# Dahan-Wang/Rethinking-Flow-and-Diffusion-Bridge-Models-for-Speech-Enhancement

Hardware: NVIDIA B200
Metric: enhanced audio-sec/sec (5-step SB bridge, ncsnpp_v2) (higher is better)
Workload: dtype fp16

## Files before the change

### include/fdbm_b200.h

```cpp
#ifndef FDBM_B200_H
#define FDBM_B200_H

#include <stddef.h>
#include <stdint.h>

#ifdef __cplusplus
extern "C" {
#endif

#define FDBM_OK        0
#define FDBM_EINVAL   -1
#define FDBM_ECUDA    -2
#define FDBM_EARCH    -3
#define FDBM_ESTATE   -4

#define FDBM_PAD_ZERO        0
#define FDBM_PAD_REFLECTION  1
#define FDBM_PAD_REPLICATION 2
#define FDBM_TRANSFORM_EXPONENT 0
#define FDBM_TRANSFORM_LOG      1
#define FDBM_TRANSFORM_NONE     2
#define FDBM_STEP_ODE 0
#define FDBM_STEP_SDE 1

const char* fdbm_last_error(void);
int fdbm_version(void);
int fdbm_check_device(void);
int fdbm_operand_is_bf16(void);

int fdbm_stft_compress(const float* wave, int batch, int64_t n_samples, int64_t wave_stride,
                       const float* window, int n_fft, int hop,
                       int transform_type, float spec_factor, float abs_exponent,
                       int pad_mode, int n_frames_out, float* spec, void* stream);

int fdbm_stft_compress_var(const float* wave, int batch, const int* lengths, int64_t min_samples, int64_t max_samples,
                           int64_t wave_stride, const float* window, int n_fft, int hop,
                           int transform_type, float spec_factor, float abs_exponent,
                           int pad_mode, int n_frames_out, float* spec, void* stream);

int fdbm_decompress_istft(const float* spec, int batch, int n_frames,
                          const float* window, int n_fft, int hop,
                          int transform_type, float spec_factor, float abs_exponent,
                          int64_t length, int64_t wave_stride, float* wave, void* stream);

int fdbm_decompress_istft_var(const float* spec, int batch, int n_frames,
                              const float* window, int n_fft, int hop,
                              int transform_type, float spec_factor, float abs_exponent,
                              const int* lengths, int64_t max_length, int64_t wave_stride, float* wave, void* stream);

int fdbm_wave_absmax(const float* wave, int batch, int64_t n_samples, const int* lengths, int64_t wave_stride, float* out,
                     void* stream);
int fdbm_stft_compress_ex(const float* wave, int batch, const int* lengths, int64_t min_samples, int64_t max_samples,
                          int64_t wave_stride, const float* window, const float* norm, int n_fft, int hop, int transform_type,
                          float spec_factor, float abs_exponent, int pad_mode, int n_frames_out, float* spec, void* stream);
int fdbm_decompress_istft_ex(const float* spec, int batch, int n_frames, const float* window, int n_fft, int hop,
                             int transform_type, float spec_factor, float abs_exponent, const int* lengths, int64_t max_length,
                             int64_t wave_stride, const float* norm, float* peak, float* wave, void* stream);
int fdbm_clip_rescale(float* wave, int batch, int64_t n_samples, const int* lengths, int64_t wave_stride, const float* peak,
                      float rescale, void* stream);

int fdbm_spec_transform(const float* in, float* out, int64_t n_complex, int transform_type, float spec_factor,
                        float abs_exponent, int inverse, void* stream);
int fdbm_pad_spec(const float* in, int64_t rows, int n_frames, int pad_mode, int n_frames_out, float* out,
                  void* stream);

int fdbm_prior_sample(const float* y, const float* z, float b, float sigma, uint64_t seed, uint64_t offset,
                      int64_t n_complex, float* x, void* stream);
int fdbm_bridge_update4(float* x, const float* d, const float* y, const float* z, const float* coef, uint64_t seed,
                        uint64_t offset, int64_t n_complex, float* x_mean_out, void* stream);
int fdbm_langevin_coef(const float* x, const float* d, const float* y, const float* z, float a, float b, float sigma,
                       float snr, uint64_t seed, uint64_t offset, int batch, int64_t n_per_utt, double* scratch,
                       float* coef_out, void* stream);
int fdbm_lincomb(float* out, const float* const* srcs, const float* coefs, int n_terms, int64_t n_floats, void* stream);
int fdbm_rk_error_norm(const float* const* srcs, const float* coefs, int n_terms, const float* y, const float* y_new,
                       float rtol, float atol, int64_t n_complex, double* out_sumsq, void* stream);
int fdbm_bridge_step(float* x, const float* d, const float* y_or_z, const float* coef, int kind,
                     uint64_t seed, uint64_t offset, int64_t n_complex, void* stream);

typedef struct fdbm_plan fdbm_plan;

typedef struct fdbm_tensor_ref {
  const char* name;
  const float* data;
  int64_t numel;
} fdbm_tensor_ref;

typedef struct fdbm_arch {
  int nf;
  int n_levels;
  int ch_mult[8];
  int num_res_blocks;
  int attn_resolution;
  int predictive;
  int image_size;
  int channel_block_real;
} fdbm_arch;

int fdbm_plan_create(const fdbm_arch* arch, int batch, int n_frames, fdbm_plan** out);
int fdbm_plan_destroy(fdbm_plan* plan);
int fdbm_plan_load_weights(fdbm_plan* plan, const fdbm_tensor_ref* tensors, int n_tensors, void* stream);
int64_t fdbm_plan_device_bytes(const fdbm_plan* plan);
int fdbm_plan_num_launches(const fdbm_plan* plan);

int fdbm_ncsnpp_forward(fdbm_plan* plan, const float* x, const float* y, const float* t, float* out,
                        void* stream);

int fdbm_sampler_run(fdbm_plan* plan, const float* y, float* x, const float* times, const float* coef,
                     int n_steps, int kind, const float* noise, uint64_t seed, void* stream);

int fdbm_plan_create_train(const fdbm_arch* arch, int batch, int n_frames, fdbm_plan** out);
int fdbm_ncsnpp_backward(fdbm_plan* plan, const float* g_out, float loss_scale, int accumulate, void* stream);
int fdbm_plan_param_info(const fdbm_plan* plan, const char* name, int64_t* offset, int64_t* numel);
int fdbm_plan_buffers(fdbm_plan* plan, float** params, float** grads, float** ema, int64_t* numel);
int fdbm_plan_repack_weights(fdbm_plan* plan, void* stream);
int fdbm_plan_num_backward_launches(const fdbm_plan* plan);
int fdbm_plan_profile_backward(fdbm_plan* plan, const float* g_out, float loss_scale, float* ms, int* kinds, int max_ops,
                               void* stream);
int fdbm_plan_optimizer_step(fdbm_plan* plan, float grad_div, float clip_norm, float lr, float beta1, float beta2,
                             float eps, int step, float ema_decay, int ema_warmup, void* stream);
int fdbm_plan_reset_optimizer(fdbm_plan* plan, void* stream);
int fdbm_plan_optimizer_state(fdbm_plan* plan, double* out, void* stream);
int fdbm_plan_set_optimizer_state(fdbm_plan* plan, double applied, double skipped, void* stream);
int fdbm_plan_swap_ema(fdbm_plan* plan, int to_ema, void* stream);

int64_t fdbm_hybrid_loss_workspace_bytes(int batch, int n_frames, int n_fft, int hop);
int fdbm_hybrid_loss(const float* x_hat, const float* x, int batch, int n_frames, const float* window, int n_fft, int hop,
                     int transform_type, float spec_factor, float abs_exponent, float loss_scale, void* workspace,
                     float* loss, float* g_out, void* stream);
int fdbm_data_prediction_loss(const float* x_hat, const float* x, int batch, int n_frames, const float* window, int n_fft, int hop,
                              int transform_type, float spec_factor, float abs_exponent, float l1_weight, float loss_scale,
                              void* workspace, float* loss, float* g_out, void* stream);
int64_t fdbm_mel_tables_bytes(void);
int fdbm_mel_tables_init(void* tables, int sample_rate, void* stream);
int64_t fdbm_mel_loss_workspace_bytes(int batch, int n_frames, int n_fft, int hop);
int fdbm_mel_loss(const float* x_hat, const float* x, int batch, int n_frames, const float* window, int n_fft, int hop,
                  int transform_type, float spec_factor, float abs_exponent, int with_phase, float loss_scale,
                  const void* tables, void* workspace, float* loss, float* g_out, void* stream);

int fdbm_pack_input(const float* x, const float* y, int batch, int n_frames, int f_in, int f_used, int c_in, float* out, void* stream);
int fdbm_im2col_input(const float* in, int c_in, int batch, int n_frames, int n_freq, void* out_h16, void* stream);
int fdbm_time_embedding(const float* t, const float* fourier_w, int nf, const float* w1, const float* b1, const float* w2,
                        const float* b2, int batch, float* out, void* stream);
int fdbm_film_rows(const float* temb_act, const float* weight, const float* bias, int batch, int k, int rows, float* out, void* stream);
int fdbm_combine(float* h, const float* pyramid, int c_pyr, const float* weight, const float* bias, int batch, int n_frames, int n_freq,
                 int channels, void* stream);
int fdbm_output_layer(const float* pyramid, int c_pyr, const float* weight, const float* bias, int batch, int n_frames, int n_freq,
                      int f_out, float* out, void* stream);

#define FDBM_OP_CONV   0
#define FDBM_OP_NORM   1
#define FDBM_OP_STATS  2
#define FDBM_OP_SKINNY 3
#define FDBM_OP_ATTN   4
#define FDBM_OP_SMALL  5
#define FDBM_OP_WGRAD  6
int fdbm_plan_profile_forward(fdbm_plan* plan, const float* x, const float* y, const float* t, float* out,
                              float* ms, int* kinds, double* flops, int max_ops, void* stream);


int fdbm_fir_resample(const float* in, int batch, int T, int F, int C, int mode, float* out, void* stream);

int fdbm_channel_stats(const float* in, int batch, int T, int F, int C, double* sums, void* stream);

int fdbm_groupnorm_act(const float* src1, const double* sums1, int C1,
                       const float* src2, const double* sums2, int C2,
                       const float* gamma, const float* beta, int batch, int T, int F,
                       int silu, int mode, void* act_out, void* raw_out, void* stream);

int fdbm_gn_resample_h16(const void* src1, const double* sums1, int C1, const void* src2, const double* sums2, int C2,
                         const float* gamma, const float* beta, float* table, int batch, int T, int F, int mode,
                         void* act_out, void* raw_out, void* stream);

int fdbm_conv_igemm(const void* in1, int C1, int ksize, const void* in2, int C2,
                    const void* wpack, const float* bias, const float* bias_b, const float* residual,
                    float scale, int batch, int T, int F, int Cout,
                    float* out_f32, void* out_h16, double* sums, void* stream);
int fdbm_conv_igemm_gn(const void* in1, int C1, int ksize, const double* sums1, const float* gamma,
                       const float* beta, int silu, float* table, const void* wpack, const float* bias,
                       const float* residual, float scale, int batch, int T, int F, int Cout,
                       float* out_f32, void* out_h16, double* sums, void* stream);
int fdbm_pack_conv_weights_dgrad(const float* w, int Cout, int Cin, int ksize, void* wpack, int64_t* bytes,
                                 void* stream);
int64_t fdbm_conv_wgrad_workspace_bytes(int Cout, int Cin, int ksize, int batch, int T, int F);
int fdbm_conv_wgrad(const void* dy, int Cout, const void* x, int Cin, int ksize, int batch, int T, int F,
                    float scale, float* dw, float* workspace, void* stream);

int fdbm_groupnorm_act_bwd(const void* g_a, const void* x, int x_is_h16, const double* sums, const float* gamma,
                           const float* beta, int silu, int batch, int T, int F, int C, float* table, double* S,
                           float* g_x_acc, void* g_x_h16, float* dgamma, float* dbeta, void* stream);
int fdbm_fir_resample_h16(const void* in, int batch, int T, int F, int C, int mode, float scale, void* out, void* stream);
int fdbm_attention_bwd(const void* qkv, int batch, int L, int C, const void* d_o, float* scratch, void* g_qkv, void* stream);
int fdbm_adam_ema_step(float* params, const float* grads, float* m, float* v, float* ema, int64_t n, double* scratch,
                       float grad_div, float clip_norm, float lr, float beta1, float beta2, float eps, int step,
                       float ema_decay, int ema_warmup, double* state, void* stream);

int fdbm_pack_conv_weights(const float* w1, int C1, int ksize, const float* w2, int C2, int Cout,
                           void* wpack, int64_t* bytes, void* stream);

int fdbm_attention(const void* q, const void* k, const void* v, int batch, int L, int C, void* o, void* stream);

int64_t fdbm_tfg_lstm_pack_bytes(void);
int fdbm_tfg_lstm_pack(const float* const* w, const float* w_lin, int hidden, void* packed, void* stream);
int fdbm_tfg_lstm_sweep(const void* xn, int n_seq, int L, const void* packed, void* y_fw, void* y_bw, void* stream);
int fdbm_tfg_pad_add_norm(const float* h, const float* emb, const float* gamma, const float* beta, int batch, int T, int Q, float eps,
                          float* xp, void* xn, void* stream);
int fdbm_tfg_sweep_post(const void* y_fw, const void* y_bw, const float* lin_bias, const float* resid, int batch, int T, int Q, int mode,
                        const float* gamma, const float* beta, float eps, float* out_full, void* xn, float* out_crop, int xn_transposed,
                        void* stream);
int fdbm_tfg_input(const float* x, const float* y, const float* w, const float* bias, const float* gn_w, const float* gn_b, int batch,
                   int T, int Q, int Cin, float eps, double* sums, float* out, void* stream);
int fdbm_tfg_time_embedding(const float* t, int t_stride, const float* fourier_w, const float* w1, const float* b1, const float* w2,
                            const float* b2, const float* w_blocks, const float* b_blocks, int n_layers, int batch, float* emb,
                            void* stream);
int64_t fdbm_tfg_attention_workspace_bytes(int batch, int T, int Q);
int fdbm_tfg_attention(const float* z, const float* const* params, int batch, int T, int Q, float eps, void* workspace, float* out,
                       void* stream);
int fdbm_tfg_output(const float* h, const float* w, const float* bias, int batch, int T, int Q, float* out, void* stream);

#ifdef __cplusplus
}
#endif
#endif
```

### rethinking-flow-and-diffusion-bridge-models-for-speech-enhancement_b200/csrc/common.cuh

```cuda
#pragma once
#include <cuda.h>
#include <cuda_runtime.h>
#include <cuda_bf16.h>
#include <cuda_fp16.h>
#include <stdint.h>
#include <stdio.h>
#include <string>
#include <algorithm>
#include "../../include/fdbm_b200.h"

namespace fdbm {

void set_error(const char* fmt, ...);
int cuda_fail(cudaError_t e, const char* what, const char* file, int line);

#define FDBM_CUDA(expr)                                                          \
  do {                                                                           \
    cudaError_t _e = (expr);                                                     \
    if (_e != cudaSuccess) return ::fdbm::cuda_fail(_e, #expr, __FILE__, __LINE__); \
  } while (0)

#define FDBM_REQUIRE(cond, ...)                \
  do {                                         \
    if (!(cond)) {                             \
      ::fdbm::set_error(__VA_ARGS__);          \
      return FDBM_EINVAL;                      \
    }                                          \
  } while (0)

#define FDBM_LAUNCH_CHECK() FDBM_CUDA(cudaGetLastError())

static inline cudaStream_t as_stream(void* s) { return reinterpret_cast<cudaStream_t>(s); }

int require_sm100();
__device__ __forceinline__ void pdl_wait_then_trigger() {
  asm volatile("griddepcontrol.wait;" ::: "memory");
  asm volatile("griddepcontrol.launch_dependents;" ::: "memory");
}
template <typename... KArgs, typename... Args>
inline cudaError_t launch_maybe_pdl(void (*kernel)(KArgs...), dim3 grid, dim3 block, size_t smem, cudaStream_t s, bool pdl, Args... args) {
  cudaLaunchConfig_t cfg = {};
  cfg.gridDim = grid; cfg.blockDim = block; cfg.dynamicSmemBytes = smem; cfg.stream = s;
  cudaLaunchAttribute attr[1];
  attr[0].id = cudaLaunchAttributeProgrammaticStreamSerialization;
  attr[0].val.programmaticStreamSerializationAllowed = 1;
  cfg.attrs = attr; cfg.numAttrs = pdl ? 1 : 0;
  return cudaLaunchKernelEx(&cfg, kernel, static_cast<KArgs>(args)...);
}
int pdl_batch_limit();
struct PdlBatchScope { int prev; explicit PdlBatchScope(int limit); ~PdlBatchScope(); PdlBatchScope(const PdlBatchScope&) = delete; };
bool pdl_enabled();
int num_sms();
int current_device();

struct PerDeviceOnce {
  bool done[64] = {};
  bool first(int dev) { if (dev < 0 || dev >= 64) return true; if (done[dev]) return false; done[dev] = true; return true; }
};

__host__ __device__ constexpr int ceil_div(int a, int b) { return (a + b - 1) / b; }
__host__ __device__ constexpr int64_t ceil_div64(int64_t a, int64_t b) { return (a + b - 1) / b; }

__device__ __forceinline__ float silu_f(float v) { return v / (1.0f + __expf(-v)); }

#ifdef FDBM_OPERAND_BF16
typedef __nv_bfloat16 op_t;
typedef __nv_bfloat162 op2_t;
constexpr int kOperandIsBf16 = 1;
__device__ __forceinline__ op_t f2op(float v) { return __float2bfloat16(v); }
__device__ __forceinline__ float op2f(op_t v) { return __bfloat162float(v); }
__device__ __forceinline__ op2_t f2op2(float a, float b) { return __floats2bfloat162_rn(a, b); }
__device__ __forceinline__ float2 op22f2(op2_t v) { return __bfloat1622float2(v); }
__device__ __forceinline__ op2_t op2_tanh(op2_t v) {
  uint32_t r; asm("tanh.approx.bf16x2 %0, %1;" : "=r"(r) : "r"(*reinterpret_cast<uint32_t*>(&v)));
  return *reinterpret_cast<op2_t*>(&r);
}
#else
typedef __half op_t;
typedef __half2 op2_t;
constexpr int kOperandIsBf16 = 0;
__device__ __forceinline__ float sat16(float v) { return fminf(fmaxf(v, -65504.0f), 65504.0f); }
__device__ __forceinline__ op_t f2op(float v) { return __float2half_rn(sat16(v)); }
__device__ __forceinline__ float op2f(op_t v) { return __half2float(v); }
__device__ __forceinline__ op2_t f2op2(float a, float b) {
  uint32_t r; asm("cvt.rn.satfinite.f16x2.f32 %0, %1, %2;" : "=r"(r) : "f"(b), "f"(a));
  return *reinterpret_cast<op2_t*>(&r);
}
__device__ __forceinline__ float2 op22f2(op2_t v) { return __half22float2(v); }
__device__ __forceinline__ op2_t op2_tanh(op2_t v) {
  uint32_t r; asm("tanh.approx.f16x2 %0, %1;" : "=r"(r) : "r"(*reinterpret_cast<uint32_t*>(&v)));
  return *reinterpret_cast<op2_t*>(&r);
}
#endif
__device__ __forceinline__ uint32_t pack_op2(float a, float b) {
  op2_t v = f2op2(a, b);
  return *reinterpret_cast<uint32_t*>(&v);
}

int launch_fir_resample(const float* in, int B, int T, int F, int C, int mode, float* out, cudaStream_t s);
int launch_fir_resample_scaled(const float* in, int B, int T, int F, int C, int mode, float scale, float* out, cudaStream_t s);
int launch_channel_stats(const float* in, int B, int T, int F, int C, double* sums, cudaStream_t s);
int launch_groupnorm_act(const void* src1, int src1_h16 , const double* sums1, int C1, const void* src2,
                         const double* sums2, int C2, const float* gamma, const float* beta, int B, int T, int F,
                         int silu, int mode, op_t* act_out, op_t* raw_out, cudaStream_t s);
int launch_pack_input(const float* x, const float* y, int B, int T, int F_in, int F, int Cin, float* out,
                      cudaStream_t s);
int launch_im2col_input(const float* in, int Cin, int B, int T, int F, op_t* out, cudaStream_t s);
int launch_combine(float* h, const float* pyr, int Cp, const float* w, const float* bias, int B, int T, int F,
                   int C, cudaStream_t s);
int launch_output_layer(const float* pyr, int Cp, const float* w, const float* bias, int B, int T, int F,
                        int F_out, float* out, cudaStream_t s);
int launch_temb(const float* t, const float* fourier_w, int nf, const float* w1, const float* b1, const float* w2,
                const float* b2, int B, int t_stride, float* temb_act, cudaStream_t s);
int launch_dense_all(const float* temb_act, const float* w, const float* bias, int B, int K, int rows, float* out,
                     cudaStream_t s);
int launch_gn_resample16(const op_t* src1, int C1, const op_t* src2, int C2, const float2* tab, int B, int T, int F,
                         int mode, op_t* act_out, op_t* raw_out, cudaStream_t s);
int launch_gn_finalize(const double* sums1, int C1, const double* sums2, int C2, const float* gamma, const float* beta,
                       int B, int64_t pixels, float2* table, cudaStream_t s, int blk_real = 0, float2* stats = nullptr);
int launch_attention(const op_t* q, const op_t* k, const op_t* v, int ld, int B, int L,
                     int C, op_t* o, int ldo, cudaStream_t s, int fp32_probs = 0);

struct ConvSeg {
  const op_t* in = nullptr; int C = 0; int taps = 9;
  const float2* norm_tab = nullptr; int tab_stride = 0; int act = 0;
};
struct ConvArgs {
  ConvSeg seg[3]; int n_seg = 0;
  const op_t* wpack = nullptr;
  const float* bias = nullptr; const float* bias_b = nullptr; int bias_b_stride = 0; const float* residual = nullptr;
  const op_t* residual_h16 = nullptr;
  float scale = 1.0f; int B = 0, T = 0, F = 0, Cout = 0;
  float* out_f32 = nullptr; op_t* out_h16 = nullptr;
  double* sums = nullptr;
  bool sums_prezeroed = false;
  float* pyr_out = nullptr; const float* pyr_prev = nullptr; int pyr_C = 0;
  bool narrow_n = false;
  const float* comb_pyr = nullptr; const float* comb_w = nullptr; const float* comb_b = nullptr; int comb_C = 0;
};
int launch_conv_igemm(const ConvArgs& a, cudaStream_t s);
int launch_pack_conv_weights_dgrad(const float* w, int Cout, int Cin, int ksize, op_t* wpack, cudaStream_t s, int Cin_total = 0,
                                   int ci_off = 0);
int64_t conv_wgrad_workspace_bytes(int Cout, int Cin, int ksize, int B, int T, int F);
int launch_conv_wgrad(const op_t* dy, int Cout, const op_t* x, int Cin, int ksize, int B, int T, int F, float scale,
                      int io_layout, float* dw, float* workspace, cudaStream_t s);
int launch_grad_prepare(const float* g, int B, int64_t P, int C, float scale, op_t* g16, float* acc_dst, double* sums, cudaStream_t s,
                        bool acc_first = false, bool sums_prezeroed = false);
int launch_gn_bwd_reduce(const op_t* g_a, int g_ld, int g_coff, const void* x, int x16, int C, int C_tot, int c_off,
                         const float2* tab, const float2* stats, int act, int B, int64_t P, double* S, cudaStream_t s, int b0 = 0);
int launch_gn_bwd_apply(const op_t* g_a, int g_ld, int g_coff, const void* x, int x16, int C, int C_tot, int c_off,
                        const float2* tab, const float2* stats, const float* gamma, int act, int B, int64_t P, const double* S,
                        float* acc_dst, op_t* out16, double* out_sums, cudaStream_t s, bool acc_first = false, int b0 = 0,
                        bool sums_prezeroed = false);
int launch_gn_param_grad(const double* S, int B, int C, float inv_scale, float* dgamma, float* dbeta, cudaStream_t s);
int launch_gn_stats(const double* sums1, int C1, const double* sums2, int C2, int B, int64_t pixels, float2* stats, cudaStream_t s);
int launch_fir_resample16(const op_t* in, int in_ld, int in_coff, int B, int T, int F, int C, int mode, float scale,
                          op_t* out16, float* acc_dst, cudaStream_t s);
int launch_col_sums16(const op_t* in, int ld, int c_off, int B, int64_t P, int C, double* sums, cudaStream_t s, bool sums_prezeroed = false);
int launch_col_sums_to(const double* sums, int B, int C, float inv_scale, float* dst, float* per_b, int per_b_ld, cudaStream_t s);
int launch_attention_bwd(const op_t* qkv, int B, int L, int C, const op_t* d_o, float* scratch, op_t* g_qkv, cudaStream_t s);
int launch_adam_ema(float* p, const float* g, float* m, float* v, float* ema, const unsigned char* trainable, int64_t n,
                    double* sumsq_scratch, float grad_div, float clip, float lr, float beta1, float beta2, float eps, int step,
                    float ema_decay, int ema_warmup, double* state, cudaStream_t s);
struct WgradCall {
  const op_t* dy = nullptr; int dy_ld = 0, dy_coff = 0, Cout = 0;
  const op_t* x = nullptr; int x_ld = 0, x_coff = 0, Cin = 0;
  int ksize = 3, B = 0, T = 0, F = 0;
  float scale = 1.0f;
  int layout = 0, Cin_total = 0, ci_off = 0, aux = 0;
  float* dw = nullptr; float* workspace = nullptr;
};
int launch_conv_wgrad_ex(const WgradCall& c, cudaStream_t s);
int launch_output_layer_bwd(const float* g_out, const float* pyr, int Cp, const float* w, int B, int T, int F, int F_out, float inv,
                            float* g_pyr, float* dw, float* db, cudaStream_t s);
int launch_small_col_sums(const float* g, int64_t n_px, int Cp, float inv, float* db, cudaStream_t s);
int launch_combine_bwd(const float* g, const float* pyr, int Cp, int64_t n_px, int C, float inv, float* dw, float* db, cudaStream_t s);
int launch_pack_pyr_dgrad(const float* w, int C, int Cp, op_t* out, cudaStream_t s);
int launch_dense_temb_bwd(const float* d, const float* act, const float* w, int B, int K, int rows, float* dw, float* db, float* g_act,
                          const float* t, const float* fw, int nf, const float* w1, const float* b1, const float* w2, const float* b2,
                          int t_stride, float* dw1, float* db1, float* dw2, float* db2, cudaStream_t s);
int make_act_tile_map(CUtensorMap* map, const op_t* ptr, int B, int T, int F, int C, int box_f, int box_t);
int64_t conv_wpack_bytes(int C1, int ksize, int C2, int Cout);
int launch_pack_conv_weights(const float* w1, int C1, int ksize, const float* w2, int C2, int Cout, int n_rows_total,
                             int row_offset, op_t* wpack, cudaStream_t s);
struct PackDesc {
  const float* w1; const float* w2; op_t* out;
  int kind;
  int C1, ksize, io, C2, Cout, rows_total, row_offset;
  long long total;
  long long first_block;
};
struct DeferDesc {
  const double* src; int B, C, kind;
  float* dst0; float* dst1; float* per_b; int per_b_ld;
};
int launch_deferred_sums(const DeferDesc* descs_dev, int n_descs, float inv_scale, cudaStream_t s);
constexpr int kPackChunk = 2048;
PackDesc pack_desc_fwd(const float* w1, int C1, int ksize, const float* w2, int C2, int Cout, int n_rows_total, int row_offset, op_t* wpack);
PackDesc pack_desc_dgrad(const float* w, int Cout, int Cin, int ksize, op_t* wpack, int Cin_total, int ci_off);
int launch_pack_batch(const PackDesc* descs_dev, int n_descs, long long n_blocks, cudaStream_t s);

}
```

### rethinking-flow-and-diffusion-bridge-models-for-speech-enhancement_b200/csrc/conv_igemm.cu

```cuda
#include <cuda.h>
#include <mutex>
#include <type_traits>
#include "common.cuh"
#include "tc05.cuh"

namespace fdbm {
int make_act_tile_map(CUtensorMap* map, const op_t* ptr, int B, int T, int F, int C, int box_f, int box_t);
namespace {

using namespace tc05;

constexpr int MT = 2;
constexpr int TILE_T = 16, TILE_F = 8;
constexpr int HALO_T = TILE_T + 2, HALO_F = TILE_F + 2;
constexpr int A_TILE_BYTES = HALO_T * HALO_F * 128;
constexpr int A_TILE_STRIDE = 23552;
#ifndef FDBM_A_STAGES
#define FDBM_A_STAGES 3
#define FDBM_B_STAGES 3
#endif
constexpr int A_STAGES = FDBM_A_STAGES;
constexpr int B_STAGES = FDBM_B_STAGES;
constexpr int BN = 128;
constexpr int B_TILE_BYTES = BN * 128;
constexpr int A_SBO = HALO_F * 128;
constexpr int NUM_THREADS = 512;
constexpr int EPI_GROUPS = 2;
constexpr int MAX_SEG = 3;
constexpr int MAX_KB = 16;
constexpr int A_TILE1_BYTES = TILE_T * TILE_F * 128;
constexpr int PIPE_REGS = 56, EPI_REGS = 168, XFORM_REGS = 120;
#ifndef FDBM_SIDE_RING_DEFAULT
#define FDBM_SIDE_RING_DEFAULT 1
#endif
#ifndef FDBM_EPI_RES2
#define FDBM_EPI_RES2 1
#endif
constexpr int STAGE_BYTES = EPI_GROUPS * 4 * 32 * 32 * 4;
constexpr int STAT_SLOTS = 2;
constexpr int STAT_BYTES = EPI_GROUPS * 4 * BN * 8;
constexpr int B_STAGES_NARROW = B_STAGES * B_TILE_BYTES / (16 * 128);
constexpr int SMEM_BYTES = A_STAGES * MT * A_TILE_STRIDE + B_STAGES * B_TILE_BYTES + STAGE_BYTES + STAT_BYTES + 512;

struct SegParams {
  int taps, norm, act, tab_stride;
  int halo;
  const float2* tab;
};

struct ConvParams {
  int B, T, F, Cout;
  int n_seg, n_kb;
  SegParams seg[MAX_SEG];
  uint32_t ksched[MAX_KB];
  int tiles_t, tiles_f, n_mtiles, n_nblocks, n_items;
  uint32_t mg_tiles_t, mg_tiles_f, mg_nblocks;
  int bn;
  int side_ring, n_main, side_gap, n_steps;
  const float* bias;
  const float* bias_b;
  int bias_b_stride;
  const float* residual;
  const op_t* residual_h16;
  float scale;
  float* out_f32;
  op_t* out_h16;
  double* sums;
  float* pyr_out;
  const float* pyr_prev;
  int pyr_C;
  const float* comb_pyr;
  const float* comb_w;
  const float* comb_b;
  int comb_C;
};

struct TileCoord { int b, t0, f0; bool valid; };

__device__ __forceinline__ int fast_div(int n, int d, uint32_t mg) { return d == 1 ? n : static_cast<int>(__umulhi(static_cast<uint32_t>(n), mg)); }
__device__ __forceinline__ int item_tile(const ConvParams& p, int item) { return fast_div(item, p.n_nblocks, p.mg_nblocks); }
__device__ __forceinline__ int item_nblk(const ConvParams& p, int item) { return item - item_tile(p, item) * p.n_nblocks; }

__device__ __forceinline__ TileCoord decode_tile(const ConvParams& p, int mi) {
  TileCoord c;
  c.valid = mi < p.n_mtiles;
  const int rest = fast_div(mi, p.tiles_t, p.mg_tiles_t);
  const int tt = mi - rest * p.tiles_t;
  c.t0 = tt * TILE_T;
  c.b = fast_div(rest, p.tiles_f, p.mg_tiles_f);
  c.f0 = (rest - c.b * p.tiles_f) * TILE_F;
  return c;
}

template <typename F>
__device__ __forceinline__ void walk_steps(const ConvParams& p, F&& f) {
  const int n_side = p.n_kb - p.n_main;
  int sd = 0, cnt = 0;
  for (int m = 0; m < p.n_main; ++m) {
    const int ntaps = p.seg[p.ksched[m] & 15].taps;
    for (int tap = 0; tap < ntaps; ++tap) {
      f(false, m, tap, ntaps);
      if (++cnt == p.side_gap && sd < n_side) { f(true, p.n_main + sd, 0, 1); ++sd; cnt = 0; }
    }
  }
  for (; sd < n_side; ++sd) f(true, p.n_main + sd, 0, 1);
}

template <bool COMB, bool RES16>
__global__ void __launch_bounds__(NUM_THREADS, 1)
conv_igemm_kernel(const __grid_constant__ CUtensorMap map_a0, const __grid_constant__ CUtensorMap map_a1,
                  const __grid_constant__ CUtensorMap map_a2, const __grid_constant__ CUtensorMap map_b,
                  const ConvParams p) {
  extern __shared__ __align__(1024) uint8_t smem_raw[];
  uint8_t* smem = smem_raw;
  if (smem_u32(smem_raw) & 1023u) __trap();
  uint8_t* sA = smem;
  uint8_t* sB = smem + A_STAGES * MT * A_TILE_STRIDE;
  uint8_t* s_stage = sB + B_STAGES * B_TILE_BYTES;
  uint8_t* s_stat = s_stage + STAGE_BYTES;
  uint64_t* bars = reinterpret_cast<uint64_t*>(s_stage + STAGE_BYTES + STAT_BYTES);
  uint64_t* a_full = bars;
  uint64_t* a_empty = a_full + A_STAGES;
  uint64_t* b_full = a_empty + A_STAGES;
  uint64_t* b_empty = b_full + B_STAGES_NARROW;
  uint64_t* acc_full = b_empty + B_STAGES_NARROW;
  const int b_stages = p.bn == 16 ? B_STAGES_NARROW : B_STAGES;
  const int b_stride = p.bn * 128;
  uint64_t* acc_empty = acc_full + 2;
  uint64_t* a_ready = acc_empty + 2;
  uint64_t* side_full = a_ready + A_STAGES;
  uint64_t* side_empty = side_full + 1;
  uint32_t* tmem_slot = reinterpret_cast<uint32_t*>(side_empty + 1);
  static_assert((3 * A_STAGES + 2 * B_STAGES_NARROW + 4 + 2) * 8 + 4 <= 512, "barrier region");
  const int a_stages = p.side_ring ? A_STAGES - 1 : A_STAGES;
  const int n_main = p.side_ring ? p.n_main : p.n_kb;

  const int warp = __shfl_sync(0xffffffffu, static_cast<int>(threadIdx.x >> 5), 0), lane = threadIdx.x & 31;
  const int n_kb = p.n_kb;

  if (threadIdx.x == 0) {
    for (int i = 0; i < A_STAGES; ++i) { mbar_init(a_full + i, 1); mbar_init(a_empty + i, 1); mbar_init(a_ready + i, 128); }
    for (int i = 0; i < B_STAGES_NARROW; ++i) { mbar_init(b_full + i, 1); mbar_init(b_empty + i, 1); }
    for (int i = 0; i < 2; ++i) { mbar_init(acc_full + i, 1); mbar_init(acc_empty + i, 4 * EPI_GROUPS); }
    mbar_init(side_full, 1); mbar_init(side_empty, 1);
    fence_barrier_init();
  }
  if (warp == 0 && lane == 0) {
    tma_prefetch_desc(&map_a0);
    tma_prefetch_desc(&map_b);
    if (p.n_seg > 1) tma_prefetch_desc(&map_a1);
    if (p.n_seg > 2) tma_prefetch_desc(&map_a2);
  }
  if (warp == 3) {
    tmem_alloc(tmem_slot, 512);
    tmem_relinquish();
  }
  fence_before_sync();
  __syncthreads();
  fence_after_sync();
  const uint32_t tmem_base = *tmem_slot;
  asm volatile("griddepcontrol.wait;" ::: "memory");
  asm volatile("griddepcontrol.launch_dependents;" ::: "memory");

  if (warp < 4) {
  reg_dec<PIPE_REGS>();
  if (warp == 0) {
    if (lane == 0) {
      uint32_t stage = 0, phase = 0;
      for (int item = blockIdx.x; item < p.n_items; item += gridDim.x) {
        const int ct = item_tile(p, item);
        TileCoord tc[MT];
        int n_valid = 0;
        for (int j = 0; j < MT; ++j) { tc[j] = decode_tile(p, ct * MT + j); n_valid += tc[j].valid; }
        for (int i = 0; i < n_main; ++i) {
          const uint32_t e = p.ksched[i];
          const int sgi = e & 15, c0 = ((e >> 4) & 0xFFF) * 64;
          const int halo = p.seg[sgi].halo;
          mbar_wait_relaxed<256>(a_empty + stage, phase ^ 1);
          mbar_expect_tx(a_full + stage, n_valid * (halo ? A_TILE_BYTES : A_TILE1_BYTES));
          const CUtensorMap* map = sgi == 0 ? &map_a0 : (sgi == 1 ? &map_a1 : &map_a2);
          for (int j = 0; j < MT; ++j) {
            if (!tc[j].valid) continue;
            tma_load_4d(sA + (stage * MT + j) * A_TILE_STRIDE, map, a_full + stage, c0, tc[j].f0 - halo, tc[j].t0 - halo,
                        tc[j].b);
          }
          if (++stage == a_stages) { stage = 0; phase ^= 1; }
        }
      }
    }
  } else if (warp == 3) {
    if (lane == 0 && p.side_ring) {
      uint32_t phase = 0;
      for (int item = blockIdx.x; item < p.n_items; item += gridDim.x) {
        const int ct = item_tile(p, item);
        TileCoord tc[MT];
        int n_valid = 0;
        for (int j = 0; j < MT; ++j) { tc[j] = decode_tile(p, ct * MT + j); n_valid += tc[j].valid; }
        for (int i = n_main; i < n_kb; ++i) {
          const uint32_t e = p.ksched[i];
          const int sgi = e & 15, c0 = ((e >> 4) & 0xFFF) * 64;
          mbar_wait_relaxed<128>(side_empty, phase ^ 1);
          mbar_expect_tx(side_full, n_valid * A_TILE1_BYTES);
          const CUtensorMap* map = sgi == 0 ? &map_a0 : (sgi == 1 ? &map_a1 : &map_a2);
          for (int j = 0; j < MT; ++j) {
            if (!tc[j].valid) continue;
            tma_load_4d(sA + ((A_STAGES - 1) * MT + j) * A_TILE_STRIDE, map, side_full, c0, tc[j].f0, tc[j].t0, tc[j].b);
          }
          phase ^= 1;
        }
      }
    }
  } else if (warp == 1) {
    if (lane == 0) {
      uint32_t stage = 0, phase = 0;
      for (int item = blockIdx.x; item < p.n_items; item += gridDim.x) {
        const int n0 = item_nblk(p, item) * BN;
        if (p.side_ring) {
          walk_steps(p, [&](bool, int idx, int tap, int) {
            const int kt = static_cast<int>(p.ksched[idx] >> 16) + tap;
            mbar_wait_relaxed<128>(b_empty + stage, phase ^ 1);
            mbar_expect_tx(b_full + stage, b_stride);
            tma_load_2d(sB + stage * b_stride, &map_b, b_full + stage, 0, kt * p.Cout + n0);
            if (++stage == b_stages) { stage = 0; phase ^= 1; }
          });
          continue;
        }
        for (int i = 0; i < n_kb; ++i) {
          const uint32_t e = p.ksched[i];
          const int ntaps = p.seg[e & 15].taps;
          int kt = e >> 16;
          for (int tap = 0; tap < ntaps; ++tap, ++kt) {
            mbar_wait_relaxed<128>(b_empty + stage, phase ^ 1);
            mbar_expect_tx(b_full + stage, b_stride);
            tma_load_2d(sB + stage * b_stride, &map_b, b_full + stage, 0, kt * p.Cout + n0);
            if (++stage == b_stages) { stage = 0; phase ^= 1; }
          }
        }
      }
    }
  } else if (warp == 2) {
    const uint32_t idesc = make_idesc_f16(128, p.bn, kOperandIsBf16);
    const uint64_t a_hi9 = make_desc_sw128(0, A_SBO) & 0xFFFFFFFF00000000ull;
    const uint64_t a_hi1 = make_desc_sw128(0, TILE_F * 128) & 0xFFFFFFFF00000000ull;
    const uint64_t b_hi = make_desc_sw128(0, 1024) & 0xFFFFFFFF00000000ull;
    const uint32_t lo_const = 1u << 16;
    const uint32_t sA_lo = (smem_u32(sA) & 0x3FFFF) >> 4, sB_lo = (smem_u32(sB) & 0x3FFFF) >> 4;
    uint32_t sa = 0, pa = 0, sb = 0, pb = 0, as = 0, pacc = 0, ps = 0;
    for (int item = blockIdx.x; item < p.n_items; item += gridDim.x) {
      const int ct = item_tile(p, item);
      const bool valid1 = (ct * MT + 1) < p.n_mtiles;
      mbar_wait(acc_empty + as, pacc ^ 1);
      fence_after_sync();
      uint32_t accumulate = 0;
      const uint32_t d0 = tmem_base + (as * MT) * BN, d1 = d0 + BN;
      if (p.side_ring) {
        int step = 0;
        walk_steps(p, [&](bool side, int idx, int tap, int ntaps) {
          const SegParams& sg = p.seg[p.ksched[idx] & 15];
          uint32_t a_base0, a_off = 0;
          if (side) {
            mbar_wait(side_full, ps);
            fence_after_sync();
            a_base0 = sA_lo + (((A_STAGES - 1) * MT) * A_TILE_STRIDE >> 4);
          } else {
            if (tap == 0) {
              mbar_wait(sg.norm ? a_ready + sa : a_full + sa, pa);
              fence_after_sync();
            }
            a_base0 = sA_lo + ((sa * MT) * A_TILE_STRIDE >> 4);
            const int df = ntaps == 9 ? tap / 3 : sg.halo, dt = ntaps == 9 ? tap - 3 * (tap / 3) : sg.halo;
            a_off = ((dt * HALO_F + df) * 128) >> 4;
          }
          const uint64_t a_hi = sg.halo ? a_hi9 : a_hi1;
          mbar_wait(b_full + sb, pb);
          fence_after_sync();
          const uint32_t b_lo = (sB_lo + (sb * b_stride >> 4)) | lo_const;
          const uint32_t a_lo0 = (a_base0 + a_off) | lo_const, a_lo1 = (a_base0 + (A_TILE_STRIDE >> 4) + a_off) | lo_const;
          const bool last_tap = tap == ntaps - 1;
          if (elect_one()) {
#pragma unroll
            for (int k = 0; k < 4; ++k)
              mma_f16(d0, a_hi | (a_lo0 + 2 * k), b_hi | (b_lo + 2 * k), idesc, k == 0 ? accumulate : 1u);
            if (valid1) {
#pragma unroll
              for (int k = 0; k < 4; ++k)
                mma_f16(d1, a_hi | (a_lo1 + 2 * k), b_hi | (b_lo + 2 * k), idesc, k == 0 ? accumulate : 1u);
            }
            mma_commit(b_empty + sb);
            if (side) mma_commit(side_empty);
            else if (last_tap) mma_commit(a_empty + sa);
            if (step == p.n_steps - 1) mma_commit(acc_full + as);
          }
          __syncwarp();
          accumulate = 1;
          ++step;
          if (++sb == b_stages) { sb = 0; pb ^= 1; }
          if (side) ps ^= 1;
          else if (last_tap && ++sa == a_stages) { sa = 0; pa ^= 1; }
        });
        if (++as == 2) { as = 0; pacc ^= 1; }
        continue;
      }
      for (int i = 0; i < n_kb; ++i) {
        const SegParams& sg = p.seg[p.ksched[i] & 15];
        const int ntaps = sg.taps;
        const uint64_t a_hi = sg.halo ? a_hi9 : a_hi1;
        mbar_wait(sg.norm ? a_ready + sa : a_full + sa, pa);
        fence_after_sync();
        const uint32_t a_base0 = sA_lo + ((sa * MT) * A_TILE_STRIDE >> 4), a_base1 = a_base0 + (A_TILE_STRIDE >> 4);
        int df = ntaps == 9 ? 0 : sg.halo, dt = df;
        for (int tap = 0; tap < ntaps; ++tap) {
          mbar_wait(b_full + sb, pb);
          fence_after_sync();
          const uint32_t a_off = ((dt * HALO_F + df) * 128) >> 4;
          const uint32_t b_lo = (sB_lo + (sb * b_stride >> 4)) | lo_const;
          const uint32_t a_lo0 = (a_base0 + a_off) | lo_const, a_lo1 = (a_base1 + a_off) | lo_const;
          if (elect_one()) {
#ifdef FDBM_MMA_WS
            if (valid1 && p.bn == BN) {
              mma_f16_ws<0, 0>(d0, a_hi | (a_lo0 + 0), b_hi | (b_lo + 0), idesc, accumulate);
              mma_f16_ws<1, 0>(d0, a_hi | (a_lo0 + 2), b_hi | (b_lo + 2), idesc, 1u);
              mma_f16_ws<2, 0>(d0, a_hi | (a_lo0 + 4), b_hi | (b_lo + 4), idesc, 1u);
              mma_f16_ws<3, 0>(d0, a_hi | (a_lo0 + 6), b_hi | (b_lo + 6), idesc, 1u);
              mma_f16_ws<0, 1>(d1, a_hi | (a_lo1 + 0), b_hi | (b_lo + 0), idesc, accumulate);
              mma_f16_ws<1, 1>(d1, a_hi | (a_lo1 + 2), b_hi | (b_lo + 2), idesc, 1u);
              mma_f16_ws<2, 1>(d1, a_hi | (a_lo1 + 4), b_hi | (b_lo + 4), idesc, 1u);
              mma_f16_ws<3, 1>(d1, a_hi | (a_lo1 + 6), b_hi | (b_lo + 6), idesc, 1u);
            } else
#endif
            {
#pragma unroll
              for (int k = 0; k < 4; ++k)
                mma_f16(d0, a_hi | (a_lo0 + 2 * k), b_hi | (b_lo + 2 * k), idesc, k == 0 ? accumulate : 1u);
              if (valid1) {
#pragma unroll
                for (int k = 0; k < 4; ++k)
                  mma_f16(d1, a_hi | (a_lo1 + 2 * k), b_hi | (b_lo + 2 * k), idesc, k == 0 ? accumulate : 1u);
              }
            }
            mma_commit(b_empty + sb);
            if (tap == ntaps - 1) mma_commit(a_empty + sa);
            if (tap == ntaps - 1 && i == n_kb - 1) mma_commit(acc_full + as);
          }
          __syncwarp();
          accumulate = 1;
          if (++dt == 3) { dt = 0; ++df; }
          if (++sb == b_stages) { sb = 0; pb ^= 1; }
        }
        if (++sa == A_STAGES) { sa = 0; pa ^= 1; }
      }
      if (++as == 2) { as = 0; pacc ^= 1; }
    }
  }
  } else if (warp >= 8 && warp < 12) {
    reg_dec<XFORM_REGS>();
    const int tt = threadIdx.x - 256;
    const int g = tt & 7, p_lane = tt >> 3;
    uint32_t stage = 0, phase = 0;
    const bool any_norm = (p.seg[0].norm | p.seg[1].norm | p.seg[2].norm) != 0;
    for (int item = blockIdx.x; any_norm && item < p.n_items; item += gridDim.x) {
      const int ct = item_tile(p, item);
      TileCoord tc[MT];
      for (int j = 0; j < MT; ++j) tc[j] = decode_tile(p, ct * MT + j);
      for (int i = 0; i < n_main; ++i) {
        const uint32_t e = p.ksched[i];
        const SegParams& sg = p.seg[e & 15];
        float2 sc[MT][4], sh[MT][4];
        if (sg.norm) {
          const int c0 = ((e >> 4) & 0xFFF) * 64 + g * 8;
          const float pre = sg.act ? 0.5f : 1.0f;
#pragma unroll
          for (int j = 0; j < MT; ++j) {
            const float4* tp = reinterpret_cast<const float4*>(sg.tab + static_cast<int64_t>(tc[j].valid ? tc[j].b : 0) * sg.tab_stride + c0);
#pragma unroll
            for (int u = 0; u < 4; ++u) {
              const float4 e = __ldg(tp + u);
              sc[j][u] = make_float2(pre * e.x, pre * e.z); sh[j][u] = make_float2(pre * e.y, pre * e.w);
            }
          }
        }
        mbar_wait_relaxed(a_full + stage, phase);
        if (sg.norm) {
#pragma unroll
          for (int j = 0; j < MT; ++j) {
            if (!tc[j].valid) continue;
            const int r_lo = tc[j].t0 == 0 ? 1 : 0, r_hi = min(HALO_T, p.T - tc[j].t0 + 1);
            const int c_lo = tc[j].f0 == 0 ? 1 : 0, c_hi = min(HALO_F, p.F - tc[j].f0 + 1);
            const bool interior = r_lo == 0 && c_lo == 0 && r_hi == HALO_T && c_hi == HALO_F;
            uint8_t* tile = sA + (stage * MT + j) * A_TILE_STRIDE;
            constexpr int N_PASS = (HALO_T * HALO_F + 63) / 64;
            auto xform = [&](uint4& rawv, auto act_tag) {
              constexpr bool ACT = decltype(act_tag)::value;
              op2_t* h2 = reinterpret_cast<op2_t*>(&rawv);
#pragma unroll
              for (int w = 0; w < 4; ++w) {
                const float2 y = __ffma2_rn(op22f2(h2[w]), sc[j][w], sh[j][w]);
                if (ACT) {
#ifdef FDBM_XF_EXACT
                  const float y0 = 2.0f * y.x, y1 = 2.0f * y.y;
                  h2[w] = f2op2(__fdividef(y0, 1.0f + __expf(-y0)), __fdividef(y1, 1.0f + __expf(-y1)));
#else
                  const op2_t h = f2op2(y.x, y.y);
                  h2[w] = __hfma2(h, op2_tanh(h), h);
#endif
                } else {
                  h2[w] = f2op2(y.x, y.y);
                }
              }
            };
            auto run_interior = [&](auto act_tag) {
              uint8_t* base = tile + p_lane * 128 + ((g ^ (p_lane & 7)) << 4);
#pragma unroll
              for (int pass = 0; pass < N_PASS; ++pass) {
                uint4 raw[4];
#pragma unroll
                for (int u = 0; u < 4; ++u) {
                  const int i = pass * 4 + u;
                  if (i < 11 || p_lane < 4) raw[u] = *reinterpret_cast<uint4*>(base + i * 2048);
                }
#pragma unroll
                for (int u = 0; u < 4; ++u) xform(raw[u], act_tag);
#pragma unroll
                for (int u = 0; u < 4; ++u) {
                  const int i = pass * 4 + u;
                  if (i < 11 || p_lane < 4) *reinterpret_cast<uint4*>(base + i * 2048) = raw[u];
                }
              }
            };
            auto run_border = [&](auto act_tag) {
#pragma unroll 1
              for (int pass = 0; pass < N_PASS; ++pass) {
                uint4 raw[4];
                uint4* slot[4];
                bool on[4];
#pragma unroll
                for (int u = 0; u < 4; ++u) {
                  const int px = p_lane + 16 * (pass * 4 + u);
                  const int hr = px / HALO_F, hc = px - hr * HALO_F;
                  on[u] = px < HALO_T * HALO_F && hr >= r_lo && hr < r_hi && hc >= c_lo && hc < c_hi;
                  slot[u] = reinterpret_cast<uint4*>(tile + px * 128 + ((g ^ (px & 7)) << 4));
                  raw[u] = on[u] ? *slot[u] : make_uint4(0u, 0u, 0u, 0u);
                }
#pragma unroll
                for (int u = 0; u < 4; ++u) xform(raw[u], act_tag);
#pragma unroll
                for (int u = 0; u < 4; ++u)
                  if (on[u]) *slot[u] = raw[u];
              }
            };
            if (interior) { if (sg.act) run_interior(std::true_type{}); else run_interior(std::false_type{}); }
            else { if (sg.act) run_border(std::true_type{}); else run_border(std::false_type{}); }
          }
          fence_proxy_async();
        }
        mbar_arrive(a_ready + stage);
        if (++stage == a_stages) { stage = 0; phase ^= 1; }
      }
    }
  } else {
    reg_inc<EPI_REGS>();
    const int q = warp & 3;
    const int eg = warp >= 12 ? 1 : 0;
    float4* stage = reinterpret_cast<float4*>(s_stage) + (eg * 4 + q) * (32 * 8);
    const int cc = lane & 7;
    const int rsub = lane >> 3;
    const int et = (threadIdx.x & 127);
    uint32_t as = 0, pacc = 0;
    const bool do_stats = p.sums != nullptr;
    float2* wstat = reinterpret_cast<float2*>(s_stat) + eg * 4 * BN;
    double acc_s[STAT_SLOTS], acc_q[STAT_SLOTS];
#pragma unroll
    for (int u = 0; u < STAT_SLOTS; ++u) { acc_s[u] = 0.0; acc_q[u] = 0.0; }
    int stat_b = -1;
    auto flush_stats = [&]() {
#pragma unroll
      for (int u = 0; u < STAT_SLOTS; ++u) {
        if (u < p.n_nblocks) {
          if (et < p.bn) {
            double* dst = p.sums + (static_cast<int64_t>(stat_b) * p.Cout + u * BN + et) * 2;
            atomicAdd(dst, acc_s[u]);
            atomicAdd(dst + 1, acc_q[u]);
          }
        }
        acc_s[u] = 0.0; acc_q[u] = 0.0;
      }
    };
    for (int item = blockIdx.x; item < p.n_items; item += gridDim.x) {
      const int ct = item_tile(p, item);
      const int nblk = item - ct * p.n_nblocks;
      const int n0 = nblk * BN;
      mbar_wait_relaxed(acc_full + as, pacc);
      fence_after_sync();
      for (int j = eg; j <= eg; ++j) {
        const TileCoord tc = decode_tile(p, ct * MT + j);
        if (!tc.valid) continue;
#if defined(FDBM_EPI_TEST)
        {
#if FDBM_EPI_TEST == 1
          uint32_t acc = 0;
#pragma unroll
          for (int ch = 0; ch < BN / 32; ++ch) {
            uint32_t v[32];
            tmem_ld_32x32(tmem_base + ((q * 32u) << 16) + (as * MT + j) * BN + ch * 32, v);
            tmem_ld_wait();
#pragma unroll
            for (int u = 0; u < 32; ++u) acc ^= v[u];
          }
          if (acc == 0x12345678u && p.out_h16) p.out_h16[0] = op_t(0);
#endif
          continue;
        }
#endif
        if (do_stats && stat_b != tc.b) {
          if (stat_b >= 0) flush_stats();
          stat_b = tc.b;
        }
        if (p.pyr_out) {
          uint32_t v[32];
          tmem_ld_32x32(tmem_base + ((q * 32u) << 16) + (as * MT + j) * BN, v);
          tmem_ld_wait();
          const int m = q * 32 + lane;
          const int t = tc.t0 + (m >> 3), f = tc.f0 + (m & 7);
          if (t < p.T && f < p.F) {
            float o[4];
#pragma unroll
            for (int c = 0; c < 4; ++c) o[c] = c < p.pyr_C ? __uint_as_float(v[c]) + __ldg(p.bias + c) : 0.f;
            if (p.pyr_prev) {
              const int Tp = p.T >> 1, Fp = p.F >> 1;
              const int t_a = (t & 1) ? (t >> 1) : (t >> 1) - 1, f_a = (f & 1) ? (f >> 1) : (f >> 1) - 1;
              const float wt_a = (t & 1) ? 0.75f : 0.25f, wf_a = (f & 1) ? 0.75f : 0.25f;
              const float* pb = p.pyr_prev + static_cast<int64_t>(tc.b) * Tp * Fp * p.pyr_C;
              if (p.pyr_C == 4) {
                float4 tap[4];
                float wg[4];
#pragma unroll
                for (int u = 0; u < 2; ++u)
#pragma unroll
                  for (int w = 0; w < 2; ++w) {
                    const int tt = t_a + u, ff = f_a + w;
                    const bool ok = tt >= 0 && tt < Tp && ff >= 0 && ff < Fp;
                    wg[u * 2 + w] = ok ? (u ? 1.0f - wt_a : wt_a) * (w ? 1.0f - wf_a : wf_a) : 0.f;
                    tap[u * 2 + w] = ok ? __ldg(reinterpret_cast<const float4*>(pb + (static_cast<int64_t>(tt) * Fp + ff) * 4))
                                        : make_float4(0.f, 0.f, 0.f, 0.f);
                  }
#pragma unroll
                for (int k = 0; k < 4; ++k) {
                  o[0] = fmaf(wg[k], tap[k].x, o[0]); o[1] = fmaf(wg[k], tap[k].y, o[1]);
                  o[2] = fmaf(wg[k], tap[k].z, o[2]); o[3] = fmaf(wg[k], tap[k].w, o[3]);
                }
              } else {
#pragma unroll
                for (int u = 0; u < 2; ++u) {
                  const int tt = t_a + u;
                  if (tt < 0 || tt >= Tp) continue;
                  const float wt = u ? 1.0f - wt_a : wt_a;
#pragma unroll
                  for (int w = 0; w < 2; ++w) {
                    const int ff = f_a + w;
                    if (ff < 0 || ff >= Fp) continue;
                    const float wgt = wt * (w ? 1.0f - wf_a : wf_a);
                    const float* src = pb + (static_cast<int64_t>(tt) * Fp + ff) * p.pyr_C;
                    for (int c = 0; c < p.pyr_C; ++c) o[c] = fmaf(wgt, __ldg(src + c), o[c]);
                  }
                }
              }
            }
            float* dst = p.pyr_out + ((static_cast<int64_t>(tc.b) * p.T + t) * p.F + f) * p.pyr_C;
            if (p.pyr_C == 4) *reinterpret_cast<float4*>(dst) = make_float4(o[0], o[1], o[2], o[3]);
            else for (int c = 0; c < p.pyr_C; ++c) dst[c] = o[c];
          }
          continue;
        }
        const bool full = tc.t0 + TILE_T <= p.T && tc.f0 + TILE_F <= p.F;
        const int64_t tile_base = ((static_cast<int64_t>(tc.b) * p.T + tc.t0) * p.F + tc.f0) * p.Cout + n0 + cc * 4;
        const int roff0 = ((q * 4) * p.F + rsub) * p.Cout, roff_t = p.F * p.Cout, roff_f = 4 * p.Cout;
        auto roff = [&](int it) { return roff0 + (it >> 1) * roff_t + (it & 1) * roff_f; };
        uint32_t okmask = 0;
#pragma unroll
        for (int it = 0; it < 8; ++it) {
          const int m = q * 32 + it * 4 + rsub;
          const bool ok = tc.t0 + (m >> 3) < p.T && tc.f0 + (m & 7) < p.F;
          okmask |= ok ? (1u << it) : 0u;
        }
        const float* res_p = !RES16 && p.residual ? p.residual + tile_base : nullptr;
        const op_t* res16_p = RES16 ? p.residual_h16 + tile_base : nullptr;
        float* of_p = p.out_f32 ? p.out_f32 + tile_base : nullptr;
        op_t* oh_p = p.out_h16 ? p.out_h16 + tile_base : nullptr;
        if (RES16 || res_p) {
          const int nitem = item + gridDim.x;
          const int nct = item_tile(p, nitem);
          const int nmi = nitem < p.n_items ? nct * MT + j : p.n_mtiles;
          const int nblk_n = nitem - nct * p.n_nblocks;
          const TileCoord nt = decode_tile(p, nmi);
          const int t = nt.t0 + (et >> 3), f = nt.f0 + (et & 7);
          if (nt.valid && t < p.T && f < p.F) {
            const int64_t po = ((static_cast<int64_t>(nt.b) * p.T + t) * p.F + f) * p.Cout + nblk_n * BN;
            if (RES16) {
#pragma unroll
              for (int u = 0; u < 2; ++u) asm volatile("prefetch.global.L2 [%0];" ::"l"(p.residual_h16 + po + u * 64));
            } else {
#pragma unroll
              for (int u = 0; u < 4; ++u) asm volatile("prefetch.global.L2 [%0];" ::"l"(p.residual + po + u * 32));
            }
          }
        }
        const float2 sc2 = make_float2(p.scale, p.scale);
        const float* bias_p = p.bias + n0 + cc * 4;
        const float* biasb_p = p.bias_b ? p.bias_b + static_cast<int64_t>(tc.b) * p.bias_b_stride + n0 + cc * 4 : nullptr;
        float4 bv = __ldg(reinterpret_cast<const float4*>(bias_p));
        float4 bvb = biasb_p ? __ldg(reinterpret_cast<const float4*>(biasb_p)) : make_float4(0.f, 0.f, 0.f, 0.f);
        float4 res[8];
#if FDBM_EPI_RES2
        uint2 res16_buf[2][8];
#define res16 res16_buf[ch & 1]
        auto load_res16 = [&](int ch) {
          uint2 (&dst)[8] = res16_buf[ch & 1];
          if (full) {
#pragma unroll
            for (int it = 0; it < 8; ++it) dst[it] = __ldg(reinterpret_cast<const uint2*>(res16_p + roff(it) + ch * 32));
          } else {
#pragma unroll
            for (int it = 0; it < 8; ++it)
              dst[it] = ((okmask >> it) & 1) ? __ldg(reinterpret_cast<const uint2*>(res16_p + roff(it) + ch * 32)) : make_uint2(0u, 0u);
          }
        };
        if (RES16) load_res16(0);
#else
        uint2 res16[8];
        auto load_res16 = [&](int ch) {
          if (full) {
#pragma unroll
            for (int it = 0; it < 8; ++it) res16[it] = __ldg(reinterpret_cast<const uint2*>(res16_p + roff(it) + ch * 32));
          } else {
#pragma unroll
            for (int it = 0; it < 8; ++it)
              res16[it] = ((okmask >> it) & 1) ? __ldg(reinterpret_cast<const uint2*>(res16_p + roff(it) + ch * 32)) : make_uint2(0u, 0u);
          }
        };
#endif
        auto load_res = [&](float4 (&r)[8], int ch) {
          if (full) {
#pragma unroll
            for (int it = 0; it < 8; ++it) r[it] = __ldg(reinterpret_cast<const float4*>(res_p + roff(it) + ch * 32));
          } else {
#pragma unroll
            for (int it = 0; it < 8; ++it)
              r[it] = ((okmask >> it) & 1) ? __ldg(reinterpret_cast<const float4*>(res_p + roff(it) + ch * 32))
                                           : make_float4(0.f, 0.f, 0.f, 0.f);
          }
        };
        const int n_chunks = p.bn >> 5;
#pragma unroll
        for (int ch = 0; ch < BN / 32; ++ch) {
          if (ch >= n_chunks) break;
          float4 cw[4], cbias = make_float4(0.f, 0.f, 0.f, 0.f);
          if constexpr (COMB) {
            const int c = n0 + ch * 32 + cc * 4;
            cbias = __ldg(reinterpret_cast<const float4*>(p.comb_b + c));
#pragma unroll
            for (int u = 0; u < 4; ++u) {
              const float* wr = p.comb_w + (c + u) * p.comb_C;
              cw[u] = make_float4(__ldg(wr), p.comb_C > 1 ? __ldg(wr + 1) : 0.f, p.comb_C > 2 ? __ldg(wr + 2) : 0.f,
                                  p.comb_C > 3 ? __ldg(wr + 3) : 0.f);
            }
          }
          float4 bvn = bv, bvbn = bvb;
          if (ch + 1 < n_chunks) {
            bvn = __ldg(reinterpret_cast<const float4*>(bias_p + (ch + 1) * 32));
            if (biasb_p) bvbn = __ldg(reinterpret_cast<const float4*>(biasb_p + (ch + 1) * 32));
          }
          uint32_t v[32];
          tmem_ld_32x32(tmem_base + ((q * 32u) << 16) + (as * MT + j) * BN + ch * 32, v);
#if FDBM_EPI_RES2
          if (RES16) { if (ch + 1 < n_chunks) load_res16(ch + 1); }
          else if (res_p) load_res(res, ch);
#else
          if (RES16) { if (ch == 0) load_res16(0); }
          else if (res_p) load_res(res, ch);
#endif
          tmem_ld_wait();
#pragma unroll
          for (int g = 0; g < 8; ++g)
            stage[lane * 8 + (g ^ (lane & 7))] = make_float4(__uint_as_float(v[4 * g]), __uint_as_float(v[4 * g + 1]),
                                                             __uint_as_float(v[4 * g + 2]), __uint_as_float(v[4 * g + 3]));
          __syncwarp();
          const float2 bs_lo = __fmul2_rn(make_float2(bv.x + bvb.x, bv.y + bvb.y), sc2), bs_hi = __fmul2_rn(make_float2(bv.z + bvb.z, bv.w + bvb.w), sc2);
          float2 o_lo[8], o_hi[8];
#pragma unroll
          for (int it = 0; it < 8; ++it) {
            const int rr = it * 4 + rsub;
            const float4 a = stage[rr * 8 + (cc ^ (rr & 7))];
            o_lo[it] = make_float2(a.x, a.y); o_hi[it] = make_float2(a.z, a.w);
          }
#pragma unroll
          for (int it = 0; it < 8; ++it) {
            o_lo[it] = __ffma2_rn(o_lo[it], sc2, bs_lo); o_hi[it] = __ffma2_rn(o_hi[it], sc2, bs_hi);
            if (RES16) {
              const op2_t* r2 = reinterpret_cast<const op2_t*>(&res16[it]);
              o_lo[it] = __ffma2_rn(op22f2(r2[0]), sc2, o_lo[it]);
              o_hi[it] = __ffma2_rn(op22f2(r2[1]), sc2, o_hi[it]);
            } else if (res_p) {
              o_lo[it] = __ffma2_rn(make_float2(res[it].x, res[it].y), sc2, o_lo[it]);
              o_hi[it] = __ffma2_rn(make_float2(res[it].z, res[it].w), sc2, o_hi[it]);
            }
            if (COMB && (full || ((okmask >> it) & 1))) {
              const int m = q * 32 + it * 4 + rsub;
              const float* pq = p.comb_pyr + ((static_cast<int64_t>(tc.b) * p.T + tc.t0 + (m >> 3)) * p.F + tc.f0 + (m & 7)) * p.comb_C;
              const float p0 = __ldg(pq), p1 = p.comb_C > 1 ? __ldg(pq + 1) : 0.f, p2 = p.comb_C > 2 ? __ldg(pq + 2) : 0.f,
                          p3 = p.comb_C > 3 ? __ldg(pq + 3) : 0.f;
              o_lo[it].x += cbias.x + cw[0].x * p0 + cw[0].y * p1 + cw[0].z * p2 + cw[0].w * p3;
              o_lo[it].y += cbias.y + cw[1].x * p0 + cw[1].y * p1 + cw[1].z * p2 + cw[1].w * p3;
              o_hi[it].x += cbias.z + cw[2].x * p0 + cw[2].y * p1 + cw[2].z * p2 + cw[2].w * p3;
              o_hi[it].y += cbias.w + cw[3].x * p0 + cw[3].y * p1 + cw[3].z * p2 + cw[3].w * p3;
            }
          }
#if !FDBM_EPI_RES2
          if (RES16 && ch + 1 < n_chunks) load_res16(ch + 1);
#endif
          float2 ssum_lo = make_float2(0.f, 0.f), ssum_hi = ssum_lo, ssq_lo = ssum_lo, ssq_hi = ssum_lo;
          if (full) {
            if (of_p) {
#pragma unroll
              for (int it = 0; it < 8; ++it)
                *reinterpret_cast<float4*>(of_p + roff(it) + ch * 32) = make_float4(o_lo[it].x, o_lo[it].y, o_hi[it].x, o_hi[it].y);
            }
            if (oh_p) {
#pragma unroll
              for (int it = 0; it < 8; ++it)
                *reinterpret_cast<uint2*>(oh_p + roff(it) + ch * 32) = make_uint2(pack_op2(o_lo[it].x, o_lo[it].y), pack_op2(o_hi[it].x, o_hi[it].y));
            }
#pragma unroll
            for (int it = 0; it < 8; ++it) {
              ssum_lo = __fadd2_rn(ssum_lo, o_lo[it]); ssum_hi = __fadd2_rn(ssum_hi, o_hi[it]);
              ssq_lo = __ffma2_rn(o_lo[it], o_lo[it], ssq_lo); ssq_hi = __ffma2_rn(o_hi[it], o_hi[it], ssq_hi);
            }
          } else {
#pragma unroll
            for (int it = 0; it < 8; ++it) {
              if ((okmask >> it) & 1) {
                if (of_p) *reinterpret_cast<float4*>(of_p + roff(it) + ch * 32) = make_float4(o_lo[it].x, o_lo[it].y, o_hi[it].x, o_hi[it].y);
                if (oh_p) *reinterpret_cast<uint2*>(oh_p + roff(it) + ch * 32) = make_uint2(pack_op2(o_lo[it].x, o_lo[it].y), pack_op2(o_hi[it].x, o_hi[it].y));
                ssum_lo = __fadd2_rn(ssum_lo, o_lo[it]); ssum_hi = __fadd2_rn(ssum_hi, o_hi[it]);
                ssq_lo = __ffma2_rn(o_lo[it], o_lo[it], ssq_lo); ssq_hi = __ffma2_rn(o_hi[it], o_hi[it], ssq_hi);
              }
            }
          }
          float4 ssum = make_float4(ssum_lo.x, ssum_lo.y, ssum_hi.x, ssum_hi.y), ssq = make_float4(ssq_lo.x, ssq_lo.y, ssq_hi.x, ssq_hi.y);
          if (do_stats) {
#pragma unroll
            for (int sft = 8; sft <= 16; sft <<= 1) {
              ssum.x += __shfl_xor_sync(0xffffffffu, ssum.x, sft); ssum.y += __shfl_xor_sync(0xffffffffu, ssum.y, sft);
              ssum.z += __shfl_xor_sync(0xffffffffu, ssum.z, sft); ssum.w += __shfl_xor_sync(0xffffffffu, ssum.w, sft);
              ssq.x += __shfl_xor_sync(0xffffffffu, ssq.x, sft); ssq.y += __shfl_xor_sync(0xffffffffu, ssq.y, sft);
              ssq.z += __shfl_xor_sync(0xffffffffu, ssq.z, sft); ssq.w += __shfl_xor_sync(0xffffffffu, ssq.w, sft);
            }
            if (rsub == 0) {
              float4* d = reinterpret_cast<float4*>(wstat + q * BN + ch * 32 + cc * 4);
              d[0] = make_float4(ssum.x, ssq.x, ssum.y, ssq.y);
              d[1] = make_float4(ssum.z, ssq.z, ssum.w, ssq.w);
            }
          }
          __syncwarp();
          bv = bvn; bvb = bvbn;
        }
#if FDBM_EPI_RES2
#undef res16
#endif
        if (do_stats) {
          asm volatile("bar.sync %0, 128;" ::"r"(1 + eg) : "memory");
          double s = 0.0, sq = 0.0;
#pragma unroll
          for (int w = 0; w < 4; ++w) { const float2 e = et < p.bn ? wstat[w * BN + et] : make_float2(0.f, 0.f); s += e.x; sq += e.y; }
#pragma unroll
          for (int u = 0; u < STAT_SLOTS; ++u) if (u == nblk) { acc_s[u] += s; acc_q[u] += sq; }
          asm volatile("bar.sync %0, 128;" ::"r"(1 + eg) : "memory");
        }
      }
      fence_before_sync();
      __syncwarp();
      if (lane == 0) mbar_arrive(acc_empty + as);
      if (++as == 2) { as = 0; pacc ^= 1; }
    }
    if (do_stats && stat_b >= 0) flush_stats();
  }

  fence_before_sync();
  __syncthreads();
  if (warp == 3) tmem_dealloc(tmem_base, 512);
}

__device__ __forceinline__ void pack_fwd_element(const PackDesc& d, int64_t i) {
  const int C1 = d.C1, C2 = d.C2, Cout = d.Cout, ksize = d.ksize, io_layout = d.io;
  const int taps = ksize * ksize;
  const int j = static_cast<int>(i % 64);
  const int co = static_cast<int>((i / 64) % Cout);
  const int kt = static_cast<int>(i / (64ll * Cout));
  float v;
  if (io_layout == 2) {
    const int tap = j / C1, ci = j % C1;
    v = tap < 9 ? d.w1[((static_cast<int64_t>(co) * C1 + ci) * 3 + tap / 3) * 3 + tap % 3] : 0.f;
  } else if (kt < (C1 / 64) * taps) {
    const int kb = kt / taps, tap = kt % taps;
    const int ci = kb * 64 + j;
    if (io_layout) v = d.w1[static_cast<int64_t>(ci) * Cout + co];
    else {
      const int kf = ksize == 3 ? tap / 3 : 0, ktm = ksize == 3 ? tap % 3 : 0;
      v = d.w1[((static_cast<int64_t>(co) * C1 + ci) * ksize + kf) * ksize + ktm];
    }
  } else {
    const int ci = (kt - (C1 / 64) * taps) * 64 + j;
    v = d.w2[static_cast<int64_t>(co) * C2 + ci];
  }
  d.out[(static_cast<int64_t>(kt) * d.rows_total + d.row_offset + co) * 64 + j] = f2op(v);
}

__device__ __forceinline__ void pack_dgrad_element(const PackDesc& d, int64_t i) {
  const int Cin = d.C1, Cin_total = d.C2, Cout = d.Cout, ksize = d.ksize, ci_off = d.row_offset;
  const int taps = ksize * ksize;
  const int j = static_cast<int>(i % 64);
  const int ci = static_cast<int>((i / 64) % Cin);
  const int kt = static_cast<int>(i / (64ll * Cin));
  const int kb = kt / taps, tap = kt % taps;
  const int co = kb * 64 + j;
  float v;
  if (d.io) v = d.w1[static_cast<int64_t>(ci_off + ci) * Cout + co];
  else {
    const int kf = ksize == 3 ? 2 - tap / 3 : 0, ktm = ksize == 3 ? 2 - tap % 3 : 0;
    v = d.w1[((static_cast<int64_t>(co) * Cin_total + ci_off + ci) * ksize + kf) * ksize + ktm];
  }
  d.out[i] = f2op(v);
}

__global__ void __launch_bounds__(256)
pack_batch_kernel(const PackDesc* __restrict__ descs, int n) {
  __shared__ PackDesc d;
  if (threadIdx.x == 0) {
    int lo = 0, hi = n - 1;
    while (lo < hi) { const int mid = (lo + hi + 1) >> 1; if (descs[mid].first_block <= static_cast<long long>(blockIdx.x)) lo = mid; else hi = mid - 1; }
    d = descs[lo];
  }
  __syncthreads();
  const int64_t i0 = (static_cast<int64_t>(blockIdx.x) - d.first_block) * kPackChunk;
#pragma unroll 1
  for (int u = 0; u < kPackChunk / 256; ++u) {
    const int64_t i = i0 + u * 256 + threadIdx.x;
    if (i < d.total) { if (d.kind == 0) pack_fwd_element(d, i); else pack_dgrad_element(d, i); }
  }
}

typedef CUresult (*EncodeFn)(CUtensorMap*, CUtensorMapDataType, cuuint32_t, void*, const cuuint64_t*, const cuuint64_t*,
                             const cuuint32_t*, const cuuint32_t*, CUtensorMapInterleave, CUtensorMapSwizzle,
                             CUtensorMapL2promotion, CUtensorMapFloatOOBfill);

EncodeFn get_encode() {
  static EncodeFn fn = nullptr;
  static std::once_flag once;
  std::call_once(once, [] {
    void* p = nullptr;
    cudaDriverEntryPointQueryResult q;
    if (cudaGetDriverEntryPoint("cuTensorMapEncodeTiled", &p, cudaEnableDefault, &q) == cudaSuccess &&
        q == cudaDriverEntryPointSuccess)
      fn = reinterpret_cast<EncodeFn>(p);
  });
  return fn;
}

int make_act_map(CUtensorMap* map, const op_t* ptr, int B, int T, int F, int C) {
  return make_act_tile_map(map, ptr, B, T, F, C, HALO_F, HALO_T);
}

int make_weight_map(CUtensorMap* map, const op_t* ptr, int64_t rows, int bn) {
  EncodeFn enc = get_encode();
  if (!enc) { set_error("cuTensorMapEncodeTiled entry point not available"); return FDBM_ECUDA; }
  cuuint64_t dims[2] = {64, (cuuint64_t)rows};
  cuuint64_t strides[1] = {128};
  cuuint32_t box[2] = {64, (cuuint32_t)bn};
  cuuint32_t es[2] = {1, 1};
  CUresult r = enc(map, (kOperandIsBf16 ? CU_TENSOR_MAP_DATA_TYPE_BFLOAT16 : CU_TENSOR_MAP_DATA_TYPE_FLOAT16), 2, const_cast<op_t*>(ptr), dims, strides, box, es,
                   CU_TENSOR_MAP_INTERLEAVE_NONE, CU_TENSOR_MAP_SWIZZLE_128B, CU_TENSOR_MAP_L2_PROMOTION_L2_256B,
                   CU_TENSOR_MAP_FLOAT_OOB_FILL_NONE);
  if (r != CUDA_SUCCESS) { set_error("cuTensorMapEncodeTiled(weights, %lld rows) failed: %d", (long long)rows, (int)r); return FDBM_ECUDA; }
  return FDBM_OK;
}

}

int make_act_tile_map(CUtensorMap* map, const op_t* ptr, int B, int T, int F, int C, int box_f, int box_t) {
  EncodeFn enc = get_encode();
  if (!enc) { set_error("cuTensorMapEncodeTiled entry point not available"); return FDBM_ECUDA; }
  cuuint64_t dims[4] = {(cuuint64_t)C, (cuuint64_t)F, (cuuint64_t)T, (cuuint64_t)B};
  cuuint64_t strides[3] = {(cuuint64_t)C * 2, (cuuint64_t)C * 2 * F, (cuuint64_t)C * 2 * F * T};
  cuuint32_t box[4] = {64, (cuuint32_t)box_f, (cuuint32_t)box_t, 1};
  cuuint32_t es[4] = {1, 1, 1, 1};
  CUresult r = enc(map, (kOperandIsBf16 ? CU_TENSOR_MAP_DATA_TYPE_BFLOAT16 : CU_TENSOR_MAP_DATA_TYPE_FLOAT16), 4, const_cast<op_t*>(ptr), dims, strides, box, es,
                   CU_TENSOR_MAP_INTERLEAVE_NONE, CU_TENSOR_MAP_SWIZZLE_128B, CU_TENSOR_MAP_L2_PROMOTION_L2_256B,
                   CU_TENSOR_MAP_FLOAT_OOB_FILL_NONE);
  if (r != CUDA_SUCCESS) { set_error("cuTensorMapEncodeTiled(activation [%d,%d,%d,%d]) failed: %d", B, T, F, C, (int)r); return FDBM_ECUDA; }
  return FDBM_OK;
}

int64_t conv_wpack_bytes(int C1, int ksize, int C2, int Cout) {
  return (static_cast<int64_t>(C1 / 64) * ksize * ksize + C2 / 64) * Cout * 64 * 2;
}

PackDesc pack_desc_fwd(const float* w1, int C1, int ksize, const float* w2, int C2, int Cout, int n_rows_total, int row_offset, op_t* wpack) {
  const int io = ksize == -1 ? 1 : (ksize == -2 ? 2 : 0);
  const int k = io ? 1 : ksize;
  PackDesc d{};
  d.w1 = w1; d.w2 = w2; d.out = wpack; d.kind = 0; d.C1 = C1; d.ksize = k; d.io = io; d.C2 = C2; d.Cout = Cout;
  d.rows_total = n_rows_total; d.row_offset = row_offset;
  d.total = io == 2 ? static_cast<long long>(Cout) * 64 : (static_cast<long long>(C1 / 64) * k * k + C2 / 64) * Cout * 64;
  return d;
}
PackDesc pack_desc_dgrad(const float* w, int Cout, int Cin, int ksize, op_t* wpack, int Cin_total, int ci_off) {
  const int k = ksize == -1 ? 1 : ksize;
  PackDesc d{};
  d.w1 = w; d.w2 = nullptr; d.out = wpack; d.kind = 1; d.C1 = Cin; d.ksize = k; d.io = ksize == -1; d.C2 = Cin_total ? Cin_total : Cin; d.Cout = Cout;
  d.rows_total = 0; d.row_offset = ci_off;
  d.total = static_cast<long long>(Cout / 64) * k * k * Cin * 64;
  return d;
}
int launch_pack_batch(const PackDesc* descs_dev, int n_descs, long long n_blocks, cudaStream_t s) {
  if (n_descs <= 0 || n_blocks <= 0) return FDBM_OK;
  pack_batch_kernel<<<static_cast<unsigned>(n_blocks), 256, 0, s>>>(descs_dev, n_descs);
  FDBM_LAUNCH_CHECK();
  return FDBM_OK;
}

__global__ void __launch_bounds__(256) pack_one_kernel(const PackDesc d) {
  for (int64_t i = blockIdx.x * 256ll + threadIdx.x; i < d.total; i += 256ll * gridDim.x) {
    if (d.kind == 0) pack_fwd_element(d, i); else pack_dgrad_element(d, i);
  }
}

int launch_pack_conv_weights(const float* w1, int C1, int ksize, const float* w2, int C2, int Cout, int n_rows_total,
                             int row_offset, op_t* wpack, cudaStream_t s) {
  FDBM_REQUIRE((ksize == -2 && C1 <= 4 && C2 == 0) ||
               (C1 % 64 == 0 && C2 % 64 == 0 && (ksize == 1 || ksize == 3 || ksize == -1)),
               "pack_conv_weights: channels must be multiples of 64, ksize 1 or 3");
  const PackDesc d = pack_desc_fwd(w1, C1, ksize, w2, C2, Cout, n_rows_total, row_offset, wpack);
  pack_one_kernel<<<static_cast<int>(std::min<int64_t>(ceil_div64(d.total, 256), 4096)), 256, 0, s>>>(d);
  FDBM_LAUNCH_CHECK();
  return FDBM_OK;
}

int launch_pack_conv_weights_dgrad(const float* w, int Cout, int Cin, int ksize, op_t* wpack, cudaStream_t s, int Cin_total, int ci_off) {
  FDBM_REQUIRE(Cout % 64 == 0 && Cin % 64 == 0 && (ksize == 1 || ksize == 3 || ksize == -1),
               "pack_conv_weights_dgrad: channels must be multiples of 64, ksize 1, 3 or -1 (NIN)");
  const PackDesc d = pack_desc_dgrad(w, Cout, Cin, ksize, wpack, Cin_total, ci_off);
  pack_one_kernel<<<static_cast<int>(std::min<int64_t>(ceil_div64(d.total, 256), 4096)), 256, 0, s>>>(d);
  FDBM_LAUNCH_CHECK();
  return FDBM_OK;
}

int launch_conv_igemm(const ConvArgs& a, cudaStream_t s) {
  FDBM_REQUIRE(a.n_seg >= 1 && a.n_seg <= MAX_SEG, "conv_igemm: 1..%d K segments", MAX_SEG);
  const int bn = a.narrow_n ? 16 : (a.Cout == 64 ? 64 : BN);
  FDBM_REQUIRE(a.Cout % bn == 0 && (!a.narrow_n || (a.Cout == 16 && a.pyr_out)), "conv_igemm: Cout must be a multiple of %d (got %d)", bn, a.Cout);
  FDBM_REQUIRE(a.out_f32 || a.out_h16 || a.pyr_out, "conv_igemm: no output");
  FDBM_REQUIRE(!a.pyr_out || (a.pyr_C >= 1 && a.pyr_C <= 4 && a.Cout == bn && !a.sums), "conv_igemm: bad pyramid epilogue arguments");
  FDBM_REQUIRE(!a.pyr_prev || (a.T % 2 == 0 && a.F % 2 == 0), "conv_igemm: pyramid level with odd size");
  static PerDeviceOnce attr_once;
  if (attr_once.first(current_device())) {
    FDBM_CUDA(cudaFuncSetAttribute(conv_igemm_kernel<false, false>, cudaFuncAttributeMaxDynamicSharedMemorySize, SMEM_BYTES));
    FDBM_CUDA(cudaFuncSetAttribute(conv_igemm_kernel<false, true>, cudaFuncAttributeMaxDynamicSharedMemorySize, SMEM_BYTES));
    FDBM_CUDA(cudaFuncSetAttribute(conv_igemm_kernel<true, false>, cudaFuncAttributeMaxDynamicSharedMemorySize, SMEM_BYTES));
  }
  FDBM_REQUIRE(!a.comb_pyr || (a.comb_w && a.comb_b && a.comb_C >= 1 && a.comb_C <= 4 && !a.pyr_out), "conv_igemm: bad Combine epilogue arguments");
  CUtensorMap map_a[MAX_SEG], map_b;
  ConvParams p;
  p.B = a.B; p.T = a.T; p.F = a.F; p.Cout = a.Cout;
  p.n_seg = a.n_seg;
  int kb = 0, n_kt = 0;
  for (int i = 0; i < MAX_SEG; ++i) {
    if (i < a.n_seg) {
      const ConvSeg& sg = a.seg[i];
      FDBM_REQUIRE(sg.in && sg.C > 0 && sg.C % 64 == 0 && (sg.taps == 9 || sg.taps == 1),
                   "conv_igemm: segment %d needs a tensor, C %% 64 == 0 and 9 or 1 taps (C=%d, taps=%d)", i, sg.C, sg.taps);
      const int halo = sg.taps == 9 || sg.norm_tab != nullptr;
      if (int rc = halo ? make_act_map(&map_a[i], sg.in, a.B, a.T, a.F, sg.C)
                        : make_act_tile_map(&map_a[i], sg.in, a.B, a.T, a.F, sg.C, TILE_F, TILE_T)) return rc;
      p.seg[i].halo = halo;
      kb += sg.C / 64; p.seg[i].taps = sg.taps;
      p.seg[i].norm = sg.norm_tab != nullptr; p.seg[i].act = sg.act; p.seg[i].tab = sg.norm_tab;
      p.seg[i].tab_stride = sg.tab_stride;
      n_kt += (sg.C / 64) * sg.taps;
    } else {
      map_a[i] = map_a[0];
      p.seg[i] = SegParams{1, 0, 0, 0, 0, nullptr};
    }
  }
  p.n_kb = kb;
  FDBM_REQUIRE(kb <= MAX_KB, "conv_igemm: at most %d K-blocks (got %d)", MAX_KB, kb);
  {
    uint32_t nine[MAX_KB], one[MAX_KB];
    int n9 = 0, n1 = 0, kt = 0;
    for (int i = 0; i < a.n_seg; ++i)
      for (int cb = 0; cb < a.seg[i].C / 64; ++cb) {
        const uint32_t e = static_cast<uint32_t>(i) | (static_cast<uint32_t>(cb) << 4) | (static_cast<uint32_t>(kt) << 16);
        if (a.seg[i].taps == 9) nine[n9++] = e; else one[n1++] = e;
        kt += a.seg[i].taps;
      }
    static const int order = getenv("FDBM_KSCHED") ? atoi(getenv("FDBM_KSCHED")) : 0;
    int n = 0;
    if (order == 1) {
      for (int i = 0; i < n1; ++i) p.ksched[n++] = one[i];
      for (int i = 0; i < n9; ++i) p.ksched[n++] = nine[i];
    } else if (order == 2 && n9 > 0) {
      p.ksched[n++] = nine[0];
      for (int i = 0; i < n1; ++i) p.ksched[n++] = one[i];
      for (int i = 1; i < n9; ++i) p.ksched[n++] = nine[i];
    } else {
      for (int i = 0; i < n9; ++i) p.ksched[n++] = nine[i];
      for (int i = 0; i < n1; ++i) p.ksched[n++] = one[i];
    }
    for (; n < MAX_KB; ++n) p.ksched[n] = 0;
    bool side_ok = order == 0 && n1 > 0 && n9 > 0;
    for (int i = 0; i < a.n_seg; ++i) side_ok = side_ok && (a.seg[i].taps == 9 || !p.seg[i].halo);
    static const int side_env = getenv("FDBM_SIDE_RING") ? atoi(getenv("FDBM_SIDE_RING")) : FDBM_SIDE_RING_DEFAULT;
    p.side_ring = side_ok && side_env ? 1 : 0;
    p.n_main = p.side_ring ? n9 : kb;
    p.side_gap = p.side_ring ? std::max(3, ceil_div(9 * n9, n1)) : 0;
    p.n_steps = n_kt;
  }
  if (int rc = make_weight_map(&map_b, a.wpack, static_cast<int64_t>(n_kt) * a.Cout, bn)) return rc;
  p.bn = bn;
  p.tiles_t = ceil_div(a.T, TILE_T); p.tiles_f = ceil_div(a.F, TILE_F);
  p.n_mtiles = a.B * p.tiles_t * p.tiles_f;
  p.n_nblocks = a.Cout / bn;
  p.n_items = ceil_div(p.n_mtiles, MT) * p.n_nblocks;
  {
    auto magic = [](int d) { return static_cast<uint32_t>((0x100000000ull + d - 1) / static_cast<uint64_t>(d)); };
    p.mg_tiles_t = magic(p.tiles_t); p.mg_tiles_f = magic(p.tiles_f); p.mg_nblocks = magic(p.n_nblocks);
    const int64_t dmax = std::max(std::max(p.tiles_t, p.tiles_f), p.n_nblocks);
    FDBM_REQUIRE((2 * (static_cast<int64_t>(p.n_items) + num_sms()) + 2) * dmax < 0x100000000ll, "conv_igemm: %d items exceed the range of the index arithmetic", p.n_items);
  }
  p.bias = a.bias; p.bias_b = a.bias_b; p.bias_b_stride = a.bias_b_stride; p.residual = a.residual; p.scale = a.scale;
  p.residual_h16 = a.residual_h16;
  FDBM_REQUIRE(!(a.residual && a.residual_h16) && !(a.residual_h16 && (a.comb_pyr || a.pyr_out)), "conv_igemm: bad residual arguments");
  p.out_f32 = a.out_f32; p.out_h16 = a.out_h16; p.sums = a.sums;
  p.pyr_out = a.pyr_out; p.pyr_prev = a.pyr_prev; p.pyr_C = a.pyr_C;
  p.comb_pyr = a.comb_pyr; p.comb_w = a.comb_w; p.comb_b = a.comb_b; p.comb_C = a.comb_C;
  if (a.sums) {
    FDBM_REQUIRE(p.n_nblocks <= STAT_SLOTS, "conv_igemm: channel sums support Cout <= %d", STAT_SLOTS * BN);
    if (!a.sums_prezeroed) FDBM_CUDA(cudaMemsetAsync(a.sums, 0, sizeof(double) * 2 * a.B * a.Cout, s));
  }
  const int grid = std::min(p.n_items, num_sms());
  cudaLaunchConfig_t cfg = {};
  cfg.gridDim = dim3(grid); cfg.blockDim = dim3(NUM_THREADS); cfg.dynamicSmemBytes = SMEM_BYTES; cfg.stream = s;
  cudaLaunchAttribute attr[1];
  attr[0].id = cudaLaunchAttributeProgrammaticStreamSerialization;
  attr[0].val.programmaticStreamSerializationAllowed = 1;
  cfg.attrs = attr; cfg.numAttrs = pdl_enabled() && a.B <= pdl_batch_limit() ? 1 : 0;
  if (a.comb_pyr) FDBM_CUDA(cudaLaunchKernelEx(&cfg, conv_igemm_kernel<true, false>, map_a[0], map_a[1], map_a[2], map_b, p));
  else if (a.residual_h16) FDBM_CUDA(cudaLaunchKernelEx(&cfg, conv_igemm_kernel<false, true>, map_a[0], map_a[1], map_a[2], map_b, p));
  else FDBM_CUDA(cudaLaunchKernelEx(&cfg, conv_igemm_kernel<false, false>, map_a[0], map_a[1], map_a[2], map_b, p));
  FDBM_LAUNCH_CHECK();
  return FDBM_OK;
}

}

using namespace fdbm;

extern "C" int fdbm_pack_conv_weights(const float* w1, int C1, int ksize, const float* w2, int C2, int Cout,
                                      void* wpack, int64_t* bytes, void* stream) {
  const int k = ksize == -1 ? 1 : ksize;
  if (bytes) *bytes = ksize == -2 ? static_cast<int64_t>(Cout) * 64 * 2 : conv_wpack_bytes(C1, k, C2, Cout);
  if (!wpack) return FDBM_OK;
  if (int rc = require_sm100()) return rc;
  FDBM_REQUIRE(w1 && ((C2 == 0) == (w2 == nullptr)), "fdbm_pack_conv_weights: null pointer");
  FDBM_REQUIRE(ksize != -2 || (C1 >= 1 && 9 * C1 <= 64 && C2 == 0), "fdbm_pack_conv_weights: ksize -2 needs 9 * C1 <= 64 and no second operand");
  return launch_pack_conv_weights(w1, C1, ksize, w2, C2, Cout, Cout, 0, reinterpret_cast<op_t*>(wpack),
                                  as_stream(stream));
}

extern "C" int fdbm_pack_conv_weights_dgrad(const float* w, int Cout, int Cin, int ksize, void* wpack, int64_t* bytes,
                                            void* stream) {
  const int k = ksize == -1 ? 1 : ksize;
  if (bytes) *bytes = conv_wpack_bytes(Cout, k, 0, Cin);
  if (!wpack) return FDBM_OK;
  if (int rc = require_sm100()) return rc;
  FDBM_REQUIRE(w, "fdbm_pack_conv_weights_dgrad: null weights");
  return launch_pack_conv_weights_dgrad(w, Cout, Cin, ksize, reinterpret_cast<op_t*>(wpack), as_stream(stream));
}

extern "C" int fdbm_conv_igemm(const void* in1, int C1, int ksize, const void* in2, int C2, const void* wpack,
                               const float* bias, const float* bias_b, const float* residual, float scale, int batch,
                               int T, int F, int Cout, float* out_f32, void* out_h16, double* sums, void* stream) {
  if (int rc = require_sm100()) return rc;
  FDBM_REQUIRE(in1 && wpack && bias && batch > 0 && T > 0 && F > 0, "fdbm_conv_igemm: bad arguments");
  FDBM_REQUIRE(ksize == 1 || ksize == 3, "fdbm_conv_igemm: ksize must be 1 or 3");
  FDBM_REQUIRE((C2 == 0) == (in2 == nullptr), "fdbm_conv_igemm: in2 / C2 mismatch");
  ConvArgs a;
  a.seg[0].in = reinterpret_cast<const op_t*>(in1); a.seg[0].C = C1; a.seg[0].taps = ksize * ksize;
  a.n_seg = 1;
  if (in2) { a.seg[1].in = reinterpret_cast<const op_t*>(in2); a.seg[1].C = C2; a.seg[1].taps = 1; a.n_seg = 2; }
  a.wpack = reinterpret_cast<const op_t*>(wpack);
  a.bias = bias; a.bias_b = bias_b; a.bias_b_stride = Cout; a.residual = residual; a.scale = scale;
  a.B = batch; a.T = T; a.F = F; a.Cout = Cout;
  a.out_f32 = out_f32; a.out_h16 = reinterpret_cast<op_t*>(out_h16); a.sums = sums;
  return launch_conv_igemm(a, as_stream(stream));
}

extern "C" int fdbm_conv_igemm_gn(const void* in1, int C1, int ksize, const double* sums1, const float* gamma,
                                  const float* beta, int silu, float* table, const void* wpack, const float* bias,
                                  const float* residual, float scale, int batch, int T, int F, int Cout, float* out_f32,
                                  void* out_h16, double* sums, void* stream) {
  if (int rc = require_sm100()) return rc;
  FDBM_REQUIRE(in1 && sums1 && gamma && beta && table && wpack && bias && batch > 0 && T > 0 && F > 0,
               "fdbm_conv_igemm_gn: bad arguments");
  FDBM_REQUIRE(ksize == 1 || ksize == 3, "fdbm_conv_igemm_gn: ksize must be 1 or 3");
  float2* tab = reinterpret_cast<float2*>(table);
  if (int rc = launch_gn_finalize(sums1, C1, nullptr, 0, gamma, beta, batch, static_cast<int64_t>(T) * F, tab, as_stream(stream)))
    return rc;
  ConvArgs a;
  a.seg[0].in = reinterpret_cast<const op_t*>(in1); a.seg[0].C = C1; a.seg[0].taps = ksize * ksize;
  a.seg[0].norm_tab = tab; a.seg[0].tab_stride = C1; a.seg[0].act = silu;
  a.n_seg = 1;
  a.wpack = reinterpret_cast<const op_t*>(wpack);
  a.bias = bias; a.residual = residual; a.scale = scale;
  a.B = batch; a.T = T; a.F = F; a.Cout = Cout;
  a.out_f32 = out_f32; a.out_h16 = reinterpret_cast<op_t*>(out_h16); a.sums = sums;
  return launch_conv_igemm(a, as_stream(stream));
}
```

### rethinking-flow-and-diffusion-bridge-models-for-speech-enhancement_b200/csrc/plan.cu

```cuda
#include <functional>
#include <map>
#include <string>
#include <unordered_map>
#include <vector>
#include "common.cuh"

using namespace fdbm;

namespace {

struct Mod {
  enum Kind { FOURIER, LINEAR, CONV3, RES, ATTN, COMBINE, GN } kind;
  int idx, cin, cout;
  bool up, down;
};

struct Slot { int64_t off; int64_t numel; bool loaded; };

struct Act {
  float* data = nullptr;
  op_t* h16 = nullptr;
  double* sums = nullptr;
  float* grad = nullptr;
  int C = 0, T = 0, F = 0;
};

struct GraphKey {
  const void* p[6]; int n_steps, kind; uint64_t seed;
  bool operator==(const GraphKey& o) const {
    for (int i = 0; i < 6; ++i) if (p[i] != o.p[i]) return false;
    return n_steps == o.n_steps && kind == o.kind && seed == o.seed;
  }
};

class Arena {
 public:
  void reset(int64_t cap) { free_.clear(); free_[0] = cap; cap_ = cap; peak_ = 0; }
  int64_t alloc(int64_t bytes) {
    bytes = (bytes + 1023) / 1024 * 1024;
    for (auto it = free_.begin(); it != free_.end(); ++it) {
      if (it->second >= bytes) {
        const int64_t off = it->first, rest = it->second - bytes;
        free_.erase(it);
        if (rest) free_[off + bytes] = rest;
        live_[off] = bytes;
        peak_ = std::max(peak_, off + bytes);
        return off;
      }
    }
    return -1;
  }
  void release(int64_t off) {
    auto it = live_.find(off);
    if (it == live_.end()) return;
    int64_t o = off, n = it->second;
    live_.erase(it);
    auto nx = free_.lower_bound(o);
    if (nx != free_.end() && o + n == nx->first) { n += nx->second; nx = free_.erase(nx); }
    if (nx != free_.begin()) {
      auto pv = std::prev(nx);
      if (pv->first + pv->second == o) { o = pv->first; n += pv->second; free_.erase(pv); }
    }
    free_[o] = n;
  }
  int64_t peak() const { return peak_; }
 private:
  std::map<int64_t, int64_t> free_, live_;
  int64_t cap_ = 0, peak_ = 0;
};

__global__ void add_vec_kernel(const float* a, const float* b, float* o, int n) {
  const int i = blockIdx.x * 256 + threadIdx.x;
  if (i < n) o[i] = a[i] + (b ? b[i] : 0.f);
}

}

struct fdbm_plan {
  fdbm_arch arch;
  int B = 0, T = 0, F = 0, F_io = 257, Cin = 4;
  std::vector<Mod> mods;
  std::unordered_map<std::string, Slot> slots;
  int64_t params_numel = 0;
  float* params = nullptr;
  op_t* wpacked = nullptr;
  int64_t wpacked_bytes = 0;
  int dense_rows = 0;
  bool weights_ready = false;
  uint8_t* arena = nullptr;
  int64_t arena_bytes = 0;
  int64_t sums_pool_bytes = 0;
  const float* cur_x = nullptr; const float* cur_y = nullptr; const float* cur_t = nullptr; int cur_t_stride = 1;
  float* cur_out = nullptr;
  float* d_buf = nullptr;
  std::vector<std::function<int(cudaStream_t)>> ops;
  std::vector<int> op_kind;
  std::vector<double> op_flops;
  std::vector<std::function<int(cudaStream_t)>> pack_ops;
  double* defer_pool = nullptr; int64_t defer_pool_bytes = 0;
  std::vector<DeferDesc> defer_descs; DeferDesc* defer_descs_d = nullptr;
  std::vector<PackDesc> pack_descs;
  PackDesc* pack_descs_d = nullptr; long long pack_blocks = 0;
  int n_launches = 0;
  bool train = false;
  float* grads = nullptr;
  op_t* wpacked_d = nullptr;
  int64_t wpacked_d_bytes = 0;
  float* wgrad_ws = nullptr;
  int64_t wgrad_ws_bytes = 0;
  std::vector<std::function<int(cudaStream_t)>> bwd_ops;
  std::vector<int> bwd_kind;
  std::vector<std::pair<void*, size_t>> zero_list;
  std::unordered_map<const void*, int> gz_index;
  std::vector<uint8_t> gz_written;
  void grads_begin() { gz_written.assign(zero_list.size(), 0); }
  bool grad_first(const float* g) {
    auto it = gz_index.find(g);
    if (it == gz_index.end() || gz_written[it->second]) return false;
    gz_written[it->second] = 1;
    return true;
  }
  int grad_ensure(const float* g, cudaStream_t s) {
    if (!grad_first(g)) return FDBM_OK;
    const auto& z = zero_list[gz_index[g]];
    FDBM_CUDA(cudaMemsetAsync(z.first, 0, z.second, s));
    return FDBM_OK;
  }
  const float* cur_gout = nullptr;
  float cur_inv = 1.0f;
  float* adam_m = nullptr; float* adam_v = nullptr; float* ema = nullptr; double* opt_scratch = nullptr;
  double* opt_state = nullptr;
  float* ema_backup = nullptr;
  bool ema_swapped = false;
  int n_bwd_launches = 0;
  int device = 0;
  static constexpr int kMaxSteps = 1024;
  static constexpr int kRing = 8;
  float* smp_y = nullptr; float* smp_x = nullptr; float* smp_times = nullptr; float* smp_coef = nullptr; uint64_t* smp_rng = nullptr;
  uint8_t* smp_pinned = nullptr;
  cudaEvent_t smp_ev[kRing] = {};
  int smp_pos = 0;
  std::vector<float> smp_h_times, smp_h_coef;
  bool have_graph = false; GraphKey graph_key{}; cudaGraphExec_t graph_exec = nullptr;
  cudaStream_t capture_stream = nullptr;
  int64_t extra_bytes = 0;
};

namespace {
constexpr size_t kSlotBytes = 16 + sizeof(float) * 4 * fdbm_plan::kMaxSteps;

int plan_guard(const fdbm_plan* plan, const char* who) {
  if (!plan) { set_error("%s: null plan", who); return FDBM_EINVAL; }
  const int dev = current_device();
  if (dev != plan->device) {
    set_error("%s: the plan lives on device %d but the current device is %d (select the tensors' device first)", who, plan->device, dev);
    return FDBM_ESTATE;
  }
  return FDBM_OK;
}
}

namespace {

std::vector<Mod> build_modules(const fdbm_arch& a) {
  std::vector<Mod> m;
  auto add = [&](Mod::Kind k, int cin, int cout, bool up = false, bool down = false) {
    m.push_back(Mod{k, static_cast<int>(m.size()), cin, cout, up, down});
  };
  const int nf = a.nf, C = a.predictive ? 2 : 4, L = a.n_levels;
  if (!a.predictive) { add(Mod::FOURIER, 0, nf); add(Mod::LINEAR, 2 * nf, 4 * nf); add(Mod::LINEAR, 4 * nf, 4 * nf); }
  add(Mod::CONV3, C, nf);
  std::vector<int> hs_c{nf};
  int in_ch = nf;
  for (int lvl = 0; lvl < L; ++lvl) {
    const int res = a.image_size >> lvl;
    for (int b = 0; b < a.num_res_blocks; ++b) {
      const int out_ch = nf * a.ch_mult[lvl];
      add(Mod::RES, in_ch, out_ch);
      in_ch = out_ch;
      if (res == a.attn_resolution) add(Mod::ATTN, in_ch, in_ch);
      hs_c.push_back(in_ch);
    }
    if (lvl != L - 1) {
      add(Mod::RES, in_ch, in_ch, false, true);
      add(Mod::COMBINE, C, in_ch);
      hs_c.push_back(in_ch);
    }
  }
  in_ch = hs_c.back();
  add(Mod::RES, in_ch, in_ch); add(Mod::ATTN, in_ch, in_ch); add(Mod::RES, in_ch, in_ch);
  for (int lvl = L - 1; lvl >= 0; --lvl) {
    const int res = a.image_size >> lvl;
    for (int b = 0; b < a.num_res_blocks + 1; ++b) {
      const int out_ch = nf * a.ch_mult[lvl];
      add(Mod::RES, in_ch + hs_c.back(), out_ch);
      hs_c.pop_back();
      in_ch = out_ch;
    }
    if (res == a.attn_resolution) add(Mod::ATTN, in_ch, in_ch);
    add(Mod::GN, in_ch, in_ch);
    add(Mod::CONV3, in_ch, C);
    if (lvl != 0) add(Mod::RES, in_ch, in_ch, true, false);
  }
  return m;
}

struct Builder {
  fdbm_plan* P;
  Arena arena;
  int64_t wp_off = 0;
  int dense_off = 0;
  bool dry = true;
  uint8_t* sums_pool = nullptr;
  int64_t sums_used = 0;

  typedef std::function<int(cudaStream_t)> Op;
  std::vector<std::vector<std::pair<Op, int>>> groups;
  int64_t wd_off = 0;
  int64_t ws_need = 0;
  op_t *T1 = nullptr, *T2 = nullptr, *T3 = nullptr, *T4 = nullptr, *T5 = nullptr;
  double *Sbuf = nullptr, *sumsA = nullptr;
  float *att_scratch = nullptr, *d_dense = nullptr, *g_temb = nullptr;
  const float* zero_bias = nullptr;
  bool train() const { return P->train; }
  int64_t defer_used = 0;
  double* site_sums(int64_t n_doubles) {
    const int64_t bytes = (n_doubles * 8 + 255) / 256 * 256;
    defer_used += bytes;
    if (dry) return reinterpret_cast<double*>(P->arena);
    return reinterpret_cast<double*>(reinterpret_cast<uint8_t*>(P->defer_pool) + defer_used - bytes);
  }
  void defer_col_sums(const double* src, int C, int64_t dst_off, float* per_b = nullptr, int per_b_ld = 0) {
    if (!dry) P->defer_descs.push_back(DeferDesc{src, P->B, C, 0, dst_off >= 0 ? P->grads + dst_off : nullptr, nullptr, per_b, per_b_ld});
  }
  void defer_gn_param(const double* S, int C, int64_t gamma_off, int64_t beta_off) {
    if (!dry) P->defer_descs.push_back(DeferDesc{S, P->B, C, 1, P->grads + gamma_off, P->grads + beta_off, nullptr, 0});
  }
  void bgroup() { if (train()) groups.emplace_back(); }
  void bop(Op f, int kind = FDBM_OP_NORM) { if (train() && !dry) groups.back().emplace_back(std::move(f), kind); }
  float* gp(int64_t off) const { return P->grads + off; }
  float* galloc(int64_t n) {
    float* g = alloc<float>(n);
    if (!dry) { P->gz_index[g] = static_cast<int>(P->zero_list.size()); P->zero_list.emplace_back(g, static_cast<size_t>(n) * sizeof(float)); }
    return g;
  }
  op_t* pack_d(int64_t w_off, int Cout, int Cin, int ksize, int Cin_total = 0, int ci_off = 0, op_t* into = nullptr) {
    const int k = ksize == -1 ? 1 : ksize;
    op_t* dst = into;
    if (!dst) {
      dst = reinterpret_cast<op_t*>(reinterpret_cast<uint8_t*>(P->wpacked_d) + wd_off);
      wd_off += (conv_wpack_bytes(Cout, k, 0, Cin) + 1023) / 1024 * 1024;
    }
    const float* w = pp(w_off);
    if (!dry) P->pack_descs.push_back(pack_desc_dgrad(w, Cout, Cin, ksize, dst, Cin_total, ci_off));
    return dst;
  }
  void dgrad_op(const op_t* dy, int Cdy, int taps, const op_t* wd, int Cdx, int T, int F, op_t* out16, float* acc) {
    ConvArgs c;
    c.seg[0] = seg(dy, Cdy, taps); c.n_seg = 1;
    c.wpack = wd; c.bias = zero_bias; c.residual = acc; c.scale = 1.0f;
    c.B = P->B; c.T = T; c.F = F; c.Cout = Cdx; c.out_f32 = acc; c.out_h16 = out16;
    fdbm_plan* plp = P;
    bop([=](cudaStream_t s) {
      ConvArgs cc = c;
      if (acc && plp->grad_first(acc)) cc.residual = nullptr;
      return launch_conv_igemm(cc, s);
    }, FDBM_OP_CONV);
  }
  void wgrad_op(WgradCall c, int64_t dw_off) {
    c.B = P->B;
    ws_need = std::max(ws_need, conv_wgrad_workspace_bytes(c.Cout, c.Cin, c.ksize, c.B, c.T, c.F));
    fdbm_plan* plp = P;
    bop([=](cudaStream_t s) {
      WgradCall cc = c;
      cc.scale = plp->cur_inv; cc.dw = plp->grads + dw_off; cc.workspace = plp->wgrad_ws;
      return launch_conv_wgrad_ex(cc, s);
    }, FDBM_OP_WGRAD);
  }
  void gn_bwd(const op_t* g_a, const Act& x1, const Act* x2, const float2* tab, const float2* stats, int64_t gw_off,
              int64_t gb_off, int act) {
    const int B = P->B, C1 = x1.C, C2 = x2 ? x2->C : 0, Ct = C1 + C2;
    const int64_t px = static_cast<int64_t>(x1.T) * x1.F;
    const float* gamma = pp(gw_off);
    double* S = site_sums(static_cast<int64_t>(B) * Ct * 2);
    defer_gn_param(S, Ct, gw_off, gb_off);
    fdbm_plan* plp = P;
    const Act a1 = x1; const Act a2 = x2 ? *x2 : Act();
    const int cb = gn_chunk(Ct, px);
    bop([=](cudaStream_t s) {
      const bool f1 = plp->grad_first(a1.grad), f2 = C2 ? plp->grad_first(a2.grad) : false;
      for (int b0 = 0; b0 < B; b0 += cb) {
        const int nb = std::min(cb, B - b0);
        if (int rc = launch_gn_bwd_reduce(g_a, Ct, 0, a1.h16, 1, C1, Ct, 0, tab, stats, act, nb, px, S, s, b0)) return rc;
        if (C2) if (int rc = launch_gn_bwd_reduce(g_a, Ct, C1, a2.h16, 1, C2, Ct, C1, tab, stats, act, nb, px, S, s, b0)) return rc;
        if (int rc = launch_gn_bwd_apply(g_a, Ct, 0, a1.h16, 1, C1, Ct, 0, tab, stats, gamma, act, nb, px, S, a1.grad, nullptr, nullptr, s, f1, b0)) return rc;
        if (C2) if (int rc = launch_gn_bwd_apply(g_a, Ct, C1, a2.h16, 1, C2, Ct, C1, tab, stats, gamma, act, nb, px, S, a2.grad, nullptr, nullptr, s, f2, b0)) return rc;
      }
      return FDBM_OK;
    });
  }
  int gn_chunk(int Ct, int64_t px) const { (void)Ct; (void)px; return P->B; }
  float2* norm_stats(const double* q1, int C1, const double* q2, int C2, int T, int F) {
    if (!train()) return nullptr;
    (void)C1; (void)q2; (void)C2; (void)T; (void)F;
    if (q1 != last_stats_q1) return nullptr;
    return last_stats;
  }

  int64_t param(const std::string& name, int64_t numel) {
    auto it = P->slots.find(name);
    if (it != P->slots.end()) return it->second.off;
    const int64_t off = P->params_numel;
    P->slots[name] = Slot{off, numel, false};
    P->params_numel += (numel + 3) / 4 * 4;
    return off;
  }
  int64_t derived(int64_t numel) {
    const int64_t off = P->params_numel;
    P->params_numel += (numel + 3) / 4 * 4;
    return off;
  }
  float* pp(int64_t off) const { return P->params + off; }
  std::string pre(const Mod& m) const { return "all_modules." + std::to_string(m.idx) + "."; }

  template <typename Tp> Tp* alloc(int64_t n_elems) {
    const int64_t off = arena.alloc(n_elems * static_cast<int64_t>(sizeof(Tp)));
    if (off < 0) return nullptr;
    return reinterpret_cast<Tp*>(P->arena + off);
  }
  void release(const void* p) { if (p && !P->train) arena.release(reinterpret_cast<const uint8_t*>(p) - P->arena); }
  double* alloc_sums(int64_t n_doubles) {
    const int64_t bytes = (n_doubles * 8 + 255) / 256 * 256;
    sums_used += bytes;
    if (dry) return reinterpret_cast<double*>(P->arena);
    return reinterpret_cast<double*>(sums_pool + sums_used - bytes);
  }
  Act new_act(int C, int T, int F) {
    Act a; a.C = C; a.T = T; a.F = F;
    a.h16 = alloc<op_t>(static_cast<int64_t>(P->B) * T * F * C);
    a.sums = alloc_sums(static_cast<int64_t>(P->B) * C * 2);
    if (P->train) a.grad = galloc(static_cast<int64_t>(P->B) * T * F * C);
    return a;
  }
  void free_act(Act& a) { release(a.data); release(a.h16); if (train()) release(a.sums); a.data = nullptr; a.h16 = nullptr; a.sums = nullptr; }
  float2* norm_table(const double* q1, int C1, const double* q2, int C2, const float* gamma, const float* beta, int T, int F) {
    const int B = P->B;
    float2* tab = alloc<float2>(static_cast<int64_t>(B) * (C1 + C2));
    const int64_t px = static_cast<int64_t>(T) * F;
    const int blk_real = P->arch.channel_block_real;
    float2* st = train() ? alloc<float2>(static_cast<int64_t>(B) * 32) : nullptr;
    last_stats = st; last_stats_q1 = q1;
    op([=](cudaStream_t s) { return launch_gn_finalize(q1, C1, q2, C2, gamma, beta, B, px, tab, s, blk_real, st); }, FDBM_OP_STATS);
    return tab;
  }
  float2* last_stats = nullptr; const double* last_stats_q1 = nullptr;
  static ConvSeg seg(const op_t* in, int C, int taps, const float2* tab = nullptr, int tab_stride = 0, int act = 0) {
    ConvSeg sg; sg.in = in; sg.C = C; sg.taps = taps; sg.norm_tab = tab; sg.tab_stride = tab_stride; sg.act = act;
    return sg;
  }

  void op(std::function<int(cudaStream_t)> f, int kind, double flops = 0.0) {
    if (dry) return;
    P->ops.push_back(std::move(f));
    P->op_kind.push_back(kind);
    P->op_flops.push_back(flops);
    P->n_launches += 1;
  }
  void conv_op(ConvArgs c, double flops = 0.0) {
    if (flops == 0.0) {
      double k = 0.0;
      for (int i = 0; i < c.n_seg; ++i) k += static_cast<double>(c.seg[i].taps) * c.seg[i].C;
      flops = 2.0 * c.B * c.T * c.F * c.Cout * k;
    }
    c.sums_prezeroed = true;
    if (c.bias_b && !train()) {
      fdbm_plan* plp = P;
      op([=](cudaStream_t s) {
        ConvArgs cc = c;
        if (plp->cur_t_stride == 0) cc.bias_b_stride = 0;
        return launch_conv_igemm(cc, s);
      }, FDBM_OP_CONV, flops);
      return;
    }
    op([=](cudaStream_t s) { return launch_conv_igemm(c, s); }, FDBM_OP_CONV, flops);
  }
  void pack_op(std::function<int(cudaStream_t)> f) { if (!dry) P->pack_ops.push_back(std::move(f)); }

  op_t* pack(const std::string& w1, int C1, int ksize, const std::string& w2, int C2, int Cout,
                      int rows_total = 0, int row_off = 0, op_t* into = nullptr) {
    const int k = ksize == -1 ? 1 : ksize;
    if (rows_total == 0) rows_total = Cout;
    op_t* dst = into;
    if (!dst) {
      dst = reinterpret_cast<op_t*>(reinterpret_cast<uint8_t*>(P->wpacked) + wp_off);
      wp_off += (conv_wpack_bytes(C1, k, C2, rows_total) + 1023) / 1024 * 1024;
    }
    const float* p1 = pp(param(w1, static_cast<int64_t>(Cout) * C1 * k * k));
    const float* p2 = C2 ? pp(param(w2, static_cast<int64_t>(Cout) * C2)) : nullptr;
    if (!dry) P->pack_descs.push_back(pack_desc_fwd(p1, C1, ksize, p2, C2, Cout, rows_total, row_off, dst));
    return dst;
  }

  struct CombineArgs { const float* pyr; const float* w; const float* b; int Cp; int64_t w_off, b_off; };
  Act resblock(const Mod& m, const Act& x1, const Act* x2, const float* dense, int dense_stride,
               const CombineArgs* comb = nullptr) {
    const int B = P->B, Cin = m.cin, Cout = m.cout;
    const int mode = m.down ? 1 : (m.up ? 2 : 0);
    const int T = x1.T, F = x1.F;
    const int To = mode == 1 ? T / 2 : (mode == 2 ? T * 2 : T), Fo = mode == 1 ? F / 2 : (mode == 2 ? F * 2 : F);
    const bool shortcut = (Cin != Cout) || m.up || m.down;
    const std::string p = pre(m);
    const int64_t o_g0w = param(p + "GroupNorm_0.weight", Cin), o_g0b = param(p + "GroupNorm_0.bias", Cin);
    const int64_t o_c0w = param(p + "Conv_0.weight", static_cast<int64_t>(Cout) * Cin * 9), o_c0b = param(p + "Conv_0.bias", Cout);
    const int64_t o_g1w = param(p + "GroupNorm_1.weight", Cout), o_g1b = param(p + "GroupNorm_1.bias", Cout);
    const int64_t o_c1w = param(p + "Conv_1.weight", static_cast<int64_t>(Cout) * Cout * 9), o_c1b = param(p + "Conv_1.bias", Cout);
    const float* g0w = pp(o_g0w); const float* g0b = pp(o_g0b); const float* c0b = pp(o_c0b);
    const float* g1w = pp(o_g1w); const float* g1b = pp(o_g1b); const float* c1b = pp(o_c1b);
    op_t* w0 = pack(p + "Conv_0.weight", Cin, 3, "", 0, Cout);
    op_t* w1 = shortcut ? pack(p + "Conv_1.weight", Cout, 3, p + "Conv_2.weight", Cin, Cout)
                                 : pack(p + "Conv_1.weight", Cout, 3, "", 0, Cout);
    const float* bias1 = c1b;
    int64_t o_c2w = -1, o_c2b = -1;
    if (shortcut) {
      o_c2w = param(p + "Conv_2.weight", static_cast<int64_t>(Cout) * Cin);
      o_c2b = param(p + "Conv_2.bias", Cout);
      const float* c2b = pp(o_c2b);
      float* bsum = pp(derived(Cout));
      bias1 = bsum;
      pack_op([=](cudaStream_t s) {
        add_vec_kernel<<<ceil_div(Cout, 256), 256, 0, s>>>(c1b, c2b, bsum, Cout);
        FDBM_LAUNCH_CHECK();
        return FDBM_OK;
      });
    }
    int dense_row = -1;
    if (!P->arch.predictive) {
      param(p + "Dense_0.weight", static_cast<int64_t>(Cout) * 4 * P->arch.nf);
      dense_row = dense_off;
      dense_off += Cout;
    }

    const int64_t npx = static_cast<int64_t>(B) * To * Fo;
    const int C1 = x1.C, C2 = x2 ? x2->C : 0;
    op_t* h1 = alloc<op_t>(npx * Cout);
    double* h1_sums = alloc_sums(static_cast<int64_t>(B) * Cout * 2);
    op_t* a0 = nullptr; op_t* xr = nullptr; float2* tab0 = nullptr;
    ConvArgs c0;
    c0.wpack = w0; c0.bias = c0b; c0.bias_b = dense_row >= 0 ? dense + dense_row : nullptr; c0.bias_b_stride = dense_stride;
    c0.B = B; c0.T = To; c0.F = Fo; c0.Cout = Cout; c0.out_h16 = h1; c0.sums = h1_sums;
    tab0 = norm_table(x1.sums, C1, x2 ? x2->sums : nullptr, C2, g0w, g0b, T, F);
    float2* stats0 = norm_stats(x1.sums, C1, x2 ? x2->sums : nullptr, C2, T, F);
    if (mode == 0) {
      c0.seg[0] = seg(x1.h16, C1, 9, tab0, Cin, 1); c0.n_seg = 1;
      if (x2) { c0.seg[1] = seg(x2->h16, C2, 9, tab0 + C1, Cin, 1); c0.n_seg = 2; }
    } else {
      a0 = alloc<op_t>(npx * Cin);
      xr = alloc<op_t>(npx * Cin);
      {
        const op_t* h1s = x1.h16; const op_t* h2s = x2 ? x2->h16 : nullptr;
        op([=](cudaStream_t s) { return launch_gn_resample16(h1s, C1, h2s, C2, tab0, B, T, F, mode, a0, xr, s); }, FDBM_OP_NORM);
      }
      c0.seg[0] = seg(a0, Cin, 9); c0.n_seg = 1;
    }
    conv_op(c0);
    release(a0); release(tab0);
    float2* tab1 = norm_table(h1_sums, Cout, nullptr, 0, g1w, g1b, To, Fo);
    float2* stats1 = norm_stats(h1_sums, Cout, nullptr, 0, To, Fo);
    Act out = new_act(Cout, To, Fo);
    {
      ConvArgs c;
      c.seg[0] = seg(h1, Cout, 9, tab1, Cout, 1); c.n_seg = 1;
      if (shortcut) {
        if (mode == 0) {
          c.seg[c.n_seg++] = seg(x1.h16, C1, 1);
          if (x2) c.seg[c.n_seg++] = seg(x2->h16, C2, 1);
        } else {
          c.seg[c.n_seg++] = seg(xr, Cin, 1);
        }
      }
      c.wpack = w1; c.bias = bias1;
      if (!shortcut) c.residual_h16 = x1.h16;
      c.scale = 0.70710678118654752f; c.B = B; c.T = To; c.F = Fo; c.Cout = Cout;
      c.out_f32 = out.data; c.out_h16 = out.h16; c.sums = out.sums;
      if (comb) { c.comb_pyr = comb->pyr; c.comb_w = comb->w; c.comb_b = comb->b; c.comb_C = comb->Cp; }
      conv_op(c);
    }
    release(h1); if (train()) release(h1_sums); release(tab1);
    release(xr);

    if (train()) {
      bgroup();
      fdbm_plan* plp = P;
      const int64_t pxo = static_cast<int64_t>(To) * Fo;
      const Act xa = x1; const Act xb = x2 ? *x2 : Act();
      op_t *t1 = T1, *t2 = T2, *t3 = T3, *t4 = T4, *t5 = T5;
      double* sA = site_sums(static_cast<int64_t>(B) * Cout);
      double* sA1 = site_sums(static_cast<int64_t>(B) * Cout);
      double* S = site_sums(static_cast<int64_t>(B) * Cout * 2);
      float* dd = d_dense;
      defer_col_sums(sA, Cout, o_c1b);
      if (o_c2b >= 0) defer_col_sums(sA, Cout, o_c2b);
      defer_gn_param(S, Cout, o_g1w, o_g1b);
      defer_col_sums(sA1, Cout, o_c0b, dense_row >= 0 ? dd + dense_row : nullptr, dense_stride);
      if (comb) {
        const CombineArgs cb = *comb; const float* og = out.grad;
        bop([=](cudaStream_t s) {
          return launch_combine_bwd(og, cb.pyr, cb.Cp, static_cast<int64_t>(B) * pxo, Cout, plp->cur_inv, plp->grads + cb.w_off, plp->grads + cb.b_off, s);
        });
      }
      {
        const float* og = out.grad; float* xg = shortcut ? nullptr : xa.grad;
        bop([=](cudaStream_t s) {
          if (int rc = plp->grad_ensure(og, s)) return rc;
          return launch_grad_prepare(og, B, pxo, Cout, 0.70710678118654752f, t1, xg, sA, s, xg && plp->grad_first(xg), true);
        });
      }
      if (shortcut) {
        if (mode == 0) {
          op_t* wd1 = pack_d(o_c2w, Cout, C1, 1, Cin, 0);
          dgrad_op(t1, Cout, 1, wd1, C1, To, Fo, nullptr, xa.grad);
          WgradCall w; w.dy = t1; w.dy_ld = Cout; w.Cout = Cout; w.x = xa.h16; w.x_ld = C1; w.Cin = C1; w.ksize = 1; w.T = To; w.F = Fo;
          w.Cin_total = Cin; w.ci_off = 0;
          wgrad_op(w, o_c2w);
          if (x2) {
            op_t* wd2 = pack_d(o_c2w, Cout, C2, 1, Cin, C1);
            dgrad_op(t1, Cout, 1, wd2, C2, To, Fo, nullptr, xb.grad);
            w.x = xb.h16; w.x_ld = C2; w.Cin = C2; w.ci_off = C1;
            wgrad_op(w, o_c2w);
          }
        } else {
          op_t* wd = pack_d(o_c2w, Cout, Cin, 1);
          dgrad_op(t1, Cout, 1, wd, Cin, To, Fo, t3, nullptr);
          float* xg = xa.grad;
          bop([=](cudaStream_t s) {
            if (int rc = plp->grad_ensure(xg, s)) return rc;
            return launch_fir_resample16(t3, Cin, 0, B, To, Fo, Cin, mode == 1 ? 2 : 1, mode == 1 ? 0.25f : 4.0f, nullptr, xg, s);
          });
          WgradCall w; w.dy = t1; w.dy_ld = Cout; w.Cout = Cout; w.x = xr; w.x_ld = Cin; w.Cin = Cin; w.ksize = 1; w.T = To; w.F = Fo;
          wgrad_op(w, o_c2w);
        }
      }
      bop([=](cudaStream_t s) { return launch_groupnorm_act(h1, 1, h1_sums, Cout, nullptr, nullptr, 0, g1w, g1b, B, To, Fo, 1, 0, t2, nullptr, s); });
      { WgradCall w; w.dy = t1; w.dy_ld = Cout; w.Cout = Cout; w.x = t2; w.x_ld = Cout; w.Cin = Cout; w.ksize = 3; w.T = To; w.F = Fo; wgrad_op(w, o_c1w); }
      dgrad_op(t1, Cout, 9, pack_d(o_c1w, Cout, Cout, 3), Cout, To, Fo, t3, nullptr);
      const int cb1 = gn_chunk(Cout, pxo);
      bop([=](cudaStream_t s) {
        for (int b0 = 0; b0 < B; b0 += cb1) {
          const int nb = std::min(cb1, B - b0);
          if (int rc = launch_gn_bwd_reduce(t3, Cout, 0, h1, 1, Cout, Cout, 0, tab1, stats1, 1, nb, pxo, S, s, b0)) return rc;
          if (int rc = launch_gn_bwd_apply(t3, Cout, 0, h1, 1, Cout, Cout, 0, tab1, stats1, g1w, 1, nb, pxo, S, nullptr, t4, sA1, s, false, b0, true)) return rc;
        }
        return FDBM_OK;
      });
      const op_t* a0b = a0;
      if (mode == 0) {
        const op_t* s1 = xa.h16; const double* q1 = xa.sums; const op_t* s2 = x2 ? xb.h16 : nullptr; const double* q2 = x2 ? xb.sums : nullptr;
        bop([=](cudaStream_t s) { return launch_groupnorm_act(s1, 1, q1, C1, s2, q2, C2, g0w, g0b, B, T, F, 1, 0, t2, nullptr, s); });
        a0b = t2;
      }
      { WgradCall w; w.dy = t4; w.dy_ld = Cout; w.Cout = Cout; w.x = a0b; w.x_ld = Cin; w.Cin = Cin; w.ksize = 3; w.T = To; w.F = Fo; wgrad_op(w, o_c0w); }
      dgrad_op(t4, Cout, 9, pack_d(o_c0w, Cout, Cin, 3), Cin, To, Fo, t3, nullptr);
      const op_t* g_act = t3;
      if (mode != 0) {
        bop([=](cudaStream_t s) { return launch_fir_resample16(t3, Cin, 0, B, To, Fo, Cin, mode == 1 ? 2 : 1, mode == 1 ? 0.25f : 4.0f, t5, nullptr, s); });
        g_act = t5;
      }
      gn_bwd(g_act, x1, x2, tab0, stats0, o_g0w, o_g0b, 1);
    }
    return out;
  }
  Act attn(const Mod& m, const Act& x) {
    const int B = P->B, C = m.cin, T = x.T, F = x.F;
    const std::string p = pre(m);
    const int64_t o_gw = param(p + "GroupNorm_0.weight", C), o_gb = param(p + "GroupNorm_0.bias", C);
    const float* gw = pp(o_gw); const float* gb = pp(o_gb);
    const int64_t o_b0 = param(p + "NIN_0.b", C), o_b1 = param(p + "NIN_1.b", C), o_b2 = param(p + "NIN_2.b", C), o_b3 = param(p + "NIN_3.b", C);
    const float* bq = pp(o_b0);
    const float* b3 = pp(o_b3);
    const int64_t o_w0 = param(p + "NIN_0.W", static_cast<int64_t>(C) * C), o_w1 = param(p + "NIN_1.W", static_cast<int64_t>(C) * C),
                  o_w2 = param(p + "NIN_2.W", static_cast<int64_t>(C) * C), o_w3 = param(p + "NIN_3.W", static_cast<int64_t>(C) * C);
    op_t* wqkv = pack(p + "NIN_0.W", C, -1, "", 0, C, 3 * C, 0);
    pack(p + "NIN_1.W", C, -1, "", 0, C, 3 * C, C, wqkv);
    pack(p + "NIN_2.W", C, -1, "", 0, C, 3 * C, 2 * C, wqkv);
    op_t* w3 = pack(p + "NIN_3.W", C, -1, "", 0, C);
    const int64_t npx = static_cast<int64_t>(B) * T * F;
    float2* tab = norm_table(x.sums, C, nullptr, 0, gw, gb, T, F);
    float2* stats = norm_stats(x.sums, C, nullptr, 0, T, F);
    op_t* qkv = alloc<op_t>(npx * 3 * C);
    {
      ConvArgs c;
      c.seg[0] = seg(x.h16, C, 1, tab, C, 0); c.n_seg = 1;
      c.wpack = wqkv; c.bias = bq; c.B = B; c.T = T; c.F = F; c.Cout = 3 * C;
      c.out_h16 = qkv;
      conv_op(c);
    }
    release(tab);
    op_t* o = alloc<op_t>(npx * C);
    const int fp32_probs = train() ? 1 : 0;
    op([=](cudaStream_t s) { return launch_attention(qkv, qkv + C, qkv + 2 * C, 3 * C, B, T * F, C, o, C, s, fp32_probs); }, FDBM_OP_ATTN);
    release(qkv);
    Act out = new_act(C, T, F);
    {
      ConvArgs c;
      c.seg[0] = seg(o, C, 1); c.n_seg = 1;
      c.wpack = w3; c.bias = b3; c.scale = 0.70710678118654752f;
      c.residual_h16 = x.h16;
      c.B = B; c.T = T; c.F = F; c.Cout = C; c.out_f32 = out.data; c.out_h16 = out.h16; c.sums = out.sums;
      conv_op(c);
    }
    release(o);
    if (train()) {
      bgroup();
      fdbm_plan* plp = P;
      const int64_t px = static_cast<int64_t>(T) * F;
      op_t *t1 = T1, *t2 = T2, *t3 = T3, *t4 = T4;
      double* sA = site_sums(static_cast<int64_t>(B) * C); float* asc = att_scratch;
      double* sQ[3] = {site_sums(static_cast<int64_t>(B) * C), site_sums(static_cast<int64_t>(B) * C), site_sums(static_cast<int64_t>(B) * C)};
      defer_col_sums(sA, C, o_b3);
      const Act xa = x;
      { const float* og = out.grad; float* xg = xa.grad;
        bop([=](cudaStream_t s) {
          if (int rc = plp->grad_ensure(og, s)) return rc;
          return launch_grad_prepare(og, B, px, C, 0.70710678118654752f, t1, xg, sA, s, plp->grad_first(xg), true);
        }); }
      { WgradCall w; w.dy = t1; w.dy_ld = C; w.Cout = C; w.x = o; w.x_ld = C; w.Cin = C; w.ksize = 1; w.T = T; w.F = F; w.layout = 1; wgrad_op(w, o_w3); }
      dgrad_op(t1, C, 1, pack_d(o_w3, C, C, -1), C, T, F, t3, nullptr);
      const int64_t o_b[3] = {o_b0, o_b1, o_b2};
      for (int i = 0; i < 3; ++i) defer_col_sums(sQ[i], C, o_b[i]);
      double *sq0 = sQ[0], *sq1 = sQ[1], *sq2 = sQ[2];
      bop([=](cudaStream_t s) {
        if (int rc = launch_attention_bwd(qkv, B, T * F, C, t3, asc, t4, s)) return rc;
        double* const sq[3] = {sq0, sq1, sq2};
        for (int i = 0; i < 3; ++i)
          if (int rc = launch_col_sums16(t4, 3 * C, i * C, B, px, C, sq[i], s, true)) return rc;
        return FDBM_OK;
      });
      { const op_t* s1 = xa.h16; const double* q1 = xa.sums;
        bop([=](cudaStream_t s) { return launch_groupnorm_act(s1, 1, q1, C, nullptr, nullptr, 0, gw, gb, B, T, F, 0, 0, t2, nullptr, s); }); }
      const int64_t o_w[3] = {o_w0, o_w1, o_w2};
      for (int i = 0; i < 3; ++i) {
        WgradCall w; w.dy = t4; w.dy_ld = 3 * C; w.dy_coff = i * C; w.Cout = C; w.x = t2; w.x_ld = C; w.Cin = C; w.ksize = 1; w.T = T; w.F = F; w.layout = 1;
        wgrad_op(w, o_w[i]);
      }
      op_t* wd = pack_d(o_w0, C, C, -1);
      pack_d(o_w1, C, C, -1); pack_d(o_w2, C, C, -1);
      dgrad_op(t4, 3 * C, 1, wd, C, T, F, t3, nullptr);
      gn_bwd(t3, x, nullptr, tab, stats, o_gw, o_gb, 0);
    }
    return out;
  }

  int build() {
    fdbm_plan& pl = *P;
    const fdbm_arch& A = pl.arch;
    const int B = pl.B, nf = A.nf, Cp = pl.Cin, L = A.n_levels;
    size_t mi = 0;
    auto next = [&]() -> const Mod& { return pl.mods[mi++]; };
    wp_off = 0; dense_off = 0; wd_off = 0; ws_need = 0; groups.clear();
    sums_used = 0;
    if (!dry && P->sums_pool_bytes > 0) {
      sums_pool = alloc<uint8_t>(P->sums_pool_bytes);
      uint8_t* pool = sums_pool; const int64_t pool_bytes = P->sums_pool_bytes;
      op([=](cudaStream_t s) { FDBM_CUDA(cudaMemsetAsync(pool, 0, pool_bytes, s)); return FDBM_OK; }, FDBM_OP_STATS);
    }
    if (train()) {
      const int64_t big = static_cast<int64_t>(B) * pl.T * pl.F * 2 * nf;
      T1 = alloc<op_t>(big); T2 = alloc<op_t>(big); T3 = alloc<op_t>(big); T4 = alloc<op_t>(big); T5 = alloc<op_t>(big);
      Sbuf = alloc<double>(static_cast<int64_t>(B) * 1024 * 2);
      sumsA = alloc<double>(static_cast<int64_t>(B) * 1024);
      const int Lmax = (pl.T >> 4) * (pl.F >> 4);
      att_scratch = alloc<float>(2ll * B * Lmax * Lmax);
      zero_bias = pp(derived(1024));
    }

    float* temb_act = nullptr; float* dense = nullptr;
    if (!A.predictive) {
      const Mod& mf = next(); const Mod& l1 = next(); const Mod& l2 = next();
// ... 614 lines not shown
```

### rethinking-flow-and-diffusion-bridge-models-for-speech-enhancement_b200/csrc/tc05.cuh

```cuda
#pragma once
#include <cuda.h>
#include <cuda_runtime.h>
#include <stdint.h>

namespace tc05 {

__device__ __forceinline__ uint32_t smem_u32(const void* p) {
  return static_cast<uint32_t>(__cvta_generic_to_shared(p));
}

__device__ __forceinline__ bool elect_one() {
  uint32_t pred = 0;
  asm volatile(
      "{\n\t.reg .pred P;\n\t"
      "elect.sync _|P, 0xffffffff;\n\t"
      "selp.u32 %0, 1, 0, P;\n\t}\n"
      : "=r"(pred));
  return pred != 0;
}

#if 0
template <int N> __device__ __forceinline__ void reg_dec() {}
template <int N> __device__ __forceinline__ void reg_inc() {}
#else
template <int N> __device__ __forceinline__ void reg_dec() { asm volatile("setmaxnreg.dec.sync.aligned.u32 %0;" :: "n"(N)); }
template <int N> __device__ __forceinline__ void reg_inc() { asm volatile("setmaxnreg.inc.sync.aligned.u32 %0;" :: "n"(N)); }
#endif

__device__ __forceinline__ void mbar_init(uint64_t* bar, uint32_t count) {
  asm volatile("mbarrier.init.shared::cta.b64 [%0], %1;" ::"r"(smem_u32(bar)), "r"(count));
}
__device__ __forceinline__ void fence_barrier_init() {
  asm volatile("fence.mbarrier_init.release.cluster;" ::: "memory");
}
__device__ __forceinline__ void fence_proxy_async() {
  asm volatile("fence.proxy.async.shared::cta;" ::: "memory");
}
__device__ __forceinline__ void mbar_expect_tx(uint64_t* bar, uint32_t bytes) {
  asm volatile("mbarrier.arrive.expect_tx.shared::cta.b64 _, [%0], %1;" ::"r"(smem_u32(bar)), "r"(bytes)
               : "memory");
}
__device__ __forceinline__ void mbar_arrive(uint64_t* bar) {
  asm volatile("mbarrier.arrive.shared::cta.b64 _, [%0];" ::"r"(smem_u32(bar)) : "memory");
}
__device__ __forceinline__ bool mbar_try_wait(uint64_t* bar, uint32_t parity) {
  uint32_t ok;
  asm volatile(
      "{\n\t.reg .pred P;\n\t"
      "mbarrier.try_wait.parity.shared::cta.b64 P, [%1], %2;\n\t"
      "selp.u32 %0, 1, 0, P;\n\t}\n"
      : "=r"(ok)
      : "r"(smem_u32(bar)), "r"(parity)
      : "memory");
  return ok != 0;
}
__device__ __forceinline__ void mbar_wait(uint64_t* bar, uint32_t parity) {
  uint32_t spins = 0;
  while (!mbar_try_wait(bar, parity)) {
    if (++spins > (1u << 22)) __trap();
  }
}

template <int NS = 40>
__device__ __forceinline__ void mbar_wait_relaxed(uint64_t* bar, uint32_t parity) {
  uint32_t spins = 0;
  while (!mbar_try_wait(bar, parity)) {
    __nanosleep(NS);
    if (++spins > (1u << 22)) __trap();
  }
}

__device__ __forceinline__ void tma_prefetch_desc(const CUtensorMap* m) {
  asm volatile("prefetch.tensormap [%0];" ::"l"(reinterpret_cast<uint64_t>(m)) : "memory");
}
__device__ __forceinline__ void tma_load_2d(void* dst, const CUtensorMap* m, uint64_t* bar, int c0, int c1) {
  asm volatile(
      "cp.async.bulk.tensor.2d.shared::cta.global.mbarrier::complete_tx::bytes [%0], [%1, {%3, %4}], [%2];"
      ::"r"(smem_u32(dst)), "l"(reinterpret_cast<uint64_t>(m)), "r"(smem_u32(bar)), "r"(c0), "r"(c1)
      : "memory");
}
__device__ __forceinline__ void tma_load_3d(void* dst, const CUtensorMap* m, uint64_t* bar, int c0, int c1, int c2) {
  asm volatile(
      "cp.async.bulk.tensor.3d.shared::cta.global.mbarrier::complete_tx::bytes [%0], [%1, {%3, %4, %5}], [%2];"
      ::"r"(smem_u32(dst)), "l"(reinterpret_cast<uint64_t>(m)), "r"(smem_u32(bar)), "r"(c0), "r"(c1), "r"(c2)
      : "memory");
}
__device__ __forceinline__ void tma_load_4d(void* dst, const CUtensorMap* m, uint64_t* bar, int c0, int c1, int c2,
                                            int c3) {
  asm volatile(
      "cp.async.bulk.tensor.4d.shared::cta.global.mbarrier::complete_tx::bytes [%0], [%1, {%3, %4, %5, %6}], [%2];"
      ::"r"(smem_u32(dst)), "l"(reinterpret_cast<uint64_t>(m)), "r"(smem_u32(bar)), "r"(c0), "r"(c1), "r"(c2),
      "r"(c3)
      : "memory");
}

__device__ __forceinline__ void tmem_alloc(uint32_t* dst_smem, uint32_t ncols) {
  asm volatile("tcgen05.alloc.cta_group::1.sync.aligned.shared::cta.b32 [%0], %1;" ::"r"(smem_u32(dst_smem)),
               "r"(ncols)
               : "memory");
}
__device__ __forceinline__ void tmem_relinquish() {
  asm volatile("tcgen05.relinquish_alloc_permit.cta_group::1.sync.aligned;" ::: "memory");
}
__device__ __forceinline__ void tmem_dealloc(uint32_t addr, uint32_t ncols) {
  asm volatile("tcgen05.dealloc.cta_group::1.sync.aligned.b32 %0, %1;" ::"r"(addr), "r"(ncols) : "memory");
}
__device__ __forceinline__ void fence_before_sync() {
  asm volatile("tcgen05.fence::before_thread_sync;" ::: "memory");
}
__device__ __forceinline__ void fence_after_sync() {
  asm volatile("tcgen05.fence::after_thread_sync;" ::: "memory");
}
__device__ __forceinline__ void mma_f16(uint32_t tmem_d, uint64_t desc_a, uint64_t desc_b, uint32_t idesc,
                                         uint32_t accumulate) {
  asm volatile(
      "{\n\t.reg .pred p;\n\t"
      "setp.ne.b32 p, %4, 0;\n\t"
      "tcgen05.mma.cta_group::1.kind::f16 [%0], %1, %2, %3, p;\n\t}\n"
      ::"r"(tmem_d), "l"(desc_a), "l"(desc_b), "r"(idesc), "r"(accumulate)
      : "memory");
}
template <int BUF, int OP>
__device__ __forceinline__ void mma_f16_ws(uint32_t tmem_d, uint64_t desc_a, uint64_t desc_b, uint32_t idesc,
                                            uint32_t accumulate) {
#define FDBM_WS_ASM(BUFS, OPS)                                                                               \
  asm volatile("{\n\t.reg .pred p;\n\tsetp.ne.b32 p, %4, 0;\n\t"                                            \
               "tcgen05.mma.ws.cta_group::1.kind::f16.collector::" BUFS "::" OPS " [%0], %1, %2, %3, p;\n\t}\n" \
               ::"r"(tmem_d), "l"(desc_a), "l"(desc_b), "r"(idesc), "r"(accumulate) : "memory")
  if constexpr (OP == 0) {
    if constexpr (BUF == 0) FDBM_WS_ASM("b0", "fill"); else if constexpr (BUF == 1) FDBM_WS_ASM("b1", "fill");
    else if constexpr (BUF == 2) FDBM_WS_ASM("b2", "fill"); else FDBM_WS_ASM("b3", "fill");
  } else if constexpr (OP == 1) {
    if constexpr (BUF == 0) FDBM_WS_ASM("b0", "lastuse"); else if constexpr (BUF == 1) FDBM_WS_ASM("b1", "lastuse");
    else if constexpr (BUF == 2) FDBM_WS_ASM("b2", "lastuse"); else FDBM_WS_ASM("b3", "lastuse");
  } else {
    if constexpr (BUF == 0) FDBM_WS_ASM("b0", "discard"); else if constexpr (BUF == 1) FDBM_WS_ASM("b1", "discard");
    else if constexpr (BUF == 2) FDBM_WS_ASM("b2", "discard"); else FDBM_WS_ASM("b3", "discard");
  }
#undef FDBM_WS_ASM
}
__device__ __forceinline__ void mma_commit(uint64_t* bar) {
  asm volatile("tcgen05.commit.cta_group::1.mbarrier::arrive::one.shared::cluster.b64 [%0];" ::"r"(smem_u32(bar))
               : "memory");
}
__device__ __forceinline__ void tmem_ld_32x32(uint32_t taddr, uint32_t (&r)[32]) {
  asm volatile(
      "tcgen05.ld.sync.aligned.32x32b.x32.b32 "
      "{%0, %1, %2, %3, %4, %5, %6, %7, %8, %9, %10, %11, %12, %13, %14, %15, "
      "%16, %17, %18, %19, %20, %21, %22, %23, %24, %25, %26, %27, %28, %29, %30, %31}, [%32];"
      : "=r"(r[0]), "=r"(r[1]), "=r"(r[2]), "=r"(r[3]), "=r"(r[4]), "=r"(r[5]), "=r"(r[6]), "=r"(r[7]),
        "=r"(r[8]), "=r"(r[9]), "=r"(r[10]), "=r"(r[11]), "=r"(r[12]), "=r"(r[13]), "=r"(r[14]), "=r"(r[15]),
        "=r"(r[16]), "=r"(r[17]), "=r"(r[18]), "=r"(r[19]), "=r"(r[20]), "=r"(r[21]), "=r"(r[22]), "=r"(r[23]),
        "=r"(r[24]), "=r"(r[25]), "=r"(r[26]), "=r"(r[27]), "=r"(r[28]), "=r"(r[29]), "=r"(r[30]), "=r"(r[31])
      : "r"(taddr)
      : "memory");
}
__device__ __forceinline__ void tmem_ld_wait() { asm volatile("tcgen05.wait::ld.sync.aligned;" ::: "memory"); }

__device__ __forceinline__ uint64_t make_desc_sw128(uint32_t smem_addr, uint32_t sbo_bytes, uint32_t base_offset = 0) {
  uint64_t d = 0;
  d |= static_cast<uint64_t>((smem_addr & 0x3FFFF) >> 4);
  d |= static_cast<uint64_t>(1) << 16;
  d |= static_cast<uint64_t>((sbo_bytes >> 4) & 0x3FFF) << 32;
  d |= static_cast<uint64_t>(1) << 46;
  d |= static_cast<uint64_t>(base_offset & 7) << 49;
  d |= static_cast<uint64_t>(2) << 61;
  return d;
}
__host__ __device__ constexpr uint32_t make_idesc_f16(int M, int N, int is_bf16) {
  return (1u << 4)
         | (static_cast<uint32_t>(is_bf16) << 7)
         | (static_cast<uint32_t>(is_bf16) << 10)
         | (static_cast<uint32_t>(N >> 3) << 17) | (static_cast<uint32_t>(M >> 4) << 24);
}

}
```

### rethinking-flow-and-diffusion-bridge-models-for-speech-enhancement_b200/fdbm_b200/_lib.py

```python
from __future__ import annotations

import ctypes as C
import functools
import os

_HERE = os.path.dirname(os.path.abspath(__file__))
LIB_PATH = os.environ.get("FDBM_B200_LIB") or os.path.join(_HERE, "libfdbm_b200.so")

FDBM_PAD = {"zero_pad": 0, "reflection": 1, "replication": 2}
FDBM_TRANSFORM = {"exponent": 0, "log": 1, "none": 2}
FDBM_STEP = {"ode_ei": 0, "sde_ei": 1}

EXPORTS = [
    "fdbm_last_error", "fdbm_version", "fdbm_check_device", "fdbm_operand_is_bf16",
    "fdbm_stft_compress", "fdbm_stft_compress_var", "fdbm_decompress_istft", "fdbm_decompress_istft_var",
    "fdbm_spec_transform", "fdbm_pad_spec",
    "fdbm_wave_absmax", "fdbm_stft_compress_ex", "fdbm_decompress_istft_ex", "fdbm_clip_rescale",
    "fdbm_prior_sample", "fdbm_bridge_step", "fdbm_bridge_update4", "fdbm_langevin_coef",
    "fdbm_lincomb", "fdbm_rk_error_norm",
    "fdbm_plan_create", "fdbm_plan_destroy", "fdbm_plan_load_weights", "fdbm_plan_device_bytes",
    "fdbm_plan_num_launches", "fdbm_ncsnpp_forward", "fdbm_sampler_run", "fdbm_plan_profile_forward",
    "fdbm_fir_resample", "fdbm_channel_stats", "fdbm_groupnorm_act", "fdbm_gn_resample_h16", "fdbm_conv_igemm", "fdbm_conv_igemm_gn",
    "fdbm_pack_conv_weights", "fdbm_attention",
    "fdbm_pack_conv_weights_dgrad", "fdbm_conv_wgrad_workspace_bytes", "fdbm_conv_wgrad",
    "fdbm_groupnorm_act_bwd", "fdbm_fir_resample_h16", "fdbm_attention_bwd", "fdbm_adam_ema_step",
    "fdbm_plan_create_train", "fdbm_ncsnpp_backward", "fdbm_plan_param_info", "fdbm_plan_buffers",
    "fdbm_plan_num_backward_launches", "fdbm_plan_optimizer_step", "fdbm_plan_profile_backward", "fdbm_plan_repack_weights",
    "fdbm_plan_reset_optimizer", "fdbm_plan_optimizer_state", "fdbm_plan_set_optimizer_state", "fdbm_plan_swap_ema",
    "fdbm_hybrid_loss_workspace_bytes", "fdbm_hybrid_loss", "fdbm_data_prediction_loss",
    "fdbm_pack_input", "fdbm_im2col_input", "fdbm_time_embedding", "fdbm_film_rows", "fdbm_combine", "fdbm_output_layer",
    "fdbm_mel_tables_bytes", "fdbm_mel_tables_init", "fdbm_mel_loss_workspace_bytes", "fdbm_mel_loss",
    "fdbm_tfg_lstm_pack_bytes", "fdbm_tfg_lstm_pack", "fdbm_tfg_lstm_sweep", "fdbm_tfg_pad_add_norm", "fdbm_tfg_sweep_post",
    "fdbm_tfg_input", "fdbm_tfg_time_embedding", "fdbm_tfg_attention_workspace_bytes", "fdbm_tfg_attention", "fdbm_tfg_output",
]


class TensorRef(C.Structure):
    _fields_ = [("name", C.c_char_p), ("data", C.c_void_p), ("numel", C.c_int64)]


class Arch(C.Structure):
    _fields_ = [("nf", C.c_int), ("n_levels", C.c_int), ("ch_mult", C.c_int * 8), ("num_res_blocks", C.c_int),
                ("attn_resolution", C.c_int), ("predictive", C.c_int), ("image_size", C.c_int), ("channel_block_real", C.c_int)]


_lib = None


def load() -> C.CDLL:
    global _lib
    if _lib is not None:
        return _lib
    if not os.path.exists(LIB_PATH):
        raise RuntimeError(
            f"{LIB_PATH} not found: build it with `python -c 'import __graft_entry__ as g; g.build()'` "
            "(or `make -C <package>/csrc`).  fdbm_b200 has no CPU or PyTorch fallback.")
    lib = C.CDLL(LIB_PATH)
    p, i, i64, f, u64, d = C.c_void_p, C.c_int, C.c_int64, C.c_float, C.c_uint64, C.c_double
    sig = {
        "fdbm_last_error": (C.c_char_p, []),
        "fdbm_version": (i, []),
        "fdbm_check_device": (i, []),
        "fdbm_operand_is_bf16": (i, []),
        "fdbm_stft_compress": (i, [p, i, i64, i64, p, i, i, i, f, f, i, i, p, p]),
        "fdbm_decompress_istft": (i, [p, i, i, p, i, i, i, f, f, i64, i64, p, p]),
        "fdbm_stft_compress_var": (i, [p, i, p, i64, i64, i64, p, i, i, i, f, f, i, i, p, p]),
        "fdbm_decompress_istft_var": (i, [p, i, i, p, i, i, i, f, f, p, i64, i64, p, p]),
        "fdbm_spec_transform": (i, [p, p, i64, i, f, f, i, p]),
        "fdbm_wave_absmax": (i, [p, i, i64, p, i64, p, p]),
        "fdbm_stft_compress_ex": (i, [p, i, p, i64, i64, i64, p, p, i, i, i, f, f, i, i, p, p]),
        "fdbm_decompress_istft_ex": (i, [p, i, i, p, i, i, i, f, f, p, i64, i64, p, p, p, p]),
        "fdbm_clip_rescale": (i, [p, i, i64, p, i64, p, f, p]),
        "fdbm_pad_spec": (i, [p, i64, i, i, i, p, p]),
        "fdbm_prior_sample": (i, [p, p, f, f, u64, u64, i64, p, p]),
        "fdbm_bridge_step": (i, [p, p, p, p, i, u64, u64, i64, p]),
        "fdbm_bridge_update4": (i, [p, p, p, p, p, u64, u64, i64, p, p]),
        "fdbm_langevin_coef": (i, [p, p, p, p, f, f, f, f, u64, u64, i, i64, p, p, p]),
        "fdbm_lincomb": (i, [p, C.POINTER(p), C.POINTER(f), i, i64, p]),
        "fdbm_rk_error_norm": (i, [C.POINTER(p), C.POINTER(f), i, p, p, f, f, i64, p, p]),
        "fdbm_plan_create": (i, [C.POINTER(Arch), i, i, C.POINTER(p)]),
        "fdbm_plan_destroy": (i, [p]),
        "fdbm_plan_load_weights": (i, [p, C.POINTER(TensorRef), i, p]),
        "fdbm_plan_device_bytes": (i64, [p]),
        "fdbm_plan_num_launches": (i, [p]),
        "fdbm_ncsnpp_forward": (i, [p, p, p, p, p, p]),
        "fdbm_sampler_run": (i, [p, p, p, p, p, i, i, p, u64, p]),
        "fdbm_plan_profile_forward": (i, [p, p, p, p, p, p, p, p, i, p]),
        "fdbm_fir_resample": (i, [p, i, i, i, i, i, p, p]),
        "fdbm_channel_stats": (i, [p, i, i, i, i, p, p]),
        "fdbm_groupnorm_act": (i, [p, p, i, p, p, i, p, p, i, i, i, i, i, p, p, p]),
        "fdbm_gn_resample_h16": (i, [p, p, i, p, p, i, p, p, p, i, i, i, i, p, p, p]),
        "fdbm_conv_igemm": (i, [p, i, i, p, i, p, p, p, p, f, i, i, i, i, p, p, p, p]),
        "fdbm_conv_igemm_gn": (i, [p, i, i, p, p, p, i, p, p, p, p, f, i, i, i, i, p, p, p, p]),
        "fdbm_pack_conv_weights": (i, [p, i, i, p, i, i, p, C.POINTER(i64), p]),
        "fdbm_pack_conv_weights_dgrad": (i, [p, i, i, i, p, C.POINTER(i64), p]),
        "fdbm_conv_wgrad_workspace_bytes": (i64, [i, i, i, i, i, i]),
        "fdbm_conv_wgrad": (i, [p, i, p, i, i, i, i, i, f, p, p, p]),
        "fdbm_groupnorm_act_bwd": (i, [p, p, i, p, p, p, i, i, i, i, i, p, p, p, p, p, p, p]),
        "fdbm_fir_resample_h16": (i, [p, i, i, i, i, i, f, p, p]),
        "fdbm_attention_bwd": (i, [p, i, i, i, p, p, p, p]),
        "fdbm_adam_ema_step": (i, [p, p, p, p, p, i64, p, f, f, f, f, f, f, i, f, i, p, p]),
        "fdbm_plan_create_train": (i, [C.POINTER(Arch), i, i, C.POINTER(p)]),
        "fdbm_ncsnpp_backward": (i, [p, p, f, i, p]),
        "fdbm_plan_param_info": (i, [p, C.c_char_p, C.POINTER(i64), C.POINTER(i64)]),
        "fdbm_plan_buffers": (i, [p, C.POINTER(p), C.POINTER(p), C.POINTER(p), C.POINTER(i64)]),
        "fdbm_plan_num_backward_launches": (i, [p]),
        "fdbm_plan_repack_weights": (i, [p, p]),
        "fdbm_hybrid_loss_workspace_bytes": (i64, [i, i, i, i]),
        "fdbm_hybrid_loss": (i, [p, p, i, i, p, i, i, i, f, f, f, p, p, p, p]),
        "fdbm_data_prediction_loss": (i, [p, p, i, i, p, i, i, i, f, f, f, f, p, p, p, p]),
        "fdbm_pack_input": (i, [p, p, i, i, i, i, i, p, p]),
        "fdbm_im2col_input": (i, [p, i, i, i, i, p, p]),
        "fdbm_time_embedding": (i, [p, p, i, p, p, p, p, i, p, p]),
        "fdbm_film_rows": (i, [p, p, p, i, i, i, p, p]),
        "fdbm_combine": (i, [p, p, i, p, p, i, i, i, i, p]),
        "fdbm_output_layer": (i, [p, i, p, p, i, i, i, i, p, p]),
        "fdbm_mel_tables_bytes": (i64, []),
        "fdbm_mel_tables_init": (i, [p, i, p]),
        "fdbm_mel_loss_workspace_bytes": (i64, [i, i, i, i]),
        "fdbm_mel_loss": (i, [p, p, i, i, p, i, i, i, f, f, i, f, p, p, p, p, p]),
        "fdbm_plan_profile_backward": (i, [p, p, f, p, p, i, p]),
        "fdbm_plan_optimizer_step": (i, [p, f, f, f, f, f, f, i, f, i, p]),
        "fdbm_plan_reset_optimizer": (i, [p, p]),
        "fdbm_plan_optimizer_state": (i, [p, C.POINTER(d), p]),
        "fdbm_plan_set_optimizer_state": (i, [p, d, d, p]),
        "fdbm_plan_swap_ema": (i, [p, i, p]),
        "fdbm_attention": (i, [p, p, p, i, i, i, p, p]),
        "fdbm_tfg_lstm_pack_bytes": (i64, []),
        "fdbm_tfg_lstm_pack": (i, [p, p, i, p, p]),
        "fdbm_tfg_lstm_sweep": (i, [p, i, i, p, p, p, p]),
        "fdbm_tfg_pad_add_norm": (i, [p, p, p, p, i, i, i, f, p, p, p]),
        "fdbm_tfg_sweep_post": (i, [p, p, p, p, i, i, i, i, p, p, f, p, p, p, i, p]),
        "fdbm_tfg_input": (i, [p, p, p, p, p, p, i, i, i, i, f, p, p, p]),
        "fdbm_tfg_time_embedding": (i, [p, i, p, p, p, p, p, p, p, i, i, p, p]),
        "fdbm_tfg_attention_workspace_bytes": (i64, [i, i, i]),
        "fdbm_tfg_attention": (i, [p, C.POINTER(p), i, i, i, f, p, p, p]),
        "fdbm_tfg_output": (i, [p, p, p, i, i, i, p, p]),
    }
    for name, (res, args) in sig.items():
        if not hasattr(lib, name) and os.environ.get("FDBM_B200_LIB"):
            continue
        fn = getattr(lib, name)
        fn.restype = res
        fn.argtypes = args
    _lib = lib
    return lib


def check(rc: int, what: str = "fdbm") -> None:
    if rc != 0:
        msg = load().fdbm_last_error()
        raise RuntimeError(f"{what} failed (code {rc}): {msg.decode() if msg else 'unknown error'}")


def operand_dtype():
    import torch
    return torch.bfloat16 if load().fdbm_operand_is_bf16() else torch.float16


def ptr(t) -> int:
    return None if t is None else t.data_ptr()


def current_stream() -> int:
    import torch
    return torch.cuda.current_stream().cuda_stream


def on_device(fn):
    @functools.wraps(fn)
    def wrapper(*args, **kwargs):
        import torch
        dev = None
        for a in list(args) + list(kwargs.values()):
            if isinstance(a, torch.Tensor) and a.is_cuda:
                if dev is None:
                    dev = a.device
                elif a.device != dev:
                    raise RuntimeError(f"{fn.__qualname__}: tensors on different devices ({dev} and {a.device})")
        if dev is None or dev.index == torch.cuda.current_device():
            return fn(*args, **kwargs)
        with torch.cuda.device(dev):
            return fn(*args, **kwargs)
    return wrapper
```

Before: 1323.

## Run implicit-GEMM conv as 2-CTA cluster pairs with cta_group::2 MMA

```diff
diff --git a/include/fdbm_b200.h b/include/fdbm_b200.h
--- a/include/fdbm_b200.h
+++ b/include/fdbm_b200.h
@@ -179,6 +179,8 @@
                        const float* beta, int silu, float* table, const void* wpack, const float* bias,
                        const float* residual, float scale, int batch, int T, int F, int Cout,
                        float* out_f32, void* out_h16, double* sums, void* stream);
+int fdbm_conv_protocol_check(int batch, int T, int F, int Cout, int n_seg, const int* seg_C, const int* seg_taps,
+                             const int* seg_norm, int flags, int n_sms, int pair_mode, int n_schedules, int* pair_out);
 int fdbm_pack_conv_weights_dgrad(const float* w, int Cout, int Cin, int ksize, void* wpack, int64_t* bytes,
                                  void* stream);
 int64_t fdbm_conv_wgrad_workspace_bytes(int Cout, int Cin, int ksize, int batch, int T, int F);
diff --git a/rethinking-flow-and-diffusion-bridge-models-for-speech-enhancement_b200/csrc/common.cuh b/rethinking-flow-and-diffusion-bridge-models-for-speech-enhancement_b200/csrc/common.cuh
--- a/rethinking-flow-and-diffusion-bridge-models-for-speech-enhancement_b200/csrc/common.cuh
+++ b/rethinking-flow-and-diffusion-bridge-models-for-speech-enhancement_b200/csrc/common.cuh
@@ -137,6 +137,7 @@
   float* pyr_out = nullptr; const float* pyr_prev = nullptr; int pyr_C = 0;
   bool narrow_n = false;
   const float* comb_pyr = nullptr; const float* comb_w = nullptr; const float* comb_b = nullptr; int comb_C = 0;
+  bool cta_pair = true;
 };
 int launch_conv_igemm(const ConvArgs& a, cudaStream_t s);
 int launch_pack_conv_weights_dgrad(const float* w, int Cout, int Cin, int ksize, op_t* wpack, cudaStream_t s, int Cin_total = 0,
diff --git a/rethinking-flow-and-diffusion-bridge-models-for-speech-enhancement_b200/csrc/conv_igemm.cu b/rethinking-flow-and-diffusion-bridge-models-for-speech-enhancement_b200/csrc/conv_igemm.cu
--- a/rethinking-flow-and-diffusion-bridge-models-for-speech-enhancement_b200/csrc/conv_igemm.cu
+++ b/rethinking-flow-and-diffusion-bridge-models-for-speech-enhancement_b200/csrc/conv_igemm.cu
@@ -1,8 +1,13 @@
 #include <cuda.h>
+#include <algorithm>
+#include <cstdio>
 #include <mutex>
+#include <string>
+#include <vector>
 #include <type_traits>
 #include "common.cuh"
 #include "tc05.cuh"
+#include "conv_walk.cuh"
 
 namespace fdbm {
 int make_act_tile_map(CUtensorMap* map, const op_t* ptr, int B, int T, int F, int C, int box_f, int box_t);
@@ -32,6 +37,9 @@
 constexpr int PIPE_REGS = 56, EPI_REGS = 168, XFORM_REGS = 120;
 #ifndef FDBM_SIDE_RING_DEFAULT
 #define FDBM_SIDE_RING_DEFAULT 1
+#endif
+#ifndef FDBM_CTA_PAIR_DEFAULT
+#define FDBM_CTA_PAIR_DEFAULT 1
 #endif
 #ifndef FDBM_EPI_RES2
 #define FDBM_EPI_RES2 1
@@ -77,6 +85,12 @@
 
 struct TileCoord { int b, t0, f0; bool valid; };
 
+__device__ __forceinline__ int cta_x() { int r; asm volatile("mov.u32 %0, %%ctaid.x;" : "=r"(r)); return r; }
+
+__host__ __device__ constexpr int a_ready_arrivals(bool pair) { return pair ? 2 * 4 : 128; }
+__host__ __device__ constexpr int acc_empty_arrivals(bool pair) { return 4 * EPI_GROUPS * (pair ? 2 : 1); }
+__host__ __device__ constexpr int side_full_arrivals(bool pair) { return pair ? 2 : 1; }
+
 __device__ __forceinline__ int fast_div(int n, int d, uint32_t mg) { return d == 1 ? n : static_cast<int>(__umulhi(static_cast<uint32_t>(n), mg)); }
 __device__ __forceinline__ int item_tile(const ConvParams& p, int item) { return fast_div(item, p.n_nblocks, p.mg_nblocks); }
 __device__ __forceinline__ int item_nblk(const ConvParams& p, int item) { return item - item_tile(p, item) * p.n_nblocks; }
@@ -92,21 +106,7 @@
   return c;
 }
 
-template <typename F>
-__device__ __forceinline__ void walk_steps(const ConvParams& p, F&& f) {
-  const int n_side = p.n_kb - p.n_main;
-  int sd = 0, cnt = 0;
-  for (int m = 0; m < p.n_main; ++m) {
-    const int ntaps = p.seg[p.ksched[m] & 15].taps;
-    for (int tap = 0; tap < ntaps; ++tap) {
-      f(false, m, tap, ntaps);
-      if (++cnt == p.side_gap && sd < n_side) { f(true, p.n_main + sd, 0, 1); ++sd; cnt = 0; }
-    }
-  }
-  for (; sd < n_side; ++sd) f(true, p.n_main + sd, 0, 1);
-}
-
-template <bool COMB, bool RES16>
+template <bool COMB, bool RES16, bool PAIR>
 __global__ void __launch_bounds__(NUM_THREADS, 1)
 conv_igemm_kernel(const __grid_constant__ CUtensorMap map_a0, const __grid_constant__ CUtensorMap map_a1,
                   const __grid_constant__ CUtensorMap map_a2, const __grid_constant__ CUtensorMap map_b,
@@ -124,8 +124,8 @@
   uint64_t* b_full = a_empty + A_STAGES;
   uint64_t* b_empty = b_full + B_STAGES_NARROW;
   uint64_t* acc_full = b_empty + B_STAGES_NARROW;
-  const int b_stages = p.bn == 16 ? B_STAGES_NARROW : B_STAGES;
-  const int b_stride = p.bn * 128;
+  const int b_stages = p.bn == 16 ? B_STAGES_NARROW : (PAIR ? 2 * B_STAGES : B_STAGES);
+  const int b_stride = PAIR ? B_TILE_BYTES / 2 : p.bn * 128;
   uint64_t* acc_empty = acc_full + 2;
   uint64_t* a_ready = acc_empty + 2;
   uint64_t* side_full = a_ready + A_STAGES;
@@ -139,10 +139,10 @@
   const int n_kb = p.n_kb;
 
   if (threadIdx.x == 0) {
-    for (int i = 0; i < A_STAGES; ++i) { mbar_init(a_full + i, 1); mbar_init(a_empty + i, 1); mbar_init(a_ready + i, 128); }
+    for (int i = 0; i < A_STAGES; ++i) { mbar_init(a_full + i, 1); mbar_init(a_empty + i, 1); mbar_init(a_ready + i, a_ready_arrivals(PAIR)); }
     for (int i = 0; i < B_STAGES_NARROW; ++i) { mbar_init(b_full + i, 1); mbar_init(b_empty + i, 1); }
-    for (int i = 0; i < 2; ++i) { mbar_init(acc_full + i, 1); mbar_init(acc_empty + i, 4 * EPI_GROUPS); }
-    mbar_init(side_full, 1); mbar_init(side_empty, 1);
+    for (int i = 0; i < 2; ++i) { mbar_init(acc_full + i, 1); mbar_init(acc_empty + i, acc_empty_arrivals(PAIR)); }
+    mbar_init(side_full, side_full_arrivals(PAIR)); mbar_init(side_empty, 1);
     fence_barrier_init();
   }
   if (warp == 0 && lane == 0) {
@@ -151,27 +151,34 @@
     if (p.n_seg > 1) tma_prefetch_desc(&map_a1);
     if (p.n_seg > 2) tma_prefetch_desc(&map_a2);
   }
+  if (PAIR) cluster_barrier_sync();
   if (warp == 3) {
-    tmem_alloc(tmem_slot, 512);
-    tmem_relinquish();
+    if (PAIR) { tmem_alloc_pair(tmem_slot, 512); tmem_relinquish_pair(); }
+    else { tmem_alloc(tmem_slot, 512); tmem_relinquish(); }
   }
   fence_before_sync();
   __syncthreads();
   fence_after_sync();
   const uint32_t tmem_base = *tmem_slot;
+  if (PAIR) cluster_barrier_sync();
   asm volatile("griddepcontrol.wait;" ::: "memory");
   asm volatile("griddepcontrol.launch_dependents;" ::: "memory");
+  const ConvWalk W = conv_walk(PAIR, static_cast<int>(blockIdx.x), static_cast<int>(gridDim.x), p.n_items);
+  const int n_rounds = W.n_rounds;
+  const uint32_t pair_rank = PAIR ? cluster_ctarank() : 0u;
+  auto in_walk = [&](int rd, int item) { return PAIR ? rd < n_rounds : item < p.n_items; };
+  auto walk_tile = [&](int item, int ct, int j) { return (PAIR && item >= p.n_items) ? p.n_mtiles : ct * MT + j; };
 
   if (warp < 4) {
   reg_dec<PIPE_REGS>();
   if (warp == 0) {
     if (lane == 0) {
       uint32_t stage = 0, phase = 0;
-      for (int item = blockIdx.x; item < p.n_items; item += gridDim.x) {
+      for (int rd = 0, item = PAIR ? W.item0 : cta_x(); in_walk(rd, item); ++rd, item += PAIR ? W.stride : static_cast<int>(gridDim.x)) {
         const int ct = item_tile(p, item);
         TileCoord tc[MT];
         int n_valid = 0;
-        for (int j = 0; j < MT; ++j) { tc[j] = decode_tile(p, ct * MT + j); n_valid += tc[j].valid; }
+        for (int j = 0; j < MT; ++j) { tc[j] = decode_tile(p, walk_tile(item, ct, j)); n_valid += tc[j].valid; }
         for (int i = 0; i < n_main; ++i) {
           const uint32_t e = p.ksched[i];
           const int sgi = e & 15, c0 = ((e >> 4) & 0xFFF) * 64;
@@ -191,20 +198,23 @@
   } else if (warp == 3) {
     if (lane == 0 && p.side_ring) {
       uint32_t phase = 0;
-      for (int item = blockIdx.x; item < p.n_items; item += gridDim.x) {
+      const uint32_t side_full_leader = PAIR ? mapa_shared(smem_u32(side_full), 0) : 0u;
+      for (int rd = 0, item = PAIR ? W.item0 : cta_x(); in_walk(rd, item); ++rd, item += PAIR ? W.stride : static_cast<int>(gridDim.x)) {
         const int ct = item_tile(p, item);
         TileCoord tc[MT];
         int n_valid = 0;
-        for (int j = 0; j < MT; ++j) { tc[j] = decode_tile(p, ct * MT + j); n_valid += tc[j].valid; }
+        for (int j = 0; j < MT; ++j) { tc[j] = decode_tile(p, walk_tile(item, ct, j)); n_valid += tc[j].valid; }
         for (int i = n_main; i < n_kb; ++i) {
           const uint32_t e = p.ksched[i];
           const int sgi = e & 15, c0 = ((e >> 4) & 0xFFF) * 64;
           mbar_wait_relaxed<128>(side_empty, phase ^ 1);
-          mbar_expect_tx(side_full, n_valid * A_TILE1_BYTES);
           const CUtensorMap* map = sgi == 0 ? &map_a0 : (sgi == 1 ? &map_a1 : &map_a2);
+          if (PAIR) mbar_arrive_expect_tx_cluster(side_full_leader, n_valid * A_TILE1_BYTES);
+          else mbar_expect_tx(side_full, n_valid * A_TILE1_BYTES);
           for (int j = 0; j < MT; ++j) {
             if (!tc[j].valid) continue;
-            tma_load_4d(sA + ((A_STAGES - 1) * MT + j) * A_TILE_STRIDE, map, side_full, c0, tc[j].f0, tc[j].t0, tc[j].b);
+            if (PAIR) tma_load_4d_pair(sA + ((A_STAGES - 1) * MT + j) * A_TILE_STRIDE, map, side_full_leader, c0, tc[j].f0, tc[j].t0, tc[j].b);
+            else tma_load_4d(sA + ((A_STAGES - 1) * MT + j) * A_TILE_STRIDE, map, side_full, c0, tc[j].f0, tc[j].t0, tc[j].b);
           }
           phase ^= 1;
         }
@@ -213,14 +223,23 @@
   } else if (warp == 1) {
     if (lane == 0) {
       uint32_t stage = 0, phase = 0;
-      for (int item = blockIdx.x; item < p.n_items; item += gridDim.x) {
+      const uint32_t b_full_leader = PAIR ? mapa_shared(smem_u32(b_full), 0) : 0u;
+      auto fetch = [&](uint32_t stage, int kt, int n0) {
+        if (PAIR) {
+          if (W.leader) mbar_expect_tx(b_full + stage, B_TILE_BYTES);
+          tma_load_2d_pair(sB + stage * b_stride, &map_b, b_full_leader + stage * 8, 0, kt * p.Cout + n0 + static_cast<int>(pair_rank) * (BN / 2));
+        } else {
+          mbar_expect_tx(b_full + stage, b_stride);
+          tma_load_2d(sB + stage * b_stride, &map_b, b_full + stage, 0, kt * p.Cout + n0);
+        }
+      };
+      for (int rd = 0, item = PAIR ? W.item0 : cta_x(); in_walk(rd, item); ++rd, item += PAIR ? W.stride : static_cast<int>(gridDim.x)) {
         const int n0 = item_nblk(p, item) * BN;
         if (p.side_ring) {
           walk_steps(p, [&](bool, int idx, int tap, int) {
             const int kt = static_cast<int>(p.ksched[idx] >> 16) + tap;
             mbar_wait_relaxed<128>(b_empty + stage, phase ^ 1);
-            mbar_expect_tx(b_full + stage, b_stride);
-            tma_load_2d(sB + stage * b_stride, &map_b, b_full + stage, 0, kt * p.Cout + n0);
+            fetch(stage, kt, n0);
             if (++stage == b_stages) { stage = 0; phase ^= 1; }
           });
           continue;
@@ -231,24 +250,27 @@
           int kt = e >> 16;
           for (int tap = 0; tap < ntaps; ++tap, ++kt) {
             mbar_wait_relaxed<128>(b_empty + stage, phase ^ 1);
-            mbar_expect_tx(b_full + stage, b_stride);
-            tma_load_2d(sB + stage * b_stride, &map_b, b_full + stage, 0, kt * p.Cout + n0);
+            fetch(stage, kt, n0);
             if (++stage == b_stages) { stage = 0; phase ^= 1; }
           }
         }
       }
     }
   } else if (warp == 2) {
-    const uint32_t idesc = make_idesc_f16(128, p.bn, kOperandIsBf16);
+    const uint32_t idesc = make_idesc_f16(PAIR ? 256 : 128, p.bn, kOperandIsBf16);
     const uint64_t a_hi9 = make_desc_sw128(0, A_SBO) & 0xFFFFFFFF00000000ull;
     const uint64_t a_hi1 = make_desc_sw128(0, TILE_F * 128) & 0xFFFFFFFF00000000ull;
     const uint64_t b_hi = make_desc_sw128(0, 1024) & 0xFFFFFFFF00000000ull;
     const uint32_t lo_const = 1u << 16;
     const uint32_t sA_lo = (smem_u32(sA) & 0x3FFFF) >> 4, sB_lo = (smem_u32(sB) & 0x3FFFF) >> 4;
     uint32_t sa = 0, pa = 0, sb = 0, pb = 0, as = 0, pacc = 0, ps = 0;
-    for (int item = blockIdx.x; item < p.n_items; item += gridDim.x) {
+    auto mma = [&](uint32_t d, uint64_t da, uint64_t db, uint32_t acc) {
+      if (PAIR) mma_f16_pair(d, da, db, idesc, acc); else mma_f16(d, da, db, idesc, acc);
+    };
+    auto commit = [&](uint64_t* bar) { if (PAIR) mma_commit_cg2(bar); else mma_commit(bar); };
+    for (int rd = 0, item = PAIR ? W.item0 : cta_x(); W.leader && in_walk(rd, item); ++rd, item += PAIR ? W.stride : static_cast<int>(gridDim.x)) {
       const int ct = item_tile(p, item);
-      const bool valid1 = (ct * MT + 1) < p.n_mtiles;
+      const bool valid1 = PAIR || (ct * MT + 1) < p.n_mtiles;
       mbar_wait(acc_empty + as, pacc ^ 1);
       fence_after_sync();
       uint32_t accumulate = 0;
@@ -264,7 +286,7 @@
             a_base0 = sA_lo + (((A_STAGES - 1) * MT) * A_TILE_STRIDE >> 4);
           } else {
             if (tap == 0) {
-              mbar_wait(sg.norm ? a_ready + sa : a_full + sa, pa);
+              mbar_wait((PAIR || sg.norm) ? a_ready + sa : a_full + sa, pa);
               fence_after_sync();
             }
             a_base0 = sA_lo + ((sa * MT) * A_TILE_STRIDE >> 4);
@@ -280,16 +302,16 @@
           if (elect_one()) {
 #pragma unroll
             for (int k = 0; k < 4; ++k)
-              mma_f16(d0, a_hi | (a_lo0 + 2 * k), b_hi | (b_lo + 2 * k), idesc, k == 0 ? accumulate : 1u);
+              mma(d0, a_hi | (a_lo0 + 2 * k), b_hi | (b_lo + 2 * k), k == 0 ? accumulate : 1u);
             if (valid1) {
 #pragma unroll
               for (int k = 0; k < 4; ++k)
-                mma_f16(d1, a_hi | (a_lo1 + 2 * k), b_hi | (b_lo + 2 * k), idesc, k == 0 ? accumulate : 1u);
+                mma(d1, a_hi | (a_lo1 + 2 * k), b_hi | (b_lo + 2 * k), k == 0 ? accumulate : 1u);
             }
-            mma_commit(b_empty + sb);
-            if (side) mma_commit(side_empty);
-            else if (last_tap) mma_commit(a_empty + sa);
-            if (step == p.n_steps - 1) mma_commit(acc_full + as);
+            commit(b_empty + sb);
+            if (side) commit(side_empty);
+            else if (last_tap) commit(a_empty + sa);
+            if (step == p.n_steps - 1) commit(acc_full + as);
           }
           __syncwarp();
           accumulate = 1;
@@ -305,7 +327,7 @@
         const SegParams& sg = p.seg[p.ksched[i] & 15];
         const int ntaps = sg.taps;
         const uint64_t a_hi = sg.halo ? a_hi9 : a_hi1;
-        mbar_wait(sg.norm ? a_ready + sa : a_full + sa, pa);
+        mbar_wait((PAIR || sg.norm) ? a_ready + sa : a_full + sa, pa);
         fence_after_sync();
         const uint32_t a_base0 = sA_lo + ((sa * MT) * A_TILE_STRIDE >> 4), a_base1 = a_base0 + (A_TILE_STRIDE >> 4);
         int df = ntaps == 9 ? 0 : sg.halo, dt = df;
@@ -331,16 +353,16 @@
             {
 #pragma unroll
               for (int k = 0; k < 4; ++k)
-                mma_f16(d0, a_hi | (a_lo0 + 2 * k), b_hi | (b_lo + 2 * k), idesc, k == 0 ? accumulate : 1u);
+                mma(d0, a_hi | (a_lo0 + 2 * k), b_hi | (b_lo + 2 * k), k == 0 ? accumulate : 1u);
               if (valid1) {
 #pragma unroll
                 for (int k = 0; k < 4; ++k)
-                  mma_f16(d1, a_hi | (a_lo1 + 2 * k), b_hi | (b_lo + 2 * k), idesc, k == 0 ? accumulate : 1u);
+                  mma(d1, a_hi | (a_lo1 + 2 * k), b_hi | (b_lo + 2 * k), k == 0 ? accumulate : 1u);
               }
             }
-            mma_commit(b_empty + sb);
-            if (tap == ntaps - 1) mma_commit(a_empty + sa);
-            if (tap == ntaps - 1 && i == n_kb - 1) mma_commit(acc_full + as);
+            commit(b_empty + sb);
+            if (tap == ntaps - 1) commit(a_empty + sa);
+            if (tap == ntaps - 1 && i == n_kb - 1) commit(acc_full + as);
           }
           __syncwarp();
           accumulate = 1;
@@ -358,10 +380,11 @@
     const int g = tt & 7, p_lane = tt >> 3;
     uint32_t stage = 0, phase = 0;
     const bool any_norm = (p.seg[0].norm | p.seg[1].norm | p.seg[2].norm) != 0;
-    for (int item = blockIdx.x; any_norm && item < p.n_items; item += gridDim.x) {
+    const uint32_t a_ready_leader = PAIR ? mapa_shared(smem_u32(a_ready), 0) : 0u;
+    for (int rd = 0, item = PAIR ? W.item0 : cta_x(); (PAIR || any_norm) && in_walk(rd, item); ++rd, item += PAIR ? W.stride : static_cast<int>(gridDim.x)) {
       const int ct = item_tile(p, item);
       TileCoord tc[MT];
-      for (int j = 0; j < MT; ++j) tc[j] = decode_tile(p, ct * MT + j);
+      for (int j = 0; j < MT; ++j) tc[j] = decode_tile(p, walk_tile(item, ct, j));
       for (int i = 0; i < n_main; ++i) {
         const uint32_t e = p.ksched[i];
         const SegParams& sg = p.seg[e & 15];
@@ -453,7 +476,12 @@
           }
           fence_proxy_async();
         }
-        mbar_arrive(a_ready + stage);
+        if (PAIR) {
+          __syncwarp();
+          if (lane == 0) mbar_arrive_cluster(a_ready_leader + stage * 8);
+        } else {
+          mbar_arrive(a_ready + stage);
+        }
         if (++stage == a_stages) { stage = 0; phase ^= 1; }
       }
     }
@@ -485,14 +513,15 @@
         acc_s[u] = 0.0; acc_q[u] = 0.0;
       }
     };
-    for (int item = blockIdx.x; item < p.n_items; item += gridDim.x) {
+    const uint32_t acc_empty_leader = PAIR ? mapa_shared(smem_u32(acc_empty), 0) : 0u;
+    for (int rd = 0, item = PAIR ? W.item0 : cta_x(); in_walk(rd, item); ++rd, item += PAIR ? W.stride : static_cast<int>(gridDim.x)) {
       const int ct = item_tile(p, item);
       const int nblk = item - ct * p.n_nblocks;
       const int n0 = nblk * BN;
       mbar_wait_relaxed(acc_full + as, pacc);
       fence_after_sync();
       for (int j = eg; j <= eg; ++j) {
-        const TileCoord tc = decode_tile(p, ct * MT + j);
+        const TileCoord tc = decode_tile(p, walk_tile(item, ct, j));
         if (!tc.valid) continue;
 #if defined(FDBM_EPI_TEST)
         {
@@ -587,7 +616,7 @@
         float* of_p = p.out_f32 ? p.out_f32 + tile_base : nullptr;
         op_t* oh_p = p.out_h16 ? p.out_h16 + tile_base : nullptr;
         if (RES16 || res_p) {
-          const int nitem = item + gridDim.x;
+          const int nitem = item + (PAIR ? W.stride : static_cast<int>(gridDim.x));
           const int nct = item_tile(p, nitem);
           const int nmi = nitem < p.n_items ? nct * MT + j : p.n_mtiles;
           const int nblk_n = nitem - nct * p.n_nblocks;
@@ -778,7 +807,7 @@
       }
       fence_before_sync();
       __syncwarp();
-      if (lane == 0) mbar_arrive(acc_empty + as);
+      if (lane == 0) { if (PAIR) mbar_arrive_cluster(acc_empty_leader + as * 8); else mbar_arrive(acc_empty + as); }
       if (++as == 2) { as = 0; pacc ^= 1; }
     }
     if (do_stats && stat_b >= 0) flush_stats();
@@ -786,7 +815,8 @@
 
   fence_before_sync();
   __syncthreads();
-  if (warp == 3) tmem_dealloc(tmem_base, 512);
+  if (PAIR) cluster_barrier_sync();
+  if (warp == 3) { if (PAIR) tmem_dealloc_pair(tmem_base, 512); else tmem_dealloc(tmem_base, 512); }
 }
 
 __device__ __forceinline__ void pack_fwd_element(const PackDesc& d, int64_t i) {
@@ -953,22 +983,14 @@
   return FDBM_OK;
 }
 
-int launch_conv_igemm(const ConvArgs& a, cudaStream_t s) {
+static int conv_setup(const ConvArgs& a, int n_sms, int pair_mode, ConvParams& p, int& grid_out, bool& pair_out) {
   FDBM_REQUIRE(a.n_seg >= 1 && a.n_seg <= MAX_SEG, "conv_igemm: 1..%d K segments", MAX_SEG);
   const int bn = a.narrow_n ? 16 : (a.Cout == 64 ? 64 : BN);
   FDBM_REQUIRE(a.Cout % bn == 0 && (!a.narrow_n || (a.Cout == 16 && a.pyr_out)), "conv_igemm: Cout must be a multiple of %d (got %d)", bn, a.Cout);
   FDBM_REQUIRE(a.out_f32 || a.out_h16 || a.pyr_out, "conv_igemm: no output");
   FDBM_REQUIRE(!a.pyr_out || (a.pyr_C >= 1 && a.pyr_C <= 4 && a.Cout == bn && !a.sums), "conv_igemm: bad pyramid epilogue arguments");
   FDBM_REQUIRE(!a.pyr_prev || (a.T % 2 == 0 && a.F % 2 == 0), "conv_igemm: pyramid level with odd size");
-  static PerDeviceOnce attr_once;
-  if (attr_once.first(current_device())) {
-    FDBM_CUDA(cudaFuncSetAttribute(conv_igemm_kernel<false, false>, cudaFuncAttributeMaxDynamicSharedMemorySize, SMEM_BYTES));
-    FDBM_CUDA(cudaFuncSetAttribute(conv_igemm_kernel<false, true>, cudaFuncAttributeMaxDynamicSharedMemorySize, SMEM_BYTES));
-    FDBM_CUDA(cudaFuncSetAttribute(conv_igemm_kernel<true, false>, cudaFuncAttributeMaxDynamicSharedMemorySize, SMEM_BYTES));
-  }
   FDBM_REQUIRE(!a.comb_pyr || (a.comb_w && a.comb_b && a.comb_C >= 1 && a.comb_C <= 4 && !a.pyr_out), "conv_igemm: bad Combine epilogue arguments");
-  CUtensorMap map_a[MAX_SEG], map_b;
-  ConvParams p;
   p.B = a.B; p.T = a.T; p.F = a.F; p.Cout = a.Cout;
   p.n_seg = a.n_seg;
   int kb = 0, n_kt = 0;
@@ -978,15 +1000,12 @@
       FDBM_REQUIRE(sg.in && sg.C > 0 && sg.C % 64 == 0 && (sg.taps == 9 || sg.taps == 1),
                    "conv_igemm: segment %d needs a tensor, C %% 64 == 0 and 9 or 1 taps (C=%d, taps=%d)", i, sg.C, sg.taps);
       const int halo = sg.taps == 9 || sg.norm_tab != nullptr;
-      if (int rc = halo ? make_act_map(&map_a[i], sg.in, a.B, a.T, a.F, sg.C)
-                        : make_act_tile_map(&map_a[i], sg.in, a.B, a.T, a.F, sg.C, TILE_F, TILE_T)) return rc;
       p.seg[i].halo = halo;
       kb += sg.C / 64; p.seg[i].taps = sg.taps;
       p.seg[i].norm = sg.norm_tab != nullptr; p.seg[i].act = sg.act; p.seg[i].tab = sg.norm_tab;
       p.seg[i].tab_stride = sg.tab_stride;
       n_kt += (sg.C / 64) * sg.taps;
     } else {
-      map_a[i] = map_a[0];
       p.seg[i] = SegParams{1, 0, 0, 0, 0, nullptr};
     }
   }
@@ -1023,7 +1042,6 @@
     p.side_gap = p.side_ring ? std::max(3, ceil_div(9 * n9, n1)) : 0;
     p.n_steps = n_kt;
   }
-  if (int rc = make_weight_map(&map_b, a.wpack, static_cast<int64_t>(n_kt) * a.Cout, bn)) return rc;
   p.bn = bn;
   p.tiles_t = ceil_div(a.T, TILE_T); p.tiles_f = ceil_div(a.F, TILE_F);
   p.n_mtiles = a.B * p.tiles_t * p.tiles_f;
@@ -1033,7 +1051,7 @@
     auto magic = [](int d) { return static_cast<uint32_t>((0x100000000ull + d - 1) / static_cast<uint64_t>(d)); };
     p.mg_tiles_t = magic(p.tiles_t); p.mg_tiles_f = magic(p.tiles_f); p.mg_nblocks = magic(p.n_nblocks);
     const int64_t dmax = std::max(std::max(p.tiles_t, p.tiles_f), p.n_nblocks);
-    FDBM_REQUIRE((2 * (static_cast<int64_t>(p.n_items) + num_sms()) + 2) * dmax < 0x100000000ll, "conv_igemm: %d items exceed the range of the index arithmetic", p.n_items);
+    FDBM_REQUIRE((2 * (static_cast<int64_t>(p.n_items) + n_sms) + 2) * dmax < 0x100000000ll, "conv_igemm: %d items exceed the range of the index arithmetic", p.n_items);
   }
   p.bias = a.bias; p.bias_b = a.bias_b; p.bias_b_stride = a.bias_b_stride; p.residual = a.residual; p.scale = a.scale;
   p.residual_h16 = a.residual_h16;
@@ -1041,21 +1059,363 @@
   p.out_f32 = a.out_f32; p.out_h16 = a.out_h16; p.sums = a.sums;
   p.pyr_out = a.pyr_out; p.pyr_prev = a.pyr_prev; p.pyr_C = a.pyr_C;
   p.comb_pyr = a.comb_pyr; p.comb_w = a.comb_w; p.comb_b = a.comb_b; p.comb_C = a.comb_C;
-  if (a.sums) {
-    FDBM_REQUIRE(p.n_nblocks <= STAT_SLOTS, "conv_igemm: channel sums support Cout <= %d", STAT_SLOTS * BN);
-    if (!a.sums_prezeroed) FDBM_CUDA(cudaMemsetAsync(a.sums, 0, sizeof(double) * 2 * a.B * a.Cout, s));
-  }
-  const int grid = std::min(p.n_items, num_sms());
+  if (a.sums) FDBM_REQUIRE(p.n_nblocks <= STAT_SLOTS, "conv_igemm: channel sums support Cout <= %d", STAT_SLOTS * BN);
+  int grid = std::min(p.n_items, n_sms);
+  bool pair = false;
+  int n_seg9 = 0;
+  for (int i = 0; i < a.n_seg; ++i) n_seg9 += a.seg[i].taps == 9;
+  const bool pick = n_seg9 == 1;
+  if (pair_mode && (pick || pair_mode == 2) && a.cta_pair && bn == BN && !a.comb_pyr && !a.pyr_out && p.n_items >= 2 * n_sms) {
+    const int g2 = grid & ~1;
+    if (g2 >= 2 && (g2 / 2) % p.n_nblocks == 0) { pair = true; grid = g2; }
+  }
+  grid_out = grid; pair_out = pair;
+  return FDBM_OK;
+}
+
+int launch_conv_igemm(const ConvArgs& a, cudaStream_t s) {
+  static PerDeviceOnce attr_once;
+  if (attr_once.first(current_device())) {
+    FDBM_CUDA(cudaFuncSetAttribute(conv_igemm_kernel<false, false, false>, cudaFuncAttributeMaxDynamicSharedMemorySize, SMEM_BYTES));
+    FDBM_CUDA(cudaFuncSetAttribute(conv_igemm_kernel<false, true, false>, cudaFuncAttributeMaxDynamicSharedMemorySize, SMEM_BYTES));
+    FDBM_CUDA(cudaFuncSetAttribute(conv_igemm_kernel<true, false, false>, cudaFuncAttributeMaxDynamicSharedMemorySize, SMEM_BYTES));
+    FDBM_CUDA(cudaFuncSetAttribute(conv_igemm_kernel<false, false, true>, cudaFuncAttributeMaxDynamicSharedMemorySize, SMEM_BYTES));
+    FDBM_CUDA(cudaFuncSetAttribute(conv_igemm_kernel<false, true, true>, cudaFuncAttributeMaxDynamicSharedMemorySize, SMEM_BYTES));
+  }
+  static const int pair_env = getenv("FDBM_CTA_PAIR") ? atoi(getenv("FDBM_CTA_PAIR")) : FDBM_CTA_PAIR_DEFAULT;
+  ConvParams p;
+  int grid = 0;
+  bool pair = false;
+  if (int rc = conv_setup(a, num_sms(), pair_env, p, grid, pair)) return rc;
+  CUtensorMap map_a[MAX_SEG], map_b;
+  for (int i = 0; i < MAX_SEG; ++i) {
+    if (i >= a.n_seg) { map_a[i] = map_a[0]; continue; }
+    const ConvSeg& sg = a.seg[i];
+    if (int rc = p.seg[i].halo ? make_act_map(&map_a[i], sg.in, a.B, a.T, a.F, sg.C)
+                               : make_act_tile_map(&map_a[i], sg.in, a.B, a.T, a.F, sg.C, TILE_F, TILE_T)) return rc;
+  }
+  if (int rc = make_weight_map(&map_b, a.wpack, static_cast<int64_t>(p.n_steps) * a.Cout, pair ? p.bn / 2 : p.bn)) return rc;
+  if (a.sums && !a.sums_prezeroed) FDBM_CUDA(cudaMemsetAsync(a.sums, 0, sizeof(double) * 2 * a.B * a.Cout, s));
   cudaLaunchConfig_t cfg = {};
   cfg.gridDim = dim3(grid); cfg.blockDim = dim3(NUM_THREADS); cfg.dynamicSmemBytes = SMEM_BYTES; cfg.stream = s;
-  cudaLaunchAttribute attr[1];
-  attr[0].id = cudaLaunchAttributeProgrammaticStreamSerialization;
-  attr[0].val.programmaticStreamSerializationAllowed = 1;
-  cfg.attrs = attr; cfg.numAttrs = pdl_enabled() && a.B <= pdl_batch_limit() ? 1 : 0;
-  if (a.comb_pyr) FDBM_CUDA(cudaLaunchKernelEx(&cfg, conv_igemm_kernel<true, false>, map_a[0], map_a[1], map_a[2], map_b, p));
-  else if (a.residual_h16) FDBM_CUDA(cudaLaunchKernelEx(&cfg, conv_igemm_kernel<false, true>, map_a[0], map_a[1], map_a[2], map_b, p));
-  else FDBM_CUDA(cudaLaunchKernelEx(&cfg, conv_igemm_kernel<false, false>, map_a[0], map_a[1], map_a[2], map_b, p));
+  cudaLaunchAttribute attr[2];
+  int n_attr = 0;
+  if (pdl_enabled() && a.B <= pdl_batch_limit()) {
+    attr[n_attr].id = cudaLaunchAttributeProgrammaticStreamSerialization;
+    attr[n_attr].val.programmaticStreamSerializationAllowed = 1;
+    ++n_attr;
+  }
+  if (pair) {
+    attr[n_attr].id = cudaLaunchAttributeClusterDimension;
+    attr[n_attr].val.clusterDim.x = 2; attr[n_attr].val.clusterDim.y = 1; attr[n_attr].val.clusterDim.z = 1;
+    ++n_attr;
+  }
+  cfg.attrs = attr; cfg.numAttrs = n_attr;
+  if (a.comb_pyr) FDBM_CUDA(cudaLaunchKernelEx(&cfg, conv_igemm_kernel<true, false, false>, map_a[0], map_a[1], map_a[2], map_b, p));
+  else if (a.residual_h16 && pair) FDBM_CUDA(cudaLaunchKernelEx(&cfg, conv_igemm_kernel<false, true, true>, map_a[0], map_a[1], map_a[2], map_b, p));
+  else if (a.residual_h16) FDBM_CUDA(cudaLaunchKernelEx(&cfg, conv_igemm_kernel<false, true, false>, map_a[0], map_a[1], map_a[2], map_b, p));
+  else if (pair) FDBM_CUDA(cudaLaunchKernelEx(&cfg, conv_igemm_kernel<false, false, true>, map_a[0], map_a[1], map_a[2], map_b, p));
+  else FDBM_CUDA(cudaLaunchKernelEx(&cfg, conv_igemm_kernel<false, false, false>, map_a[0], map_a[1], map_a[2], map_b, p));
   FDBM_LAUNCH_CHECK();
+  return FDBM_OK;
+}
+
+
+namespace {
+enum : int { OP_WAIT, OP_ARRIVE, OP_EXPECT, OP_COMPLETE };
+struct SimOp { int kind, bar, count; int64_t bytes, target; int parity; };
+struct SimBar { int init = 1, pending = 1; int64_t tx = 0, completed = 0; };
+struct SimRole { const char* name; int cta; std::vector<SimOp> ops; size_t pc = 0; };
+
+constexpr int BAR_A_FULL = 0, BAR_A_EMPTY = BAR_A_FULL + A_STAGES, BAR_B_FULL = BAR_A_EMPTY + A_STAGES,
+              BAR_B_EMPTY = BAR_B_FULL + B_STAGES_NARROW, BAR_ACC_FULL = BAR_B_EMPTY + B_STAGES_NARROW, BAR_ACC_EMPTY = BAR_ACC_FULL + 2,
+              BAR_A_READY = BAR_ACC_EMPTY + 2, BAR_SIDE_FULL = BAR_A_READY + A_STAGES, BAR_SIDE_EMPTY = BAR_SIDE_FULL + 1,
+              N_BARS = BAR_SIDE_EMPTY + 1;
+
+struct ProtocolSim {
+  const ConvParams& p;
+  bool pair;
+  int grid;
+  std::vector<SimBar> bars;
+  std::vector<SimRole> roles;
+  std::string err;
+  ProtocolSim(const ConvParams& p_, bool pair_, int grid_) : p(p_), pair(pair_), grid(grid_) {}
+
+  int bid(int cta, int local) const { return cta * N_BARS + local; }
+  struct Uses {
+    std::vector<int64_t> n = std::vector<int64_t>(2 * N_BARS, 0);
+    int64_t& operator[](int b) { return n[b]; }
+  };
+  static SimOp wait(int bar, int parity, int64_t target) { return SimOp{OP_WAIT, bar, 0, 0, target, parity}; }
+
+  void build_cta(int block, int r) {
+    const ConvWalk W = conv_walk(pair, block, grid, p.n_items);
+    const int a_stages = p.side_ring ? A_STAGES - 1 : A_STAGES;
+    const int n_main = p.side_ring ? p.n_main : p.n_kb;
+    const int b_stages = p.bn == 16 ? B_STAGES_NARROW : (pair ? 2 * B_STAGES : B_STAGES);
+    const int b_stride = pair ? B_TILE_BYTES / 2 : p.bn * 128;
+    const int lead = 0;
+    auto n_valid_of = [&](int item) {
+      if (item >= p.n_items) return 0;
+      const int ct = item / p.n_nblocks;
+      int v = 0;
+      for (int j = 0; j < MT; ++j) v += (ct * MT + j) < p.n_mtiles;
+      return v;
+    };
+    {
+      SimRole R{"A producer", r, {}}; Uses u;
+      uint32_t stage = 0, phase = 0;
+      for (int rd = 0; rd < W.n_rounds; ++rd) {
+        const int nv = n_valid_of(walk_item(W, rd));
+        for (int i = 0; i < n_main; ++i) {
+          const int halo = p.seg[p.ksched[i] & 15].halo;
+          const int ae = bid(r, BAR_A_EMPTY + stage), af = bid(r, BAR_A_FULL + stage);
+          R.ops.push_back(wait(ae, phase ^ 1, u[af] - 1));
+          const int64_t tile = halo ? A_TILE_BYTES : A_TILE1_BYTES;
+          R.ops.push_back(SimOp{OP_EXPECT, af, 1, nv * tile, u[af], 0});
+          for (int j = 0; j < nv; ++j) R.ops.push_back(SimOp{OP_COMPLETE, af, 0, tile, u[af], 0});
+          ++u[af];
+          if (++stage == static_cast<uint32_t>(a_stages)) { stage = 0; phase ^= 1; }
+        }
+      }
+      roles.push_back(std::move(R));
+    }
+    if (p.side_ring) {
+      SimRole R{"side producer", r, {}}; Uses u;
+      uint32_t phase = 0;
+      const int sf = bid(pair ? lead : r, BAR_SIDE_FULL), se = bid(r, BAR_SIDE_EMPTY);
+      for (int rd = 0; rd < W.n_rounds; ++rd) {
+        const int nv = n_valid_of(walk_item(W, rd));
+        for (int i = n_main; i < p.n_kb; ++i) {
+          R.ops.push_back(wait(se, phase ^ 1, u[se] - 1));
+          ++u[se];
+          R.ops.push_back(SimOp{OP_EXPECT, sf, 1, static_cast<int64_t>(nv) * A_TILE1_BYTES, u[sf], 0});
+          for (int j = 0; j < nv; ++j) R.ops.push_back(SimOp{OP_COMPLETE, sf, 0, A_TILE1_BYTES, u[sf], 0});
+          ++u[sf];
+          phase ^= 1;
+        }
+      }
+      roles.push_back(std::move(R));
+    }
+    {
+      SimRole R{"B producer", r, {}}; Uses u;
+      uint32_t stage = 0, phase = 0;
+      for (int rd = 0; rd < W.n_rounds; ++rd) {
+        const int item = walk_item(W, rd);
+        const int nblk = item % p.n_nblocks;
+        if (pair && r == 1) {
+          const ConvWalk L = conv_walk(true, block - 1, grid, p.n_items);
+          const int litem = walk_item(L, rd);
+          if (litem >= p.n_items) { err = "pair: the leader has no item in a round of its peer"; return; }
+          if (litem % p.n_nblocks != nblk) { err = "pair: the two CTAs are on different output-channel blocks in one round"; return; }
+        }
+        auto step = [&]() {
+          const int be = bid(r, BAR_B_EMPTY + stage), bf = bid(pair ? lead : r, BAR_B_FULL + stage);
+          R.ops.push_back(wait(be, phase ^ 1, u[be] - 1));
+          ++u[be];
+          if (!pair || r == 0) R.ops.push_back(SimOp{OP_EXPECT, bf, 1, pair ? B_TILE_BYTES : b_stride, u[bf], 0});
+          R.ops.push_back(SimOp{OP_COMPLETE, bf, 0, b_stride, u[bf], 0});
+          ++u[bf];
+          if (++stage == static_cast<uint32_t>(b_stages)) { stage = 0; phase ^= 1; }
+        };
+        if (p.side_ring) walk_steps(p, [&](bool, int, int, int) { step(); });
+        else for (int i = 0; i < p.n_kb; ++i) for (int tap = 0; tap < p.seg[p.ksched[i] & 15].taps; ++tap) step();
+      }
+      roles.push_back(std::move(R));
+    }
+    if (W.leader) {
+      SimRole R{"MMA issuer", r, {}}; Uses u;
+      uint32_t sa = 0, pa = 0, sb = 0, pb = 0, as = 0, pacc = 0, ps = 0;
+      const int peer = pair ? 1 : -1;
+      auto commit = [&](int local) {
+        const int b0 = bid(r, local);
+        R.ops.push_back(SimOp{OP_ARRIVE, b0, 1, 0, u[b0]++, 0});
+        if (peer >= 0) { const int b1 = bid(peer, local); R.ops.push_back(SimOp{OP_ARRIVE, b1, 1, 0, u[b1]++, 0}); }
+      };
+      Uses wu;
+      for (int rd = 0; rd < W.n_rounds; ++rd) {
+        const int ae = bid(r, BAR_ACC_EMPTY + as);
+        R.ops.push_back(wait(ae, pacc ^ 1, wu[ae]++ - 1));
+        if (p.side_ring) {
+          int stp = 0;
+          walk_steps(p, [&](bool side, int idx, int tap, int ntaps) {
+            const SegParams& sg = p.seg[p.ksched[idx] & 15];
+            if (side) { const int b = bid(r, BAR_SIDE_FULL); R.ops.push_back(wait(b, ps, wu[b]++)); }
+            else if (tap == 0) { const int b = bid(r, ((pair || sg.norm) ? BAR_A_READY : BAR_A_FULL) + sa); R.ops.push_back(wait(b, pa, wu[b]++)); }
+            { const int b = bid(r, BAR_B_FULL + sb); R.ops.push_back(wait(b, pb, wu[b]++)); }
+            const bool last_tap = tap == ntaps - 1;
+            commit(BAR_B_EMPTY + sb);
+            if (side) commit(BAR_SIDE_EMPTY);
+            else if (last_tap) commit(BAR_A_EMPTY + sa);
+            if (stp == p.n_steps - 1) commit(BAR_ACC_FULL + as);
+            ++stp;
+            if (++sb == static_cast<uint32_t>(b_stages)) { sb = 0; pb ^= 1; }
+            if (side) ps ^= 1;
+            else if (last_tap && ++sa == static_cast<uint32_t>(a_stages)) { sa = 0; pa ^= 1; }
+          });
+        } else {
+          for (int i = 0; i < p.n_kb; ++i) {
+            const SegParams& sg = p.seg[p.ksched[i] & 15];
+            { const int b = bid(r, ((pair || sg.norm) ? BAR_A_READY : BAR_A_FULL) + sa); R.ops.push_back(wait(b, pa, wu[b]++)); }
+            for (int tap = 0; tap < sg.taps; ++tap) {
+              { const int b = bid(r, BAR_B_FULL + sb); R.ops.push_back(wait(b, pb, wu[b]++)); }
+              commit(BAR_B_EMPTY + sb);
+              if (tap == sg.taps - 1) commit(BAR_A_EMPTY + sa);
+              if (tap == sg.taps - 1 && i == p.n_kb - 1) commit(BAR_ACC_FULL + as);
+              if (++sb == static_cast<uint32_t>(b_stages)) { sb = 0; pb ^= 1; }
+            }
+            if (++sa == A_STAGES) { sa = 0; pa ^= 1; }
+          }
+        }
+        if (++as == 2) { as = 0; pacc ^= 1; }
+      }
+      roles.push_back(std::move(R));
+    }
+    const bool any_norm = (p.seg[0].norm | p.seg[1].norm | p.seg[2].norm) != 0;
+    if (pair || any_norm) {
+      SimRole R{"transform", r, {}}; Uses u;
+      uint32_t stage = 0, phase = 0;
+      for (int rd = 0; rd < W.n_rounds; ++rd)
+        for (int i = 0; i < n_main; ++i) {
+          const int af = bid(r, BAR_A_FULL + stage), ar = bid(pair ? lead : r, BAR_A_READY + stage);
+          R.ops.push_back(wait(af, phase, u[af]++));
+          R.ops.push_back(SimOp{OP_ARRIVE, ar, pair ? 4 : 128, 0, u[ar]++, 0});
+          if (++stage == static_cast<uint32_t>(a_stages)) { stage = 0; phase ^= 1; }
+        }
+      roles.push_back(std::move(R));
+    }
+    for (int eg = 0; eg < EPI_GROUPS; ++eg) {
+      SimRole R{eg ? "epilogue 1" : "epilogue 0", r, {}}; Uses u;
+      uint32_t as = 0, pacc = 0;
+      for (int rd = 0; rd < W.n_rounds; ++rd) {
+        const int af = bid(r, BAR_ACC_FULL + as), ae = bid(pair ? lead : r, BAR_ACC_EMPTY + as);
+        R.ops.push_back(wait(af, pacc, u[af]++));
+        R.ops.push_back(SimOp{OP_ARRIVE, ae, 4, 0, u[ae]++, 0});
+        if (++as == 2) { as = 0; pacc ^= 1; }
+      }
+      roles.push_back(std::move(R));
+    }
+  }
+
+  void init_bars() {
+    bars.assign(2 * N_BARS, SimBar{});
+    for (int c = 0; c < 2; ++c) {
+      auto set = [&](int local, int n) { bars[bid(c, local)].init = n; bars[bid(c, local)].pending = n; };
+      for (int i = 0; i < A_STAGES; ++i) set(BAR_A_READY + i, a_ready_arrivals(pair));
+      for (int i = 0; i < 2; ++i) set(BAR_ACC_EMPTY + i, acc_empty_arrivals(pair));
+      set(BAR_SIDE_FULL, side_full_arrivals(pair));
+    }
+  }
+
+  std::string where(const SimRole& R, const SimOp& o) const {
+    char buf[256];
+    const SimBar& b = bars[o.bar];
+    snprintf(buf, sizeof buf, "%s of CTA %d, barrier %d of CTA %d (phase %lld, pending %d, tx %lld), op for phase %lld", R.name, R.cta,
+             o.bar % N_BARS, o.bar / N_BARS, static_cast<long long>(b.completed), b.pending, static_cast<long long>(b.tx),
+             static_cast<long long>(o.target));
+    return buf;
+  }
+
+  bool step(SimRole& R) {
+    const SimOp& o = R.ops[R.pc];
+    SimBar& b = bars[o.bar];
+    if (o.kind == OP_WAIT) {
+      if (((b.completed & 1) == static_cast<int64_t>(o.parity))) return false;
+      if (((o.target + 2) & 1) != o.parity) { err = "wait parity does not match the phase it means: " + where(R, o); return false; }
+      if (b.completed != o.target + 1) { err = "wait passes on the wrong phase (parity aliasing): " + where(R, o); return false; }
+    } else {
+      if (b.completed != o.target) { err = "arrival / bytes land in another phase: " + where(R, o); return false; }
+      if (o.kind == OP_ARRIVE || o.kind == OP_EXPECT) {
+        b.pending -= o.count;
+        if (b.pending < 0) { err = "more arrivals than the init count in one phase: " + where(R, o); return false; }
+      }
+      if (o.kind == OP_EXPECT) b.tx += o.bytes;
+      if (o.kind == OP_COMPLETE) b.tx -= o.bytes;
+      if (b.pending == 0 && b.tx == 0) { ++b.completed; b.pending = b.init; }
+    }
+    ++R.pc;
+    return true;
+  }
+
+  bool run(int schedule) {
+    init_bars();
+    for (auto& R : roles) R.pc = 0;
+    uint64_t rng = 0x9E3779B97F4A7C15ull * static_cast<uint64_t>(schedule + 1);
+    auto next = [&]() { rng ^= rng << 13; rng ^= rng >> 7; rng ^= rng << 17; return rng; };
+    for (;;) {
+      bool progress = false, done = true;
+      const size_t n = roles.size();
+      const size_t off = schedule ? next() % n : 0;
+      for (size_t k = 0; k < n; ++k) {
+        SimRole& R = roles[(k + off) % n];
+        const int burst = schedule ? 1 + static_cast<int>(next() % 64) : 1;
+        for (int t = 0; t < burst && R.pc < R.ops.size(); ++t) {
+          if (!step(R)) break;
+          progress = true;
+        }
+        if (!err.empty()) return false;
+        done = done && R.pc == R.ops.size();
+      }
+      if (done) break;
+      if (!progress) {
+        err = "deadlock:";
+        for (auto& R : roles)
+          if (R.pc < R.ops.size()) err += " [" + where(R, R.ops[R.pc]) + (R.ops[R.pc].kind == OP_WAIT ? " waits]" : "]");
+        return false;
+      }
+    }
+    for (int i = 0; i < static_cast<int>(bars.size()); ++i)
+      if (bars[i].pending != bars[i].init || bars[i].tx != 0) {
+        char buf[160];
+        snprintf(buf, sizeof buf, "barrier %d of CTA %d ends inside a phase (pending %d of %d, tx %lld)", i % N_BARS, i / N_BARS,
+                 bars[i].pending, bars[i].init, static_cast<long long>(bars[i].tx));
+        err = buf;
+        return false;
+      }
+    return true;
+  }
+};
+}
+
+static int conv_protocol_check(const ConvArgs& a, int n_sms, int pair_mode, int n_schedules, int* pair_out) {
+  ConvParams p;
+  int grid = 0;
+  bool pair = false;
+  if (int rc = conv_setup(a, n_sms, pair_mode, p, grid, pair)) return rc;
+  if (pair_out) *pair_out = pair ? 1 : 0;
+  std::vector<int> seen(p.n_items, 0);
+  for (int blk = 0; blk < grid; ++blk) {
+    const ConvWalk W = conv_walk(pair, blk, grid, p.n_items);
+    for (int rd = 0; rd < W.n_rounds; ++rd) {
+      const int item = walk_item(W, rd);
+      if (item < p.n_items) ++seen[item];
+      else FDBM_REQUIRE(pair && (blk & 1) && rd == W.n_rounds - 1, "conv protocol: ghost round outside the last round of a pair's second CTA");
+    }
+  }
+  for (int i = 0; i < p.n_items; ++i) FDBM_REQUIRE(seen[i] == 1, "conv protocol: item %d walked %d times", i, seen[i]);
+  const int unit = pair ? 2 : 1, n_units = grid / unit;
+  std::vector<int> pick;
+  int prev_sig = -1;
+  for (int q = 0; q < n_units; ++q) {
+    int sig = 0;
+    for (int r = 0; r < unit; ++r) {
+      const ConvWalk W = conv_walk(pair, q * unit + r, grid, p.n_items);
+      const int last = W.n_rounds ? walk_item(W, W.n_rounds - 1) : 0;
+      const int ct = last / p.n_nblocks;
+      sig = sig * 4096 + W.n_rounds * 4 + (last >= p.n_items ? 2 : 0) + ((ct * MT + 1) < p.n_mtiles ? 1 : 0);
+    }
+    if (q == 0 || q == n_units - 1 || sig != prev_sig) { if (q > 0 && sig != prev_sig) pick.push_back(q - 1); pick.push_back(q); }
+    prev_sig = sig;
+  }
+  std::sort(pick.begin(), pick.end());
+  pick.erase(std::unique(pick.begin(), pick.end()), pick.end());
+  for (int q : pick) {
+    ProtocolSim sim(p, pair, grid);
+    for (int r = 0; r < unit; ++r) sim.build_cta(q * unit + r, r);
+    FDBM_REQUIRE(sim.err.empty(), "conv protocol (CTA %d): %s", q * unit, sim.err.c_str());
+    for (int sch = 0; sch < n_schedules; ++sch)
+      FDBM_REQUIRE(sim.run(sch), "conv protocol (CTA %d, %s, schedule %d): %s", q * unit, pair ? "pair" : "alone", sch, sim.err.c_str());
+  }
   return FDBM_OK;
 }
 
@@ -1124,3 +1484,23 @@
   a.out_f32 = out_f32; a.out_h16 = reinterpret_cast<op_t*>(out_h16); a.sums = sums;
   return launch_conv_igemm(a, as_stream(stream));
 }
+
+extern "C" int fdbm_conv_protocol_check(int batch, int T, int F, int Cout, int n_seg, const int* seg_C, const int* seg_taps,
+                                        const int* seg_norm, int flags, int n_sms, int pair_mode, int n_schedules, int* pair_out) {
+  FDBM_REQUIRE(n_seg >= 1 && n_seg <= 3 && seg_C && seg_taps && batch > 0 && T > 0 && F > 0 && n_sms >= 1, "fdbm_conv_protocol_check: bad arguments");
+  static const float dummy_f[16] = {};
+  static const op_t dummy_h[8] = {};
+  static const float2 dummy_tab[1] = {};
+  ConvArgs a;
+  a.n_seg = n_seg;
+  for (int i = 0; i < n_seg; ++i) {
+    a.seg[i].in = dummy_h; a.seg[i].C = seg_C[i]; a.seg[i].taps = seg_taps[i];
+    a.seg[i].norm_tab = seg_norm && seg_norm[i] ? dummy_tab : nullptr; a.seg[i].act = 1; a.seg[i].tab_stride = seg_C[i];
+  }
+  a.wpack = dummy_h; a.bias = dummy_f; a.B = batch; a.T = T; a.F = F; a.Cout = Cout;
+  a.out_h16 = const_cast<op_t*>(dummy_h);
+  if (flags & 1) { a.narrow_n = true; a.pyr_out = const_cast<float*>(dummy_f); a.pyr_C = 4; a.out_h16 = nullptr; }
+  if (flags & 2) { a.comb_pyr = dummy_f; a.comb_w = dummy_f; a.comb_b = dummy_f; a.comb_C = 2; }
+  if (flags & 4) a.cta_pair = false;
+  return conv_protocol_check(a, n_sms, pair_mode, n_schedules, pair_out);
+}
diff --git a/rethinking-flow-and-diffusion-bridge-models-for-speech-enhancement_b200/csrc/conv_walk.cuh b/rethinking-flow-and-diffusion-bridge-models-for-speech-enhancement_b200/csrc/conv_walk.cuh
--- /dev/null
+++ b/rethinking-flow-and-diffusion-bridge-models-for-speech-enhancement_b200/csrc/conv_walk.cuh
@@ -0,0 +1,40 @@
+#pragma once
+
+namespace fdbm {
+
+struct ConvWalk {
+  int item0;
+  int lead0;
+  int stride;
+  int n_rounds;
+  bool leader;
+};
+
+__host__ __device__ inline ConvWalk conv_walk(bool pair, int block, int grid, int n_items) {
+  ConvWalk w;
+  w.stride = grid;
+  w.lead0 = pair ? block >> 1 : block;
+  w.item0 = pair ? (block >> 1) + (block & 1) * (grid >> 1) : block;
+  const int first = pair ? w.lead0 : w.item0;
+  w.n_rounds = first < n_items ? (n_items - 1 - first) / grid + 1 : 0;
+  w.leader = !pair || (block & 1) == 0;
+  return w;
+}
+__host__ __device__ inline int walk_item(const ConvWalk& w, int round) { return w.item0 + round * w.stride; }
+
+#pragma nv_exec_check_disable
+template <typename P, typename F>
+__host__ __device__ __forceinline__ void walk_steps(const P& p, F&& f) {
+  const int n_side = p.n_kb - p.n_main;
+  int sd = 0, cnt = 0;
+  for (int m = 0; m < p.n_main; ++m) {
+    const int ntaps = p.seg[p.ksched[m] & 15].taps;
+    for (int tap = 0; tap < ntaps; ++tap) {
+      f(false, m, tap, ntaps);
+      if (++cnt == p.side_gap && sd < n_side) { f(true, p.n_main + sd, 0, 1); ++sd; cnt = 0; }
+    }
+  }
+  for (; sd < n_side; ++sd) f(true, p.n_main + sd, 0, 1);
+}
+
+}
diff --git a/rethinking-flow-and-diffusion-bridge-models-for-speech-enhancement_b200/csrc/plan.cu b/rethinking-flow-and-diffusion-bridge-models-for-speech-enhancement_b200/csrc/plan.cu
--- a/rethinking-flow-and-diffusion-bridge-models-for-speech-enhancement_b200/csrc/plan.cu
+++ b/rethinking-flow-and-diffusion-bridge-models-for-speech-enhancement_b200/csrc/plan.cu
@@ -260,6 +260,7 @@
     c.seg[0] = seg(dy, Cdy, taps); c.n_seg = 1;
     c.wpack = wd; c.bias = zero_bias; c.residual = acc; c.scale = 1.0f;
     c.B = P->B; c.T = T; c.F = F; c.Cout = Cdx; c.out_f32 = acc; c.out_h16 = out16;
+    c.cta_pair = false;
     fdbm_plan* plp = P;
     bop([=](cudaStream_t s) {
       ConvArgs cc = c;
@@ -373,6 +374,7 @@
       flops = 2.0 * c.B * c.T * c.F * c.Cout * k;
     }
     c.sums_prezeroed = true;
+    if (train()) c.cta_pair = false;
     if (c.bias_b && !train()) {
       fdbm_plan* plp = P;
       op([=](cudaStream_t s) {
diff --git a/rethinking-flow-and-diffusion-bridge-models-for-speech-enhancement_b200/csrc/tc05.cuh b/rethinking-flow-and-diffusion-bridge-models-for-speech-enhancement_b200/csrc/tc05.cuh
--- a/rethinking-flow-and-diffusion-bridge-models-for-speech-enhancement_b200/csrc/tc05.cuh
+++ b/rethinking-flow-and-diffusion-bridge-models-for-speech-enhancement_b200/csrc/tc05.cuh
@@ -54,10 +54,17 @@
       : "memory");
   return ok != 0;
 }
+__device__ __forceinline__ void mbar_timeout(uint64_t* bar, uint32_t parity) {
+#ifdef FDBM_MBAR_DEBUG
+  printf("mbarrier wait timed out: block %d (cluster rank %u) thread %d barrier +0x%x parity %u\n", static_cast<int>(blockIdx.x),
+         blockIdx.x & 1u, static_cast<int>(threadIdx.x), smem_u32(bar) & 0x3FFFFu, parity);
+#endif
+  __trap();
+}
 __device__ __forceinline__ void mbar_wait(uint64_t* bar, uint32_t parity) {
   uint32_t spins = 0;
   while (!mbar_try_wait(bar, parity)) {
-    if (++spins > (1u << 22)) __trap();
+    if (++spins > (1u << 22)) mbar_timeout(bar, parity);
   }
 }
 
@@ -66,7 +73,7 @@
   uint32_t spins = 0;
   while (!mbar_try_wait(bar, parity)) {
     __nanosleep(NS);
-    if (++spins > (1u << 22)) __trap();
+    if (++spins > (1u << 22)) mbar_timeout(bar, parity);
   }
 }
 
@@ -143,6 +150,55 @@
   asm volatile("tcgen05.commit.cta_group::1.mbarrier::arrive::one.shared::cluster.b64 [%0];" ::"r"(smem_u32(bar))
                : "memory");
 }
+__device__ __forceinline__ uint32_t cluster_ctarank() { uint32_t r; asm volatile("mov.u32 %0, %%cluster_ctarank;" : "=r"(r)); return r; }
+__device__ __forceinline__ uint32_t mapa_shared(uint32_t local_addr, uint32_t rank) {
+  uint32_t r; asm volatile("mapa.shared::cluster.u32 %0, %1, %2;" : "=r"(r) : "r"(local_addr), "r"(rank)); return r;
+}
+__device__ __forceinline__ void cluster_barrier_sync() {
+  asm volatile("barrier.cluster.arrive.release;" ::: "memory");
+  asm volatile("barrier.cluster.wait.acquire;" ::: "memory");
+}
+__device__ __forceinline__ void mbar_arrive_cluster(uint32_t bar_cluster_addr) {
+  asm volatile("mbarrier.arrive.release.cluster.shared::cluster.b64 _, [%0];" ::"r"(bar_cluster_addr) : "memory");
+}
+__device__ __forceinline__ void mbar_arrive_expect_tx_cluster(uint32_t bar_cluster_addr, uint32_t bytes) {
+  asm volatile("mbarrier.arrive.expect_tx.release.cluster.shared::cluster.b64 _, [%0], %1;" ::"r"(bar_cluster_addr), "r"(bytes)
+               : "memory");
+}
+__device__ __forceinline__ void tmem_alloc_pair(uint32_t* dst_smem, uint32_t ncols) {
+  asm volatile("tcgen05.alloc.cta_group::2.sync.aligned.shared::cta.b32 [%0], %1;" ::"r"(smem_u32(dst_smem)), "r"(ncols) : "memory");
+}
+__device__ __forceinline__ void tmem_relinquish_pair() { asm volatile("tcgen05.relinquish_alloc_permit.cta_group::2.sync.aligned;" ::: "memory"); }
+__device__ __forceinline__ void tmem_dealloc_pair(uint32_t addr, uint32_t ncols) {
+  asm volatile("tcgen05.dealloc.cta_group::2.sync.aligned.b32 %0, %1;" ::"r"(addr), "r"(ncols) : "memory");
+}
+__device__ __forceinline__ void mma_f16_pair(uint32_t tmem_d, uint64_t desc_a, uint64_t desc_b, uint32_t idesc, uint32_t accumulate) {
+  asm volatile(
+      "{\n\t.reg .pred p;\n\t"
+      "setp.ne.b32 p, %4, 0;\n\t"
+      "tcgen05.mma.cta_group::2.kind::f16 [%0], %1, %2, %3, p;\n\t}\n"
+      ::"r"(tmem_d), "l"(desc_a), "l"(desc_b), "r"(idesc), "r"(accumulate)
+      : "memory");
+}
+__device__ __forceinline__ void mma_commit_cg2(uint64_t* bar) {
+  const uint16_t mask = 3;
+  asm volatile("tcgen05.commit.cta_group::2.mbarrier::arrive::one.shared::cluster.multicast::cluster.b64 [%0], %1;" ::"r"(smem_u32(bar)), "h"(mask)
+               : "memory");
+}
+__device__ __forceinline__ void tma_load_2d_pair(void* dst, const CUtensorMap* m, uint32_t bar_cluster_addr, int c0, int c1) {
+  asm volatile(
+      "cp.async.bulk.tensor.2d.cta_group::2.shared::cluster.global.mbarrier::complete_tx::bytes [%0], [%1, {%3, %4}], [%2];"
+      ::"r"(smem_u32(dst)), "l"(reinterpret_cast<uint64_t>(m)), "r"(bar_cluster_addr), "r"(c0), "r"(c1)
+      : "memory");
+}
+__device__ __forceinline__ void tma_load_4d_pair(void* dst, const CUtensorMap* m, uint32_t bar_cluster_addr, int c0, int c1, int c2,
+                                                 int c3) {
+  asm volatile(
+      "cp.async.bulk.tensor.4d.cta_group::2.shared::cluster.global.mbarrier::complete_tx::bytes [%0], [%1, {%3, %4, %5, %6}], [%2];"
+      ::"r"(smem_u32(dst)), "l"(reinterpret_cast<uint64_t>(m)), "r"(bar_cluster_addr), "r"(c0), "r"(c1), "r"(c2), "r"(c3)
+      : "memory");
+}
+
 __device__ __forceinline__ void tmem_ld_32x32(uint32_t taddr, uint32_t (&r)[32]) {
   asm volatile(
       "tcgen05.ld.sync.aligned.32x32b.x32.b32 "
diff --git a/rethinking-flow-and-diffusion-bridge-models-for-speech-enhancement_b200/fdbm_b200/_lib.py b/rethinking-flow-and-diffusion-bridge-models-for-speech-enhancement_b200/fdbm_b200/_lib.py
--- a/rethinking-flow-and-diffusion-bridge-models-for-speech-enhancement_b200/fdbm_b200/_lib.py
+++ b/rethinking-flow-and-diffusion-bridge-models-for-speech-enhancement_b200/fdbm_b200/_lib.py
@@ -21,6 +21,7 @@
     "fdbm_plan_create", "fdbm_plan_destroy", "fdbm_plan_load_weights", "fdbm_plan_device_bytes",
     "fdbm_plan_num_launches", "fdbm_ncsnpp_forward", "fdbm_sampler_run", "fdbm_plan_profile_forward",
     "fdbm_fir_resample", "fdbm_channel_stats", "fdbm_groupnorm_act", "fdbm_gn_resample_h16", "fdbm_conv_igemm", "fdbm_conv_igemm_gn",
+    "fdbm_conv_protocol_check",
     "fdbm_pack_conv_weights", "fdbm_attention",
     "fdbm_pack_conv_weights_dgrad", "fdbm_conv_wgrad_workspace_bytes", "fdbm_conv_wgrad",
     "fdbm_groupnorm_act_bwd", "fdbm_fir_resample_h16", "fdbm_attention_bwd", "fdbm_adam_ema_step",
@@ -92,6 +93,7 @@
         "fdbm_gn_resample_h16": (i, [p, p, i, p, p, i, p, p, p, i, i, i, i, p, p, p]),
         "fdbm_conv_igemm": (i, [p, i, i, p, i, p, p, p, p, f, i, i, i, i, p, p, p, p]),
         "fdbm_conv_igemm_gn": (i, [p, i, i, p, p, p, i, p, p, p, p, f, i, i, i, i, p, p, p, p]),
+        "fdbm_conv_protocol_check": (i, [i, i, i, i, i, p, p, p, i, i, i, i, p]),
         "fdbm_pack_conv_weights": (i, [p, i, i, p, i, i, p, C.POINTER(i64), p]),
         "fdbm_pack_conv_weights_dgrad": (i, [p, i, i, i, p, C.POINTER(i64), p]),
         "fdbm_conv_wgrad_workspace_bytes": (i64, [i, i, i, i, i, i]),
```

Measured after the change: 1346 (median of 6 runs). +1.7%, better.
